# NJU-LHRS/LHRS-Bot

Hardware: AMD Instinct MI355X
Metric: stage-1 pretrain samples/sec (224^2 image + 128-tok caption) (higher is better)
Workload: dtype bf16

## Files before the change

### include/lhrs_hip.h

```cpp
#ifndef LHRS_HIP_H
#define LHRS_HIP_H
#include <stdint.h>
#ifdef __cplusplus
extern "C" {
#endif

typedef uint16_t lhrs_bf16_t;

const char* lhrs_last_error(void);
int lhrs_abi_version(void);
const char* lhrs_target_arch(void);

int lhrs_gemm_bf16_nt(const void* A, int lda, const void* B, int ldb, void* C, int ldc, int M, int N, int K,
                      const void* bias, const void* residual, int ldr, int act, int out_f32, int accumulate,
                      float alpha, void* stream);

int lhrs_gemm_bf16_nt_lora(const void* A, int lda, const void* B, int ldb, const void* A2, int lda2, const void* B2, int ldb2,
                           int K2, void* C, int ldc, int M, int N, int K, const void* bias, const void* residual, int ldr,
                           int out_f32, int accumulate, float alpha, void* stream);
int lhrs_gemm_fp8_nt(const void* A8, long lda, const float* sa, const void* B8, long ldb, const float* sb, void* C, int ldc,
                     int M, int N, int K, const void* residual, int ldr, float alpha, void* stream);
int lhrs_gemm_fp8_nt_lora(const void* A8, long lda, const float* sa, const void* B8, long ldb, const float* sb, const void* A2,
                          int lda2, const void* B2, int ldb2, int K2, void* C, int ldc, int M, int N, int K,
                          const void* residual, int ldr, float alpha, void* stream);
int lhrs_rmsnorm_fwd_q(const void* x, long ldx, const void* w, void* y, long ldy, void* y8, float* y8scale, int rows,
                       int cols, float eps, void* stream);
int lhrs_rmsnorm_bwd_q(const void* dy, const void* x, const void* w, const float* rstd, const void* add, void* dx,
                       void* dx8, float* dx8scale, int rows, int cols, float eps, void* stream);
int lhrs_swiglu_fwd_q(const void* gate_up, void* act, void* act8, float* scale, long rows, int F, void* stream);
int lhrs_swiglu_bwd_q(const void* dact, const void* gate_up, void* dgu, void* dgu8, float* scale, long rows, int F, void* stream);
int lhrs_gemm_skinny_splits(int K, int N);
int lhrs_gemm_bf16_nt_skinny(const void* A, int lda, const void* B, int ldb, void* C, int ldc, int M, int N, int K, float alpha,
                             float* workspace, void* stream);
int lhrs_gemm_splitk_splits(int M, int N, int K);
int lhrs_gemm_tn_splits(int T, int Mo, int No);
int lhrs_gemm_tn_f32(const void* P, long ldp, const void* Q, long ldq, float* C, long ldc, int T, int Mo, int No, float* workspace,
                     void* stream);
int lhrs_gemm_bf16_nt_splitk_f32(const void* A, int lda, const void* B, int ldb, float* C, int ldc, int M, int N, int K,
                                 float* workspace, void* stream);
int lhrs_gemm_swiglu_fusable(int M, int ff, int K_fwd, int K_bwd, int K2);
int lhrs_gemm_swiglu_fwd(const void* X, int ldx, const void* Wgu, int ldw, const void* A2, int lda2, const void* B2, int ldb2,
                         int K2, void* gu, int ld_gu, void* act, int ld_act, int M, int ff, int K, void* stream);
int lhrs_gemm_swiglu_bwd(const void* dY, int ldy, const void* WdT, int ldw, const void* A2, int lda2, const void* B2, int ldb2,
                         int K2, const void* gu, void* dgu, int ld_gu, void* dact_scratch, int M, int ff, int K, void* stream);
int lhrs_gemm_rope_fwd(const void* X, int ldx, const void* W, int ldw, const void* A2, int lda2, const void* B2, int ldb2, int K2,
                       void* C, int ldc, int M, int N, int K, const float* cos_t, const float* sin_t, int pos_mod, int pos0,
                       int rope_cols, int head_dim, void* stream);
int lhrs_dropout_bf16(const void* x, long ldx, void* out, long ldo, long rows, int cols, float p, unsigned seed, void* stream);
int lhrs_gemm_bf16_nt_dropmask(const void* A, int lda, const void* B, int ldb, void* C, int ldc, int M, int N, int K,
                               const void* residual, int ldr, float alpha, float p, unsigned seed, void* stream);
int lhrs_gemm_set_policy(int allow_256);
int lhrs_gemm_set_tail_split(int on);
int lhrs_gemm_set_persistent(int on);

int lhrs_gemm_set_bm144(int mode);
long lhrs_gemm_workspace_bytes(void);
int lhrs_gemm_set_workspace(void* ws, long bytes);
int lhrs_quant_int8_rows(const void* W, long ldw, void* Q, long ldq, float* scale, int N, int K, void* stream);
int lhrs_dequant_int8_rows(const void* Q, long ldq, const float* scale, void* W, long ldw, int N, int K, void* stream);
int lhrs_int8_prepare(const void* X, long ldx, int M, int K, float thr, const void* WQ, long ldwq, const float* wscale, int N, void* XQ,
                      long ldq, float* sx, int* flags, int* idx, int* meta, void* A2, long lda2, void* B2, long ldb2, void* stream);
int lhrs_gemm_int8_nt(const void* A8, long lda, const float* sa, const void* B8, long ldb, const float* sb, const void* A2, int lda2,
                      const void* B2, int ldb2, int K2, const int* k2_dev, void* C, int ldc, int M, int N, int K, const void* residual, int ldr,
                      float alpha, void* stream);
int lhrs_quant4_blocks(const void* W, long n, int fp4, void* packed, float* absmax, void* stream);
int lhrs_dequant4_blocks(const void* packed, const float* absmax, long n, int fp4, void* W, void* stream);
int lhrs_quant8_dynamic(const float* x, long n, const float* code256, void* q, float* absmax2, void* stream);
int lhrs_dequant8_dynamic(const void* q, const float* absmax2, long n, const float* code256, float offset, float* out, void* stream);
int lhrs_gemm_set_small_thresh(int n);
int lhrs_gemm_set_min_tiles(int n);
int lhrs_gemm_profile_enable(int max_samples);
int lhrs_gemm_profile_stride(int n);
int lhrs_gemm_profile_read(double* out5_host);
int lhrs_gemm_profile_read_kinds(double* out30_host);
int lhrs_gemm_set_u4(int on);
int lhrs_gemm_u4_takes(int M, int N, int K, int lda, int ldb, int ldc, int ldr, int has_bias, int act, int out_f32, int accumulate, float alpha);
int lhrs_gemm_u4_nt(const void* A, int lda, const void* B, int ldb, void* C, int ldc, int M, int N, int K, const void* residual, int ldr,
                    void* stream);
int lhrs_gemm_u4_nt_lora(const void* A, int lda, const void* B, int ldb, const void* A2, int lda2, const void* B2, int ldb2, int K2, void* C, int ldc,
                         int M, int N, int K, const void* residual, int ldr, void* stream);
int lhrs_gemm_u4_fused_takes(int kind, int M, int tiles_n, int K, int K2);
int lhrs_gemm_u4_main_rows(int M, int N);
int lhrs_gemm_u4_rope(const void* X, int ldx, const void* W, int ldw, void* C, int ldc, int M, int N, int K, const float* cos_t,
                      const float* sin_t, int pos_mod, int pos0, int rope_cols, void* stream);
int lhrs_gemm_u4_rope_lora(const void* X, int ldx, const void* W, int ldw, const void* A2, int lda2, const void* B2, int ldb2, int K2, void* C, int ldc,
                           int M, int N, int K, const float* cos_t, const float* sin_t, int pos_mod, int pos0, int rope_cols, void* stream);
int lhrs_gemm_u4_swiglu_fwd(const void* X, int ldx, const void* Wgu, int ldw, void* gu, int ld_gu, void* act, int ld_act, int M, int ff, int K,
                            void* stream);
int lhrs_gemm_u4_swiglu_bwd(const void* dY, int ldy, const void* WdT, int ldw, const void* gu, void* dgu, int ld_gu, int M, int ff, int K,
                            void* stream);

int lhrs_tn_skinny_splits(int M, int N);
int lhrs_gemm_tn_skinny(const void* P, long ldp, const void* Q, long ldq, float* C, long ldc, float* partial, int M, int N,
                        int KP, int accumulate, void* stream);
int lhrs_blockdiag_mask(float* g, long ld, int rows, int cols, int r, int w, int active_mask, void* stream);

int lhrs_layernorm_fwd(const void* x, long ldx, const void* gamma, const void* beta, void* y, long ldy, float* mean,
                       float* rstd, int rows, int cols, float eps, void* stream);
int lhrs_layernorm_bwd_nblk(int rows);
int lhrs_layernorm_bwd(const void* dy, long ld_dy, const void* x, long ldx, const void* gamma, const float* mean,
                       const float* rstd, const void* add, void* dx, long ld_dx, float* dgamma, float* dbeta,
                       float* partial, int accumulate, int rows, int cols, void* stream);
int lhrs_rmsnorm_fwd(const void* x, long ldx, const void* w, void* y, long ldy, float* rstd, int rows, int cols,
                     float eps, void* stream);
int lhrs_rmsnorm_bwd(const void* dy, const void* x, const void* w, const float* rstd, const void* add, void* dx,
                     int rows, int cols, float eps, void* stream);

int lhrs_seq_transpose(const void* in, long ld_in, void* out, int cols, int LT, const int* desc, int nseq, int use_kv,
                       void* stream);
int lhrs_attn_fwd(const void* q, long ldq, const void* k, long ldk, const void* v, long ldv, void* o, long ldo, float* lse,
                  const int* desc, int nseq, int H, int D, int max_q, int max_kv, int LTq, int causal, float scale,
                  void* stream);
int lhrs_attn_fwd_kmask(const void* q, long ldq, const void* k, long ldk, const void* v, long ldv, void* o, long ldo,
                        float* lse, const int* desc, int nseq, int H, int D, int max_q, int max_kv, int LTq,
                        int causal, float scale, const unsigned char* key_mask, long ld_mask, void* stream);
int lhrs_attn_delta(const void* o, long ldo, const void* dout, long ld_do, float* delta, const int* desc, int nseq, int H,
                    int D, int max_q, int LTq, void* stream);
int lhrs_attn_bwd(const void* q, long ldq, const void* k, long ldk, const void* v, long ldv, const void* dout,
                  long ld_do, const float* lse, const float* delta, void* dq, long ld_dq, void* dk, long ld_dk, void* dv,
                  long ld_dv, const int* desc, int nseq, int H, int D, int max_q, int max_kv, int LTq, int causal,
                  float scale, void* stream);
int lhrs_attn_bwd_rope(const void* q, long ldq, const void* k, long ldk, const void* v, long ldv, const void* dout,
                       long ld_do, const float* lse, const float* delta, void* dq, long ld_dq, void* dk, long ld_dk, void* dv,
                       long ld_dv, const int* desc, int nseq, int H, int D, int max_q, int max_kv, int LTq, int causal,
                       float scale, const float* cos_t, const float* sin_t, int pos_mod, int pos0, long rows, void* stream);
int lhrs_attn_bwd_o(const void* q, long ldq, const void* k, long ldk, const void* v, long ldv, const void* dout, long ld_do,
                    const void* o, long ldo, const float* lse, float* delta, void* dq, long ld_dq, void* dk, long ld_dk, void* dv,
                    long ld_dv, const int* desc, int nseq, int H, int D, int max_q, int max_kv, int LTq, int causal, float scale,
                    const float* cos_t, const float* sin_t, int pos_mod, int pos0, long rows, void* stream);

int lhrs_patchify(const float* rgb, void* out, int B, int img, int P, int KP, void* stream);
int lhrs_vit_assemble(const void* patch, const void* cls, const void* pos, void* out, int B, int NP, int dim,
                      void* stream);
int lhrs_rope(void* x, long ld, int rows, int nheads, int D, const float* cos_t, const float* sin_t, const int* pos_ids,
              int pos_mod, int pos0, int inverse, void* stream);
int lhrs_swiglu_fwd(const void* gate_up, void* act, long rows, int F, void* stream);
int lhrs_swiglu_bwd(const void* dact, const void* gate_up, void* dgate_up, long rows, int F, void* stream);
int lhrs_map(int op, const void* a, const void* b, void* out, long n, void* stream);
int lhrs_colsum_nsplit(int rows);
int lhrs_colsum(const void* x, long ld, float* out, float* partial, int rows, int cols, int accumulate, void* stream);
int lhrs_cast_f32_to_bf16(const float* in, void* out, long n, void* stream);
int lhrs_cast_bf16_to_f32(const void* in, float* out, long n, void* stream);
int lhrs_transpose(const void* in, long ld_in, void* out, long ld_out, int rows, int cols, int rows_pad, void* stream);
int lhrs_transpose_batched(const long* desc, int n, int total_tiles, void* stream);

int lhrs_pooler_build(const void* query, const void* img, void* t, void* kv, int B, int nq0, int nq1, int nq2, int ni0,
                      int ni1, int ni2, int dim, void* stream);
int lhrs_pooler_query_grad(const void* dt0, const void* dkv, float* dquery, int B, int nq0, int nq1, int nq2, int ni0,
                           int ni1, int ni2, int dim, int accumulate, void* stream);
int lhrs_copy_2d(void* dst, long dst_pitch_bytes, const void* src, long src_pitch_bytes, long width_bytes, long height,
                 void* stream);
int lhrs_debug_poison_lds(unsigned pattern, void* stream);

int lhrs_splice_fwd(const long* ids, const long* labels, const uint8_t* mask, const void* image, const void* embed,
                    void* out_embeds, long* out_labels, uint8_t* out_mask, int* img_pos, int B, int T, int NI, int dim,
                    int S, int vocab, void* stream);
int lhrs_splice_bwd(const void* d_embeds, const int* img_pos, void* d_image, int B, int NI, int dim, int S, void* stream);
int lhrs_splice_map_fwd(const long* ids, const int* src_tok, const int* src_img, const void* image, const void* embed, void* out_embeds, int B,
                        int T, int dim, int S, int vocab, void* stream);
int lhrs_splice_map_bwd(const void* d_embeds, const int* inv, void* d_image, int n_rows, int dim, void* stream);
int lhrs_gather_rows(const void* src, long ld_src, const int* idx, void* dst, long ld_dst, int n, int dim, void* stream);
int lhrs_scatter_rows(const void* src, long ld_src, const int* idx, void* dst, long ld_dst, int n, int dim, void* stream);
int lhrs_argmax_rows(const float* x, long ld, long* out, int n, int V, void* stream);
int lhrs_sample_rows(const float* logits, long ld, long* out, int n, int V,
                     int mode,
                     float temperature, int top_k , float top_p ,
                     float repetition_penalty , unsigned* seen ,
                     unsigned long long seed, const int* step_dev , long step_host,
                     long long* weights_out , void* stream);
int lhrs_cross_entropy(const void* logits, long ld, const int* target, float* row_loss, float* loss_out, void* dlogits,
                       long ld_d, int n, int V, void* stream);

int lhrs_gemv_bf16(const void* W, long ldw, const void* x, long ldx, const void* residual, long ldr, void* y, long ldy, int B,
                   int N, int K, int out_f32, void* stream);
int lhrs_gemv(const void* W, long ldw, const float* wscale, int w_format, const void* x, long ldx, int prologue, const void* norm_w,
              float eps, const void* residual, long ldr, void* y, long ldy, int B, int N, int K, int out_f32, void* stream);
int lhrs_repack_bf16_mfma(const void* W, long ldw, void* out, int N, int K, void* stream);
int lhrs_gemv_set_tuning(int rows_per_wave, int chunks_per_iteration);
int lhrs_quant_fp8_rows(const void* W, long ldw, void* W8, long ld8, float* scale, int N, int K, void* stream);
int lhrs_rope_kv_append(void* qkv, long ld, void* kcache, void* vcache, const float* cos_t, const float* sin_t, const int* pos, int B,
                        int H, int D, int max_ctx, void* stream);
int lhrs_decode_advance(int* state, int* desc, int* pos, int B, int max_ctx, int step_inc, void* stream);
int lhrs_decode_advance_cs(int* state, int* desc, int* pos, const float* cos_t, const float* sin_t, float* cs, int B, int max_ctx,
                           int step_inc, void* stream);
int lhrs_kv_append(const void* qkv, long ld, void* kcache, void* vcache, const int* pos, int B, int d, int max_ctx, void* stream);
int lhrs_decode_emit(const long* next_ids, int* tok32, long* out_ids, int* state, int B, int max_new, void* stream);
int lhrs_graph_begin(void* stream);
int lhrs_graph_end(void* stream, void** exec_out);
int lhrs_graph_launch(void* exec, void* stream);
int lhrs_graph_destroy(void* exec);

int lhrs_sqnorm_nblk(long n);
int lhrs_sqnorm(const float* g, long n, float* partial, float* out, int accumulate, void* stream);
int lhrs_accum_f32(float* y, const float* x, long n, int copy_only, void* stream);
int lhrs_adan_step(float* param, const float* grad, float* exp_avg, float* exp_avg_diff, float* exp_avg_sq,
                   float* pre_grad, void* shadow_bf16, long n, int step, float lr, float beta1, float beta2, float beta3,
                   float eps, float weight_decay, int no_prox, const float* gnorm_sq, float max_norm, float grad_scale,
                   void* stream);
int lhrs_adamw_step(float* param, const float* grad, float* exp_avg, float* exp_avg_sq, void* shadow_bf16, long n,
                    int step, float lr, float beta1, float beta2, float eps, float weight_decay, const float* gnorm_sq,
                    float max_norm, float grad_scale, void* stream);

int lhrs_gemv_fp8_mfma(const void* W8, long ldw, const float* wscale, const void* x8, long ldx, const float* xscale,
                       const void* residual, long ldr, void* y, long ldy, int B, int N, int K, int out_f32, int w_packed, void* stream);
int lhrs_gemv_fp8_mfma_fused(const void* W8, long ldw, const float* wscale, const void* x, long ldx, int prologue, const void* norm_w,
                             float eps, const void* residual, long ldr, void* y, long ldy, int B, int N, int K, int out_f32,
                             int w_packed, void* stream);
int lhrs_repack_fp8_mfma(const void* W8, long ldw, void* out, int N, int K, void* stream);
int lhrs_decode_attn(const void* qkv, long ld, void* kcache, void* vcache, const float* cos_t, const float* sin_t,
                     const int* pos, const unsigned char* key_mask, long ld_mask, void* out, long ldo, int B, int H, int D,
                     int max_ctx, float scale, void* stream);
int lhrs_decode_attn_split(const void* qkv, long ld, void* kcache, void* vcache, const float* cos_t, const float* sin_t,
                           const int* pos, const unsigned char* key_mask, long ld_mask, void* out, long ldo, int B, int H, int D,
                           int max_ctx, float scale, int nsplit, float* part, int* tickets, const float* cs, void* stream);
long lhrs_clip_preprocess_workspace(int H, int W);
int lhrs_clip_preprocess(const unsigned char* img, int H, int W, long row_stride, float* out, void* workspace,
                         long workspace_bytes, void* stream);
long lhrs_image_preprocess_workspace(int H, int W, int short_edge);
int lhrs_image_preprocess(const unsigned char* img, int H, int W, long row_stride, float* out, void* workspace, long workspace_bytes,
                          int short_edge, int crop_round, int rescale_mode, const float* mean, const float* stdv, void* stream);

int lhrs_llama_layer_forward(const void* x, const void* ln1_w, const void* qkv_w, const void* o_w, const void* ln2_w, const void* gu_w,
                             const void* down_w, const float* cos_t, const float* sin_t, const int* desc, int B, int S, int LT, int d,
                             int heads, int ff, float eps, void* h, void* qkv, void* o, float* lse, void* x_mid, void* gu,
                             void* act, void* x_out, void* stream);
int lhrs_vit_layer_forward(void* x, const void* ln1_w, const void* ln1_b, const void* qkv_w, const void* qkv_b, const void* o_w,
                           const void* o_b, const void* ln2_w, const void* ln2_b, const void* fc1_w, const void* fc1_b, const void* fc2_w,
                           const void* fc2_b, const int* desc, int B, int n, int LT, int d, int heads, int ff, void* h, void* qkv, void* o,
                           void* f, void* stream);
int lhrs_llama_layer_backward(const void* dx_out, const void* x_in, const void* x_mid, const void* qkv, const void* o, const float* lse,
                              void* gu, const void* ln1_w, const void* ln2_w, const void* qkv_wT, const void* o_wT, const void* gu_wT,
                              const void* down_wT, const float* cos_t, const float* sin_t, const int* desc, int B, int S, int LT, int d,
                              int heads, int ff, float eps, void* dh, void* d_o, void* dqkv, float* delta, void* dact, void* dx_in,
                              void* stream);

#ifdef __cplusplus
}
#endif
#endif
```

### lhrs_bot_amd/csrc/attention.hip

```cpp
#include "common.h"
#include <type_traits>

namespace {

struct AttnArgs {
  const bf16_t* q; const bf16_t* k; const bf16_t* v; const bf16_t* dout;
  long ldq, ldk, ldv, ldo, ld_do, ld_dq, ld_dk, ld_dv;
  bf16_t* o; bf16_t* dq; bf16_t* dk; bf16_t* dv;
  int LTq;
  float* lse;
  const float* delta;
  const int* desc;
  int H;
  float scale;
  const unsigned char* kmask;
  long ld_kmask;
  const float* rope_cos;
  const float* rope_sin;
  int rope_mod, rope_pos0;
  const bf16_t* o_in;
  long ld_oin;
  float* delta_w;
  int wide;
};
// ... 318 lines not shown
#pragma unroll
    for (int db = 0; db < DB; ++db) store4bf(p + db * 16, dq[db], 1.f);
  }
}

template <int D, bool CAUSAL>
__global__ __launch_bounds__(256) void attn_bwd_dkv_kernel(AttnArgs a) {
  constexpr int KS = D / 32, DB = D / 16;
  __shared__ __attribute__((aligned(16))) char lds_q[64 * D * 2];
  __shared__ __attribute__((aligned(16))) char lds_do[64 * D * 2];
  __shared__ __attribute__((aligned(16))) float lds_lse[64];
  __shared__ __attribute__((aligned(16))) float lds_delta[64];
  const int seq = blockIdx.z, h = blockIdx.y;
  const int* ds = a.desc + seq * 8;
  const int q_off = ds[0], q_len = ds[1], kv_off = ds[2], kv_len = ds[3], kv_rows = ds[4], coff = ds[5];
  const int k0 = blockIdx.x * 64;
  if (k0 >= kv_rows) return;
  const int tid = threadIdx.x, lane = tid & 63, wave = tid >> 6, fr = lane & 15, fg = lane >> 4;
  const int key = k0 + wave * 16 + fr;
  const int key_c = min(key, kv_rows - 1);
  const bf16_t* kp = a.k + (long)(kv_off + key_c) * a.ldk + h * D;
  const bf16_t* vp = a.v + (long)(kv_off + key_c) * a.ldv + h * D;
  bf16x8 kf[KS], vf[KS];
#pragma unroll
  for (int ks = 0; ks < KS; ++ks) {
    kf[ks] = *reinterpret_cast<const bf16x8*>(kp + ks * 32 + fg * 8);
    vf[ks] = *reinterpret_cast<const bf16x8*>(vp + ks * 32 + fg * 8);
  }
  f32x4 dk[DB], dv[DB];
#pragma unroll
  for (int i = 0; i < DB; ++i) { dk[i] = f32x4{0.f, 0.f, 0.f, 0.f}; dv[i] = f32x4{0.f, 0.f, 0.f, 0.f}; }

  const int nq_tiles = (q_len + 63) >> 6;
  int i0 = 0;
  if (CAUSAL) i0 = max(0, (k0 - coff) >> 6);
  const bf16_t* qbase = a.q + (long)q_off * a.ldq + h * D;
  const bf16_t* dobase = a.dout + (long)q_off * a.ld_do + h * D;
  const float* lsebase = a.lse + (long)(seq * a.H + h) * a.LTq;
  const float* deltabase = a.delta + (long)(seq * a.H + h) * a.LTq;
  TrAddr<D> tq, tdo;
  tq.init(lds_q, lane);
  tdo.init(lds_do, lane);
  TileRegs<D> qr, dor;
  float stat_r = 0.f;
  auto prefetch = [&](int i) {
    tile_load<D>(qr, qbase, a.ldq, i * 64, q_len, tid);
    tile_load<D>(dor, dobase, a.ld_do, i * 64, q_len, tid);
    if (tid < 64) stat_r = lsebase[i * 64 + tid];
    else if (tid < 128) stat_r = deltabase[i * 64 + tid - 64];
  };
  if (i0 < nq_tiles) prefetch(i0);

  for (int i = i0; i < nq_tiles; ++i) {
    __syncthreads();
    tile_store<D>(lds_q, qr, tid);
    tile_store<D>(lds_do, dor, tid);
    if (tid < 64) lds_lse[tid] = stat_r;
    else if (tid < 128) lds_delta[tid - 64] = stat_r;
    __syncthreads();
    if (i + 1 < nq_tiles) prefetch(i + 1);
    f32x4 s[4], dp[4];
#pragma unroll
    for (int qb = 0; qb < 4; ++qb) {
      s[qb] = f32x4{0.f, 0.f, 0.f, 0.f};
      dp[qb] = f32x4{0.f, 0.f, 0.f, 0.f};
#pragma unroll
      for (int ks = 0; ks < KS; ++ks) {
        s[qb] = MFMA(frag_rm<D>(lds_q, qb * 16 + fr, ks, fg), kf[ks], s[qb]);
        dp[qb] = MFMA(frag_rm<D>(lds_do, qb * 16 + fr, ks, fg), vf[ks], dp[qb]);
      }
    }
    bf16x4 alo[DB], ahi[DB], blo[DB], bhi[DB];
    tr_issue<D, 0>(tdo, alo, ahi);
#pragma unroll
    for (int qb = 0; qb < 4; ++qb) {
      const f32x4 lq = *reinterpret_cast<const f32x4*>(&lds_lse[qb * 16 + fg * 4]);
      const f32x4 dl = *reinterpret_cast<const f32x4*>(&lds_delta[qb * 16 + fg * 4]);
#pragma unroll
      for (int r = 0; r < 4; ++r) {
        const int q = i * 64 + qb * 16 + fg * 4 + r;
        const bool ok = q < q_len && key < kv_len && (!CAUSAL || key <= q + coff);
        const float p = ok ? __expf(s[qb][r] * a.scale - lq[r]) : 0.f;
        dp[qb][r] = ok ? p * (dp[qb][r] - dl[r]) * a.scale : 0.f;
        s[qb][r] = p;
      }
    }
    const bf16x8 p0 = pack_frag(s[0], s[1]), p1 = pack_frag(s[2], s[3]);
    const bf16x8 d0 = pack_frag(dp[0], dp[1]), d1 = pack_frag(dp[2], dp[3]);
    tr_wait<DB>(alo, ahi);
    tr_issue<D, 0>(tq, blo, bhi);
    __builtin_amdgcn_sched_barrier(0);
#pragma unroll
    for (int db = 0; db < DB; ++db) dv[db] = MFMA(join(alo[db], ahi[db]), p0, dv[db]);
    tr_wait<DB>(blo, bhi);
    tr_issue<D, 1>(tdo, alo, ahi);
    __builtin_amdgcn_sched_barrier(0);
#pragma unroll
    for (int db = 0; db < DB; ++db) dk[db] = MFMA(join(blo[db], bhi[db]), d0, dk[db]);
    tr_wait<DB>(alo, ahi);
    tr_issue<D, 1>(tq, blo, bhi);
    __builtin_amdgcn_sched_barrier(0);
#pragma unroll
    for (int db = 0; db < DB; ++db) dv[db] = MFMA(join(alo[db], ahi[db]), p1, dv[db]);
    tr_wait<DB>(blo, bhi);
#pragma unroll
    for (int db = 0; db < DB; ++db) dk[db] = MFMA(join(blo[db], bhi[db]), d1, dk[db]);
  }
  if (key < kv_rows) {
    bf16_t* pk = a.dk + (long)(kv_off + key) * a.ld_dk + h * D + fg * 4;
    bf16_t* pv = a.dv + (long)(kv_off + key) * a.ld_dv + h * D + fg * 4;
#pragma unroll
    for (int db = 0; db < DB; ++db) { store4bf(pk + db * 16, dk[db], 1.f); store4bf(pv + db * 16, dv[db], 1.f); }
  }
}

template <int D> constexpr int res_rows() { return 163840 / (2 * D * 2); }

template <int D>
__device__ __forceinline__ void res_load(char* lds, const bf16_t* base, long ld, int rows, int len, int lane, int wave) {
  constexpr int CH = D / 8, R = 1024 / (D * 2);
  typedef const __attribute__((address_space(1))) void* gp;
  typedef __attribute__((address_space(3))) void* lp;
  for (int r0 = wave * R; r0 < rows; r0 += 8 * R) {
    const int row = r0 + lane / CH;
    const int c = (lane % CH) ^ swz<D>(row);
    const bf16_t* src = base + (long)min(row, len - 1) * ld + c * 8;
    __builtin_amdgcn_global_load_lds((gp)src, (lp)(lds + r0 * (D * 2)), 16, 0, 0);
  }
}
__device__ __forceinline__ int zigzag_group(int p, int wave, int G, bool descending) {
  const int k = p * 8 + ((p & 1) ? 7 - wave : wave);
  if (k >= G) return -1;
  return descending ? G - 1 - k : k;
}

#ifdef ATTN_DIAG
__device__ unsigned long long* g_attn_dbg = nullptr;
__device__ int g_attn_dbg_sel = 0;
#define DIAG_T(slot) do { if (g_attn_dbg && g_attn_dbg_sel == DIAG_KID && lane == 0) g_attn_dbg[((long)(blockIdx.y * gridDim.x + blockIdx.x) * 8 + wave) * 8 + (slot)] = wall_clock64(); } while (0)
#define DIAG_DECL(id) constexpr int DIAG_KID = id; unsigned long long dg_t = 0, dg_acc[3] = {0, 0, 0}; int dg_units = 0
#define DIAG_MARK() do { asm volatile("s_waitcnt vmcnt(0) lgkmcnt(0)" ::: "memory"); dg_t = wall_clock64(); } while (0)
#define DIAG_ACC(k) do { asm volatile("s_waitcnt vmcnt(0) lgkmcnt(0)" ::: "memory"); const unsigned long long t_ = wall_clock64(); dg_acc[k] += t_ - dg_t; dg_t = t_; } while (0)
#define DIAG_UNITS(n) dg_units += (n)
#define DIAG_FLUSH() do { if (g_attn_dbg && g_attn_dbg_sel == DIAG_KID && lane == 0) { unsigned long long* d_ = g_attn_dbg + ((long)(blockIdx.y * gridDim.x + blockIdx.x) * 8 + wave) * 8; d_[2] = dg_acc[0]; d_[3] = dg_acc[1]; d_[5] = dg_acc[2]; d_[6] = dg_units; } } while (0)
#else
#define DIAG_T(slot) do { } while (0)
#define DIAG_DECL(id)
#define DIAG_MARK() do { } while (0)
#define DIAG_ACC(k) do { } while (0)
#define DIAG_UNITS(n) do { } while (0)
#define DIAG_FLUSH() do { } while (0)
#endif

template <int D, bool CAUSAL>
__global__ __launch_bounds__(512, 2) void attn_fwd_res_kernel(AttnArgs a) {
  constexpr int KS = D / 32, DB = D / 16, TILE = 64 * D * 2;
  __shared__ __attribute__((aligned(16))) char smem[163840];
  char* lds_k = smem;
  char* lds_v = smem + res_rows<D>() * D * 2;
  const int seq = blockIdx.y, h = blockIdx.x;
  const int* ds = a.desc + seq * 8;
  const int q_off = ds[0], q_len = ds[1], kv_off = ds[2], kv_len = ds[3], coff = ds[5];
  const int tid = threadIdx.x, lane = tid & 63, fr = lane & 15, fg = lane >> 4;
  const int wave = __builtin_amdgcn_readfirstlane(tid >> 6);
  DIAG_DECL(0);
  DIAG_T(0);
  int kv_need = kv_len;
  if (CAUSAL) kv_need = max(0, min(kv_len, q_len + coff));
  const int rows = ((kv_need + 63) >> 6) << 6;
  if (rows > 0) {
    res_load<D>(lds_k, a.k + (long)kv_off * a.ldk + h * D, a.ldk, rows, kv_len, lane, wave);
    res_load<D>(lds_v, a.v + (long)kv_off * a.ldv + h * D, a.ldv, rows, kv_len, lane, wave);
  }
  asm volatile("s_waitcnt vmcnt(0)" ::: "memory");
  __syncthreads();
  DIAG_T(1);
  TrAddr<D> tv;
  tv.init(lds_v, lane);
  const float c2 = a.scale * 1.4426950408889634f;
  const int G = (q_len + 15) >> 4;
  for (int p = 0;; ++p) {
    const int g = zigzag_group(p, wave, G, CAUSAL);
    if (g < 0) break;
    DIAG_MARK();
    const int qrow = g * 16 + fr;
    const bf16_t* qp = a.q + (long)(q_off + min(qrow, q_len - 1)) * a.ldq + h * D;
    bf16x8 qf[KS];
#pragma unroll
    for (int ks = 0; ks < KS; ++ks) qf[ks] = *reinterpret_cast<const bf16x8*>(qp + ks * 32 + fg * 8);
    DIAG_ACC(0);
    float m = NEG_INF, l = 0.f;
    f32x4 o[DB];
#pragma unroll
    for (int i = 0; i < DB; ++i) o[i] = f32x4{0.f, 0.f, 0.f, 0.f};
    int kv_end = kv_len;
    if (CAUSAL) kv_end = max(0, min(kv_len, min(g * 16 + 16, q_len) + coff));
    const int ntiles = (kv_end + 63) >> 6;
    for (int j = 0; j < ntiles; ++j) {
      const char* kt = lds_k + j * TILE;
      f32x4 s[4];
#pragma unroll
      for (int nb = 0; nb < 4; ++nb) {
        s[nb] = f32x4{0.f, 0.f, 0.f, 0.f};
#pragma unroll
        for (int ks = 0; ks < KS; ++ks) s[nb] = MFMA(frag_rm<D>(kt, nb * 16 + fr, ks, fg), qf[ks], s[nb]);
      }
      TrAddr<D> tj;
#pragma unroll
      for (int db = 0; db < DB; ++db) tj.base[db] = tv.base[db] + j * TILE;
      bf16x4 v0lo[DB], v0hi[DB], v1lo[DB], v1hi[DB];
      tr_issue<D, 0>(tj, v0lo, v0hi);
      const bool full = (j + 1) * 64 <= kv_len && (!CAUSAL || j * 64 + 63 <= g * 16 + coff);
      if (!full) {
#pragma unroll
        for (int nb = 0; nb < 4; ++nb)
#pragma unroll
          for (int r = 0; r < 4; ++r) {
            const int key = j * 64 + nb * 16 + fg * 4 + r;
            const bool ok = key < kv_len && (!CAUSAL || key <= qrow + coff);
            s[nb][r] = ok ? s[nb][r] : NEG_INF;
          }
      }
      float mx = NEG_INF;
#pragma unroll
      for (int nb = 0; nb < 4; ++nb)
#pragma unroll
        for (int r = 0; r < 4; ++r) mx = fmaxf(mx, s[nb][r]);
      mx = group_max(mx);
      const float m_new = fmaxf(m, mx);
      const float m_use = (m_new == NEG_INF) ? 0.f : m_new;
      const float mc = m_use * c2;
      const float alpha = __builtin_amdgcn_exp2f(m * c2 - mc);
      float rs = 0.f;
#pragma unroll
      for (int nb = 0; nb < 4; ++nb)
#pragma unroll
        for (int r = 0; r < 4; ++r) {
          s[nb][r] = __builtin_amdgcn_exp2f(__builtin_fmaf(s[nb][r], c2, -mc));
          rs += s[nb][r];
        }
      l = l * alpha + rs;
      m = m_new;
#pragma unroll
      for (int i = 0; i < DB; ++i) o[i] *= alpha;
      const bf16x8 p0 = pack_frag(s[0], s[1]), p1 = pack_frag(s[2], s[3]);
      tr_wait<DB>(v0lo, v0hi);
      tr_issue<D, 1>(tj, v1lo, v1hi);
      __builtin_amdgcn_sched_barrier(0);
#pragma unroll
      for (int db = 0; db < DB; ++db) o[db] = MFMA(join(v0lo[db], v0hi[db]), p0, o[db]);
      tr_wait<DB>(v1lo, v1hi);
#pragma unroll
      for (int db = 0; db < DB; ++db) o[db] = MFMA(join(v1lo[db], v1hi[db]), p1, o[db]);
    }
    DIAG_ACC(1);
    DIAG_UNITS(ntiles);
    l = group_sum(l);
    if (qrow < q_len) {
      const float inv = l > 0.f ? 1.f / l : 0.f;
      bf16_t* op = a.o + (long)(q_off + qrow) * a.ldo + h * D;
      if (a.wide) store_row_wide<DB>(op, o, inv, fg);
      else {
#pragma unroll
        for (int db = 0; db < DB; ++db) store4bf(op + fg * 4 + db * 16, o[db], inv);
      }
      if (a.lse && fg == 0) a.lse[(long)(seq * a.H + h) * a.LTq + qrow] = (l > 0.f) ? m * a.scale + __logf(l) : NEG_INF;
    }
    DIAG_ACC(2);
  }
  DIAG_T(4);
  DIAG_FLUSH();
}

template <int D, bool CAUSAL>
__global__ __launch_bounds__(512, 2) void attn_bwd_dq_res_kernel(AttnArgs a) {
  constexpr int KS = D / 32, DB = D / 16, TILE = 64 * D * 2;
  __shared__ __attribute__((aligned(16))) char smem[163840];
  char* lds_k = smem;
  char* lds_v = smem + res_rows<D>() * D * 2;
  const int seq = blockIdx.y, h = blockIdx.x;
  const int* ds = a.desc + seq * 8;
  const int q_off = ds[0], q_len = ds[1], kv_off = ds[2], kv_len = ds[3], coff = ds[5];
  const int tid = threadIdx.x, lane = tid & 63, fr = lane & 15, fg = lane >> 4;
  const int wave = __builtin_amdgcn_readfirstlane(tid >> 6);
  DIAG_DECL(1);
  DIAG_T(0);
  int kv_need = kv_len;
  if (CAUSAL) kv_need = max(0, min(kv_len, q_len + coff));
  const int rows = ((kv_need + 63) >> 6) << 6;
  if (rows > 0) {
    res_load<D>(lds_k, a.k + (long)kv_off * a.ldk + h * D, a.ldk, rows, kv_len, lane, wave);
    res_load<D>(lds_v, a.v + (long)kv_off * a.ldv + h * D, a.ldv, rows, kv_len, lane, wave);
  }
  asm volatile("s_waitcnt vmcnt(0)" ::: "memory");
  __syncthreads();
  DIAG_T(1);
  TrAddr<D> tk;
  tk.init(lds_k, lane);
  const int G = (q_len + 15) >> 4;
  for (int p = 0;; ++p) {
    const int g = zigzag_group(p, wave, G, CAUSAL);
    if (g < 0) break;
    DIAG_MARK();
    const int qrow = g * 16 + fr;
    const int qrow_c = min(qrow, q_len - 1);
    const bf16_t* qp = a.q + (long)(q_off + qrow_c) * a.ldq + h * D;
    const bf16_t* dop = a.dout + (long)(q_off + qrow_c) * a.ld_do + h * D;
    bf16x8 qf[KS], dof[KS];
#pragma unroll
    for (int ks = 0; ks < KS; ++ks) {
      qf[ks] = *reinterpret_cast<const bf16x8*>(qp + ks * 32 + fg * 8);
      dof[ks] = *reinterpret_cast<const bf16x8*>(dop + ks * 32 + fg * 8);
// ... 155 lines not shown
          s[qb] = MFMA(frag_rm<D>(qt, qb * 16 + fr, ks, fg), kf[ks], s[qb]);
          dp[qb] = MFMA(frag_rm<D>(dot, qb * 16 + fr, ks, fg), vf[ks], dp[qb]);
        }
      }
      if (!hf) {
#pragma unroll
        for (int qb = 2; qb < 4; ++qb) {
          s[qb] = f32x4{0.f, 0.f, 0.f, 0.f};
          dp[qb] = f32x4{0.f, 0.f, 0.f, 0.f};
#pragma unroll
          for (int ks = 0; ks < KS; ++ks) {
            s[qb] = MFMA(frag_rm<D>(qt, qb * 16 + fr, ks, fg), kf[ks], s[qb]);
            dp[qb] = MFMA(frag_rm<D>(dot, qb * 16 + fr, ks, fg), vf[ks], dp[qb]);
          }
        }
      }
      TrAddr<D> tqi, tdi;
#pragma unroll
      for (int db = 0; db < DB; ++db) { tqi.base[db] = tq.base[db] + i * TILE; tdi.base[db] = tdo.base[db] + i * TILE; }
      bf16x4 alo[DB], ahi[DB];
      const bool full = (i + 1) * 64 <= q_len && g * 16 + 15 < kv_len && (!CAUSAL || g * 16 + 15 <= i * 64 + coff);
      auto probs = [&](const int qb) {
        const f32x4 lq = *reinterpret_cast<const f32x4*>(lds_lse + i * 64 + qb * 16 + fg * 4);
        const f32x4 dl = *reinterpret_cast<const f32x4*>(lds_delta + i * 64 + qb * 16 + fg * 4);
        if (full) {
#pragma unroll
          for (int r = 0; r < 4; ++r) {
            const float pv = __expf(s[qb][r] * a.scale - lq[r]);
            dp[qb][r] = pv * (dp[qb][r] - dl[r]) * a.scale;
            s[qb][r] = pv;
          }
        } else {
#pragma unroll
          for (int r = 0; r < 4; ++r) {
            const int q = i * 64 + qb * 16 + fg * 4 + r;
            const bool ok = q < q_len && key < kv_len && (!CAUSAL || key <= q + coff);
            const float pv = ok ? __expf(s[qb][r] * a.scale - lq[r]) : 0.f;
            dp[qb][r] = ok ? pv * (dp[qb][r] - dl[r]) * a.scale : 0.f;
            s[qb][r] = pv;
          }
        }
      };
      probs(0); probs(1);
      const bf16x8 p0 = pack_frag(s[0], s[1]), d0 = pack_frag(dp[0], dp[1]);
      tr_issue<D, 0>(tdi, alo, ahi);
      tr_wait<DB>(alo, ahi);
#pragma unroll
      for (int db = 0; db < DB; ++db) dv[db] = MFMA(join(alo[db], ahi[db]), p0, dv[db]);
      __builtin_amdgcn_sched_barrier(0);
      tr_issue<D, 0>(tqi, alo, ahi);
      tr_wait<DB>(alo, ahi);
#pragma unroll
      for (int db = 0; db < DB; ++db) dk[db] = MFMA(join(alo[db], ahi[db]), d0, dk[db]);
      __builtin_amdgcn_sched_barrier(0);
      if (!hf) {
        probs(2); probs(3);
        const bf16x8 p1 = pack_frag(s[2], s[3]), d1 = pack_frag(dp[2], dp[3]);
        tr_issue<D, 1>(tdi, alo, ahi);
        tr_wait<DB>(alo, ahi);
#pragma unroll
        for (int db = 0; db < DB; ++db) dv[db] = MFMA(join(alo[db], ahi[db]), p1, dv[db]);
        __builtin_amdgcn_sched_barrier(0);
        tr_issue<D, 1>(tqi, alo, ahi);
        tr_wait<DB>(alo, ahi);
#pragma unroll
        for (int db = 0; db < DB; ++db) dk[db] = MFMA(join(alo[db], ahi[db]), d1, dk[db]);
        __builtin_amdgcn_sched_barrier(0);
      }
    }
    RopeRow<DB> rr;
    const bool rope = a.rope_cos != nullptr;
    if (rope) rope_row_load<DB>(rr, a, (long)kv_off + key_c, fg);
    DIAG_ACC(1);
    if (key < kv_rows) {
      if (rope) rope_row_apply<DB>(dk, rr);
      bf16_t* pk = a.dk + (long)(kv_off + key) * a.ld_dk + h * D;
      bf16_t* pv = a.dv + (long)(kv_off + key) * a.ld_dv + h * D;
      if (a.wide) { store_row_wide<DB>(pk, dk, 1.f, fg); store_row_wide<DB>(pv, dv, 1.f, fg); }
      else {
#pragma unroll
        for (int db = 0; db < DB; ++db) { store4bf(pk + fg * 4 + db * 16, dk[db], 1.f); store4bf(pv + fg * 4 + db * 16, dv[db], 1.f); }
      }
    }
    DIAG_ACC(2);
  }
  DIAG_T(4);
  DIAG_FLUSH();
}

template <int D>
__global__ void attn_delta_kernel(const bf16_t* __restrict__ o, long ldo, const bf16_t* __restrict__ dout, long ld_do,
                                  float* __restrict__ delta, const int* __restrict__ desc, int H, int LTq) {
  constexpr int TPR = D / 8;
  const int seq = blockIdx.z, h = blockIdx.y;
  const int q_off = desc[seq * 8 + 0], q_len = desc[seq * 8 + 1];
  const int t = blockIdx.x * (256 / TPR) + threadIdx.x / TPR;
  const int c = threadIdx.x % TPR;
  float s = 0.f;
  if (t < q_len) {
    const uint4 a = *reinterpret_cast<const uint4*>(o + (long)(q_off + t) * ldo + h * D + c * 8);
    const uint4 b = *reinterpret_cast<const uint4*>(dout + (long)(q_off + t) * ld_do + h * D + c * 8);
    s = bflo(a.x) * bflo(b.x) + bfhi(a.x) * bfhi(b.x) + bflo(a.y) * bflo(b.y) + bfhi(a.y) * bfhi(b.y) +
        bflo(a.z) * bflo(b.z) + bfhi(a.z) * bfhi(b.z) + bflo(a.w) * bflo(b.w) + bfhi(a.w) * bfhi(b.w);
  }
#pragma unroll
  for (int off = TPR / 2; off > 0; off >>= 1) s += __shfl_xor(s, off, 64);
  if (t < q_len && c == 0) delta[(long)(seq * H + h) * LTq + t] = s;
}

__global__ __launch_bounds__(256) void seq_transpose_kernel(const bf16_t* __restrict__ in, long ld_in, bf16_t* __restrict__ out,
                                                            int cols, int LT, const int* __restrict__ desc, int off_idx,
                                                            int len_idx) {
  __shared__ bf16_t tile[64][66];
  const int seq = blockIdx.z;
  const int off = desc[seq * 8 + off_idx], len = desc[seq * 8 + len_idx];
  const int t0 = blockIdx.x * 64, c0 = blockIdx.y * 64;
  const int tx = threadIdx.x & 63, ty = threadIdx.x >> 6;
  for (int r = ty; r < 64; r += 4) {
    const int t = t0 + r, c = c0 + tx;
    tile[r][tx] = (t < len && c < cols) ? in[(long)(off + t) * ld_in + c] : (bf16_t)0;
  }
  __syncthreads();
  for (int r = ty; r < 64; r += 4) {
    const int c = c0 + r, t = t0 + tx;
    if (c < cols && t < LT) out[((long)seq * cols + c) * LT + t] = tile[tx][r];
  }
}

int check_common(const AttnArgs& a, int D, int nseq, const char* who) {
  LHRS_REQUIRE(D == 64 || D == 128, "%s: head_dim %d unsupported (64 or 128)", who, D);
  LHRS_REQUIRE(nseq > 0 && a.H > 0, "%s: nseq=%d H=%d", who, nseq, a.H);
  LHRS_REQUIRE(a.LTq % 64 == 0, "%s: LTq must be a multiple of 64", who);
  return 0;
}

}

#ifdef ATTN_DIAG
extern "C" int lhrs_attn_set_dbg(void* p, int sel) {
  unsigned long long* v = (unsigned long long*)p;
  if (hipMemcpyToSymbol(HIP_SYMBOL(g_attn_dbg_sel), &sel, sizeof(sel)) != hipSuccess) return -1;
  return hipMemcpyToSymbol(HIP_SYMBOL(g_attn_dbg), &v, sizeof(v)) == hipSuccess ? 0 : -1;
}
#endif
extern "C" int lhrs_seq_transpose(const void* in, long ld_in, void* out, int cols, int LT, const int* desc, int nseq,
                                  int use_kv, void* stream) {
  LHRS_REQUIRE(LT % 64 == 0 && cols > 0 && nseq > 0, "seq_transpose: LT=%d cols=%d nseq=%d", LT, cols, nseq);
  hipLaunchKernelGGL(seq_transpose_kernel, dim3(LT / 64, cdiv(cols, 64), nseq), dim3(256), 0, (hipStream_t)stream,
                     (const bf16_t*)in, ld_in, (bf16_t*)out, cols, LT, desc, use_kv ? 2 : 0, use_kv ? (use_kv == 2 ? 4 : 3) : 1);
  LHRS_CHECK_LAUNCH("seq_transpose");
  return 0;
}

static int attn_fwd_impl(const void* q, long ldq, const void* k, long ldk, const void* v, long ldv, void* o, long ldo,
                         float* lse, const int* desc, int nseq, int H, int D, int max_q, int max_kv, int LTq,
                         int causal, float scale, const unsigned char* key_mask, long ld_mask, void* stream) {
  AttnArgs a; memset(&a, 0, sizeof(a));
  a.kmask = key_mask; a.ld_kmask = ld_mask;
  if (key_mask != nullptr) max_kv = 1 << 30;
  a.q = (const bf16_t*)q; a.ldq = ldq; a.k = (const bf16_t*)k; a.ldk = ldk; a.v = (const bf16_t*)v; a.ldv = ldv;
  a.o = (bf16_t*)o; a.ldo = ldo; a.lse = lse; a.desc = desc; a.H = H; a.LTq = LTq; a.scale = scale;
  a.wide = (ldo % 8 == 0 && (size_t)o % 16 == 0) ? 1 : 0;
  if (check_common(a, D, nseq, "attn_fwd")) return -1;
  const dim3 grid(cdiv(max_q, 64), H, nseq), blk(256);
  hipStream_t s = (hipStream_t)stream;
  if (max_kv > 0 && max_kv <= (D == 128 ? res_rows<128>() : res_rows<64>())) {
    const dim3 rg(H, nseq), rb(512);
    if (D == 128) {
      if (causal) hipLaunchKernelGGL((attn_fwd_res_kernel<128, true>), rg, rb, 0, s, a);
      else hipLaunchKernelGGL((attn_fwd_res_kernel<128, false>), rg, rb, 0, s, a);
    } else {
      if (causal) hipLaunchKernelGGL((attn_fwd_res_kernel<64, true>), rg, rb, 0, s, a);
      else hipLaunchKernelGGL((attn_fwd_res_kernel<64, false>), rg, rb, 0, s, a);
    }
    LHRS_CHECK_LAUNCH("attn_fwd_res");
    return 0;
  }
  if (D == 128) {
    if (causal) hipLaunchKernelGGL((attn_fwd_kernel<128, true>), grid, blk, 0, s, a);
    else hipLaunchKernelGGL((attn_fwd_kernel<128, false>), grid, blk, 0, s, a);
  } else {
    if (causal) hipLaunchKernelGGL((attn_fwd_kernel<64, true>), grid, blk, 0, s, a);
    else hipLaunchKernelGGL((attn_fwd_kernel<64, false>), grid, blk, 0, s, a);
  }
  LHRS_CHECK_LAUNCH("attn_fwd");
  return 0;
}

extern "C" int lhrs_attn_fwd(const void* q, long ldq, const void* k, long ldk, const void* v, long ldv, void* o, long ldo,
                             float* lse, const int* desc, int nseq, int H, int D, int max_q, int max_kv, int LTq,
                             int causal, float scale, void* stream) {
  return attn_fwd_impl(q, ldq, k, ldk, v, ldv, o, ldo, lse, desc, nseq, H, D, max_q, max_kv, LTq, causal, scale, nullptr, 0, stream);
}

extern "C" int lhrs_attn_fwd_kmask(const void* q, long ldq, const void* k, long ldk, const void* v, long ldv, void* o, long ldo,
                                   float* lse, const int* desc, int nseq, int H, int D, int max_q, int max_kv, int LTq,
                                   int causal, float scale, const unsigned char* key_mask, long ld_mask, void* stream) {
  LHRS_REQUIRE(key_mask != nullptr && ld_mask > 0, "attn_fwd_kmask: key_mask=%p ld_mask=%ld", (const void*)key_mask, ld_mask);
  return attn_fwd_impl(q, ldq, k, ldk, v, ldv, o, ldo, lse, desc, nseq, H, D, max_q, max_kv, LTq, causal, scale, key_mask, ld_mask, stream);
}

extern "C" int lhrs_attn_delta(const void* o, long ldo, const void* dout, long ld_do, float* delta, const int* desc,
                               int nseq, int H, int D, int max_q, int LTq, void* stream) {
  LHRS_REQUIRE(D == 64 || D == 128, "attn_delta: head_dim %d", D);
  const int rows_per_blk = 256 / (D / 8);
  const dim3 grid(cdiv(max_q, rows_per_blk), H, nseq);
  if (D == 128)
    hipLaunchKernelGGL((attn_delta_kernel<128>), grid, dim3(256), 0, (hipStream_t)stream, (const bf16_t*)o, ldo,
                       (const bf16_t*)dout, ld_do, delta, desc, H, LTq);
  else
    hipLaunchKernelGGL((attn_delta_kernel<64>), grid, dim3(256), 0, (hipStream_t)stream, (const bf16_t*)o, ldo,
                       (const bf16_t*)dout, ld_do, delta, desc, H, LTq);
  LHRS_CHECK_LAUNCH("attn_delta");
  return 0;
}

extern "C" int lhrs_rope(void* x, long ld, int rows, int nheads, int D, const float* cos_t, const float* sin_t, const int* pos_ids, int pos_mod,
                         int pos0, int inverse, void* stream);

static int attn_bwd_impl(const void* q, long ldq, const void* k, long ldk, const void* v, long ldv,
                         const void* dout, long ld_do, const float* lse, const float* delta, void* dq, long ld_dq,
                         void* dk, long ld_dk, void* dv, long ld_dv, const int* desc, int nseq, int H, int D,
                         int max_q, int max_kv, int LTq, int causal, float scale, const float* rope_cos, const float* rope_sin,
                         int rope_mod, int rope_pos0, long rope_rows, void* stream, const void* o = nullptr, long ldo = 0) {
  AttnArgs a; memset(&a, 0, sizeof(a));
  if (o != nullptr) {
    const int rmax0 = D == 128 ? res_rows<128>() : res_rows<64>();
    if (max_kv <= rmax0) { a.o_in = (const bf16_t*)o; a.ld_oin = ldo; a.delta_w = const_cast<float*>(delta); }
    else if (lhrs_attn_delta(o, ldo, dout, ld_do, const_cast<float*>(delta), desc, nseq, H, D, max_q, LTq, stream)) return -1;
  }
  const bool rope = rope_cos != nullptr;
  const int rmax_ = D == 128 ? res_rows<128>() : res_rows<64>();
  const bool dkv_fits = max_q <= rmax_ && (long)((max_q + 31) / 32 * 32) * D * 2 + 2L * LTq * 4 <= (long)rmax_ * D * 2;
  const bool fuse_rope = rope && max_kv <= rmax_ && dkv_fits;
  if (fuse_rope) { a.rope_cos = rope_cos; a.rope_sin = rope_sin; a.rope_mod = rope_mod; a.rope_pos0 = rope_pos0; }
  a.q = (const bf16_t*)q; a.ldq = ldq; a.k = (const bf16_t*)k; a.ldk = ldk; a.v = (const bf16_t*)v; a.ldv = ldv;
  a.dout = (const bf16_t*)dout; a.ld_do = ld_do; a.lse = (float*)lse; a.delta = delta;
  a.dq = (bf16_t*)dq; a.ld_dq = ld_dq; a.dk = (bf16_t*)dk; a.ld_dk = ld_dk; a.dv = (bf16_t*)dv; a.ld_dv = ld_dv;
  a.desc = desc; a.H = H; a.LTq = LTq; a.scale = scale;
  a.wide = (ld_dq % 8 == 0 && ld_dk % 8 == 0 && ld_dv % 8 == 0 && ((size_t)dq | (size_t)dk | (size_t)dv) % 16 == 0) ? 1 : 0;
  if (check_common(a, D, nseq, "attn_bwd")) return -1;
  hipStream_t s = (hipStream_t)stream;
  const dim3 gq(cdiv(max_q, 64), H, nseq), gk(cdiv(max_kv, 64), H, nseq), blk(256);
  const int rmax = D == 128 ? res_rows<128>() : res_rows<64>();
  const dim3 rg(H, nseq), rb(512);
  bool dq_done = false, dkv_done = false;
  if (max_kv <= rmax) {
    if (D == 128) { if (causal) hipLaunchKernelGGL((attn_bwd_dq_res_kernel<128, true>), rg, rb, 0, s, a); else hipLaunchKernelGGL((attn_bwd_dq_res_kernel<128, false>), rg, rb, 0, s, a); }
    else { if (causal) hipLaunchKernelGGL((attn_bwd_dq_res_kernel<64, true>), rg, rb, 0, s, a); else hipLaunchKernelGGL((attn_bwd_dq_res_kernel<64, false>), rg, rb, 0, s, a); }
    dq_done = true;
  }
  if (dkv_fits) {
    if (D == 128) { if (causal) hipLaunchKernelGGL((attn_bwd_dkv_res_kernel<128, true>), rg, rb, 0, s, a); else hipLaunchKernelGGL((attn_bwd_dkv_res_kernel<128, false>), rg, rb, 0, s, a); }
    else { if (causal) hipLaunchKernelGGL((attn_bwd_dkv_res_kernel<64, true>), rg, rb, 0, s, a); else hipLaunchKernelGGL((attn_bwd_dkv_res_kernel<64, false>), rg, rb, 0, s, a); }
    dkv_done = true;
  }
  if (dq_done && dkv_done) { LHRS_CHECK_LAUNCH("attn_bwd_res"); return 0; }
#define LAUNCH_TILED(KERN, GRID)                                                                 \
  do {                                                                                           \
    if (D == 128) { if (causal) hipLaunchKernelGGL((KERN<128, true>), GRID, blk, 0, s, a); else hipLaunchKernelGGL((KERN<128, false>), GRID, blk, 0, s, a); } \
    else { if (causal) hipLaunchKernelGGL((KERN<64, true>), GRID, blk, 0, s, a); else hipLaunchKernelGGL((KERN<64, false>), GRID, blk, 0, s, a); }          \
  } while (0)
  if (!dq_done) LAUNCH_TILED(attn_bwd_dq_kernel, gq);
  if (!dkv_done) LAUNCH_TILED(attn_bwd_dkv_kernel, gk);
#undef LAUNCH_TILED
  LHRS_CHECK_LAUNCH("attn_bwd");
  if (rope) {
    if (lhrs_rope(dq, ld_dq, (int)rope_rows, H, D, rope_cos, rope_sin, nullptr, rope_mod, rope_pos0, 1, stream)) return -1;
    if (lhrs_rope(dk, ld_dk, (int)rope_rows, H, D, rope_cos, rope_sin, nullptr, rope_mod, rope_pos0, 1, stream)) return -1;
  }
  return 0;
}

extern "C" int lhrs_attn_bwd(const void* q, long ldq, const void* k, long ldk, const void* v, long ldv,
                             const void* dout, long ld_do, const float* lse, const float* delta, void* dq, long ld_dq,
                             void* dk, long ld_dk, void* dv, long ld_dv, const int* desc, int nseq, int H, int D,
                             int max_q, int max_kv, int LTq, int causal, float scale, void* stream) {
  return attn_bwd_impl(q, ldq, k, ldk, v, ldv, dout, ld_do, lse, delta, dq, ld_dq, dk, ld_dk, dv, ld_dv, desc, nseq, H, D, max_q, max_kv, LTq,
                       causal, scale, nullptr, nullptr, 1, 0, 0, stream);
}

extern "C" int lhrs_attn_bwd_rope(const void* q, long ldq, const void* k, long ldk, const void* v, long ldv,
                                  const void* dout, long ld_do, const float* lse, const float* delta, void* dq, long ld_dq,
                                  void* dk, long ld_dk, void* dv, long ld_dv, const int* desc, int nseq, int H, int D,
                                  int max_q, int max_kv, int LTq, int causal, float scale, const float* cos_t, const float* sin_t,
                                  int pos_mod, int pos0, long rows, void* stream) {
  LHRS_REQUIRE(cos_t && sin_t && pos_mod > 0 && rows > 0, "attn_bwd_rope: cos/sin tables, pos_mod=%d, rows=%ld", pos_mod, rows);
  return attn_bwd_impl(q, ldq, k, ldk, v, ldv, dout, ld_do, lse, delta, dq, ld_dq, dk, ld_dk, dv, ld_dv, desc, nseq, H, D, max_q, max_kv, LTq,
                       causal, scale, cos_t, sin_t, pos_mod, pos0, rows, stream);
}

extern "C" int lhrs_attn_bwd_o(const void* q, long ldq, const void* k, long ldk, const void* v, long ldv, const void* dout, long ld_do,
                               const void* o, long ldo, const float* lse, float* delta, void* dq, long ld_dq, void* dk, long ld_dk,
                               void* dv, long ld_dv, const int* desc, int nseq, int H, int D, int max_q, int max_kv, int LTq, int causal,
                               float scale, const float* cos_t, const float* sin_t, int pos_mod, int pos0, long rows, void* stream) {
  LHRS_REQUIRE(o != nullptr && delta != nullptr, "attn_bwd_o: o=%p delta=%p", o, (void*)delta);
  LHRS_REQUIRE(cos_t == nullptr || (sin_t && pos_mod > 0 && rows > 0), "attn_bwd_o: cos/sin tables, pos_mod=%d, rows=%ld", pos_mod, rows);
  return attn_bwd_impl(q, ldq, k, ldk, v, ldv, dout, ld_do, lse, delta, dq, ld_dq, dk, ld_dk, dv, ld_dv, desc, nseq, H, D, max_q, max_kv, LTq,
                       causal, scale, cos_t, sin_t, cos_t ? pos_mod : 1, cos_t ? pos0 : 0, cos_t ? rows : 0, stream, o, ldo);
}
```

### lhrs_bot_amd/csrc/gemm.hip

```cpp
#include "common.h"
#include <array>
#include <map>
#include <type_traits>

namespace {

struct GemmArgs {
  const bf16_t* A;
  const bf16_t* B;
  void* C;
  const bf16_t* bias;
  const bf16_t* res;
  int M, N, K;
  int lda, ldb, ldc, ldr;
  float alpha;
  int act;
  int out_f32;
  int accum;
  int tilesM, tilesN;
  const bf16_t* A2;
  const bf16_t* B2;
  int lda2, ldb2, K2;
  int epi, ff;
  const bf16_t* aux;
// ... 193 lines not shown
  __shared__ __attribute__((aligned(16))) char smem[2 * STAGE];

  const int ntiles = g.tilesM * g.tilesN;
  int t = blockIdx.x;
  if (t >= ntiles) return;
  const int tid = threadIdx.x;
  const int lane = tid & 63;
  const int wave = __builtin_amdgcn_readfirstlane(tid >> 6);

  const bool isA = wave < 8;
  const char* base1 = reinterpret_cast<const char*>(isA ? g.A : g.B);
  const char* base2 = reinterpret_cast<const char*>(isA ? g.A2 : g.B2);
  const long ld1 = isA ? g.lda : g.ldb, ld2 = isA ? g.lda2 : g.ldb2;
  const int rmax = (isA ? g.M : g.N) - 1;
  const int nk1 = g.K / BK;
  const int nk = (g.K + (K2P ? g.K2 : 0)) / BK;
  auto dma_row = [&](int tm_, int tn_, int j) {
    const int row0 = isA ? tm_ * BM : tn_ * BN;
    const int ridx = (wave & 7) * 4 + j;
    int row = min(row0 + ridx * 8 + (lane >> 3), rmax);
    if (EPI == 1 && !isA) {
      const int r = ridx * 8 + (lane >> 3);
      row = ((r >> 5) & 1) * g.ff + tn_ * 128 + (r >> 6) * 32 + (r & 31);
    }
    if (EPI == 3 && !isA && tn_ * BN < g.rope_cols) {
      const int r = ridx * 8 + (lane >> 3);
      row = tn_ * BN + ((r >> 7) << 7) + ((r >> 5) & 1) * 64 + ((r >> 6) & 1) * 32 + (r & 31);
    }
    return row;
  };
  auto dma_rows = [&](int tm_, int tn_, unsigned (&o1)[4]) {
#pragma unroll
    for (int j = 0; j < 4; ++j) {
      const int lchunk = (lane & 7) ^ ((((j & 1) << 2) + (lane >> 4)) & 7);
      o1[j] = (unsigned)(((long)dma_row(tm_, tn_, j) * ld1 + lchunk * 8) * 2);
    }
  };
  const int dst0 = (isA ? 0 : A_BYTES) + (wave & 7) * 4096;
  auto dma_piece = [&](const char* sp, unsigned vo, int buf, int j) {
    const unsigned lds_dst = (unsigned)(size_t)((__attribute__((address_space(3))) char*)smem) + buf * STAGE + dst0 + j * 1024;
    asm volatile("s_mov_b64 s[100:101], %1\n\ts_mov_b32 m0, %2\n\ts_nop 0\n\tglobal_load_lds_dwordx4 %0, s[100:101]" ::"v"(vo), "s"(sp), "s"(lds_dst) : "memory", "m0", "s100", "s101");
  };
  auto issue1 = [&](const unsigned (&o1)[4], int kt, int buf, int j) {
    const int kb_ = __builtin_amdgcn_readfirstlane(kt * (BK * 2));
    dma_piece(base1 + kb_, o1[j], buf, j);
  };
  auto issue2 = [&](int tm_, int tn_, int kt2, int buf, int j) {
    const int kb_ = __builtin_amdgcn_readfirstlane(kt2 * (BK * 2));
    const int lchunk = (lane & 7) ^ ((((j & 1) << 2) + (lane >> 4)) & 7);
    dma_piece(base2 + kb_, (unsigned)(((long)dma_row(tm_, tn_, j) * ld2 + lchunk * 8) * 2), buf, j);
  };

  const int wm = wave >> 2, wn = wave & 3;
  const int sw = ((lane & 15) >> 1) & 7;
  const unsigned lds0 = (unsigned)(size_t)((__attribute__((address_space(3))) char*)smem);
  const unsigned a0 = lds0 + (wm * 64 + (lane & 15)) * 128 + (((lane >> 4)) ^ sw) * 16;
  const unsigned b0 = lds0 + A_BYTES + (wn * 64 + (lane & 15)) * 128 + (((lane >> 4)) ^ sw) * 16;

  const int nkl = nk;
  int tm, tn;
  tile_coords_lin(g, t, ntiles, tm, tn);
  unsigned off1[4];
  dma_rows(tm, tn, off1);
  int pb = 0;
#pragma unroll
  for (int j = 0; j < 4; ++j) issue1(off1, 0, 0, j);
  asm volatile("s_waitcnt vmcnt(0)" ::: "memory");

  bf16x8 A[4], B[4];
#define RDQ(dst, addr, off) asm volatile("ds_read_b128 %0, %1 offset:" #off : "=v"(dst) : "v"(addr))
#define SB __builtin_amdgcn_sched_barrier(0);
#define MF(mi, ni) acc[mi][ni] = __builtin_amdgcn_mfma_f32_16x16x32_bf16(B[ni], A[mi], acc[mi][ni], 0, 0, 0); SB

  for (;;) {
    const int tnext = t + (int)gridDim.x;
    const bool has_next = tnext < ntiles;
    f32x4 acc[4][4];
#pragma unroll
    for (int i = 0; i < 4; ++i)
#pragma unroll
      for (int j = 0; j < 4; ++j) acc[i][j] = f32x4{0.f, 0.f, 0.f, 0.f};

    __builtin_amdgcn_s_barrier();
#pragma unroll
    for (int j = 0; j < 4; ++j) {
      if (!K2P || 1 < nk1) issue1(off1, 1, pb ^ 1, j);
      else issue2(tm, tn, 1 - nk1, pb ^ 1, j);
    }
    {
      const unsigned aa = a0 ^ (unsigned)(pb * STAGE), ba = b0 ^ (unsigned)(pb * STAGE);
      RDQ(A[0], aa, 0); RDQ(A[1], aa, 2048); RDQ(A[2], aa, 4096); RDQ(A[3], aa, 6144);
      RDQ(B[0], ba, 0); RDQ(B[1], ba, 2048); RDQ(B[2], ba, 4096); RDQ(B[3], ba, 6144);
      lds_wait8(A, B);
    }
#define STAGE_S(s_)                                                                                             \
    {                                                                                                           \
      const unsigned so = (((s_) + pb) & 1) * STAGE, sn = so ^ STAGE;                                           \
      { const unsigned aa = a0 ^ (so | 64u), ba = b0 ^ (so | 64u); S_BLOCK0(aa, ba) }                           \
      { const unsigned aa = a0 ^ sn, ba = b0 ^ sn; S_BLOCK1(aa, ba) }                                           \
    }
    const int nA = K2P ? min(nkl - 2, nk1 - 2) : nkl - 2;
#define ISS(j) issue1(off1, s + 2, (s + pb) & 1, j);
    for (int s = 0; s < nA; ++s) STAGE_S(s)
#undef ISS
    if (K2P) {
#define ISS(j) issue2(tm, tn, s + 2 - nk1, (s + pb) & 1, j);
      for (int s = max(nA, 0); s < nkl - 2; ++s) STAGE_S(s)
#undef ISS
    }
    int ntm = 0, ntn = 0;
    if (has_next) {
      tile_coords_lin(g, tnext, ntiles, ntm, ntn);
      dma_rows(ntm, ntn, off1);
    }
#define ISS(j) if (has_next) issue1(off1, 0, (nkl + pb) & 1, j);
    STAGE_S(nkl - 2)
#undef ISS
#undef STAGE_S
    {
      const unsigned so = ((nkl - 1 + pb) & 1) * STAGE;
      { const unsigned aa = a0 ^ (so | 64u), ba = b0 ^ (so | 64u); S_BLOCK0(aa, ba) }
      S_BLOCK1_FINAL(0, 0)
    }

    int le = lane;
    asm volatile("" : "+v"(le));
    const int fr = le & 15, fg = le >> 4;
    if (g.out_f32) {
#pragma unroll
      for (int mi = 0; mi < 4; ++mi) {
        const int m = tm * BM + wm * 64 + mi * 16 + fr;
        if (m >= g.M) continue;
#pragma unroll
        for (int ni = 0; ni < 4; ++ni) {
          const int n = tn * BN + wn * 64 + ni * 16 + fg * 4;
          if (n >= g.N) continue;
          store4<ACT>(g, m, n, acc[mi][ni]);
        }
      }
    } else {
      __builtin_amdgcn_s_barrier();
      char* reg = smem + ((nkl - 1 + pb) & 1) * STAGE + wave * 4096;
      const bool rope_tile = EPI == 3 && tn * BN < g.rope_cols;
      const int rsub = le >> 3, c = le & 7;
      const int n = EPI == 1   ? (c < 4 ? 0 : g.ff) + tn * 128 + wn * 32 + (c & 3) * 8
                    : rope_tile ? tn * BN + (wn >> 1) * 128 + (c < 4 ? 0 : 64) + (wn & 1) * 32 + (c & 3) * 8
                                : tn * BN + wn * 64 + c * 8;
      constexpr bool SWB = EPI == 2;
      const int nlim = SWB ? g.ff : g.N;
      const bool col_ok = n < nlim;
#pragma unroll
      for (int ps = 0; ps < 2; ++ps) {
        uint4 pre_a[4], pre_b[4];
        if (SWB || (EPI == 0 && g.res)) {
#pragma unroll
          for (int i = 0; i < 4; ++i) {
            const int m = tm * BM + wm * 64 + ps * 32 + i * 8 + rsub;
            pre_a[i] = make_uint4(0, 0, 0, 0); pre_b[i] = make_uint4(0, 0, 0, 0);
            if (m < g.M && col_ok) {
              if (SWB) {
                pre_a[i] = *reinterpret_cast<const uint4*>(g.aux + (long)m * g.ld_aux + n);
                pre_b[i] = *reinterpret_cast<const uint4*>(g.aux + (long)m * g.ld_aux + g.ff + n);
              } else {
                pre_a[i] = *reinterpret_cast<const uint4*>(g.res + (long)m * g.ldr + n);
              }
            }
          }
        }
#pragma unroll
        for (int h = 0; h < 2; ++h) {
          const int mi = ps * 2 + h;
          const int row = h * 16 + fr;
          if (rope_tile) {
            const int pos = (tm * BM + wm * 64 + mi * 16 + fr) % g.rope_mod + g.rope_pos0;
#pragma unroll
            for (int ni = 0; ni < 2; ++ni) {
              const float4 c4 = *reinterpret_cast<const float4*>(g.rope_cos + (long)pos * 64 + (wn & 1) * 32 + ni * 16 + fg * 4);
              const float4 s4 = *reinterpret_cast<const float4*>(g.rope_sin + (long)pos * 64 + (wn & 1) * 32 + ni * 16 + fg * 4);
              const float cv[4] = {c4.x, c4.y, c4.z, c4.w}, sv[4] = {s4.x, s4.y, s4.z, s4.w};
              float o1[4], o2[4];
#pragma unroll
              for (int i = 0; i < 4; ++i)
                rope_pair(bf2f(f2bf(acc[mi][ni][i] * g.alpha)), bf2f(f2bf(acc[mi][ni + 2][i] * g.alpha)), cv[i], sv[i], o1[i], o2[i]);
              const int u = ni * 4 + fg;
              *reinterpret_cast<uint2*>(reg + row * 128 + ((u ^ ((row & 7) << 1)) << 3)) = make_uint2(pack2bf(o1[0], o1[1]), pack2bf(o1[2], o1[3]));
              *reinterpret_cast<uint2*>(reg + row * 128 + (((8 + u) ^ ((row & 7) << 1)) << 3)) = make_uint2(pack2bf(o2[0], o2[1]), pack2bf(o2[2], o2[3]));
            }
          } else {
#pragma unroll
            for (int ni = 0; ni < 4; ++ni) {
              float v[4];
              uint2 bb = make_uint2(0, 0);
              if (EPI == 0 && g.bias) bb = *reinterpret_cast<const uint2*>(g.bias + min(tn * BN + wn * 64 + ni * 16 + fg * 4, g.N - 4));
              const float bias_v[4] = {bflo(bb.x), bfhi(bb.x), bflo(bb.y), bfhi(bb.y)};
#pragma unroll
              for (int i = 0; i < 4; ++i) {
                v[i] = acc[mi][ni][i] * g.alpha;
                if (EPI == 0 && g.drop_thresh) {
                  const long e = (long)(tm * BM + wm * 64 + mi * 16 + fr) * g.N + tn * BN + wn * 64 + ni * 16 + fg * 4 + i;
                  v[i] = drop_keep(g.drop_seed, e, g.drop_thresh) ? v[i] * g.drop_scale : 0.f;
                }
                v[i] += bias_v[i];
                if (ACT) v[i] = apply_act(v[i], ACT);
              }
              const int u = ni * 4 + fg;
              *reinterpret_cast<uint2*>(reg + row * 128 + ((u ^ ((row & 7) << 1)) << 3)) = make_uint2(pack2bf(v[0], v[1]), pack2bf(v[2], v[3]));
            }
          }
        }
        asm volatile("s_waitcnt vmcnt(0) lgkmcnt(0)" ::: "memory");
#pragma unroll
        for (int i = 0; i < 4; ++i) {
          const int r32 = i * 8 + rsub;
          const int m = tm * BM + wm * 64 + ps * 32 + r32;
          uint4 val = *reinterpret_cast<const uint4*>(reg + r32 * 128 + ((c ^ (r32 & 7)) << 4));
          if (SWB && m < g.M && col_ok) {
            const uint4 gq = pre_a[i], uq = pre_b[i];
            float d[8], gg[8], uu[8], dg[8], du[8];
            unpack8(val, d); unpack8(gq, gg); unpack8(uq, uu);
#pragma unroll
            for (int e = 0; e < 8; ++e) {
              const float sg = sigmoid_f(gg[e]);
              du[e] = d[e] * gg[e] * sg;
              dg[e] = d[e] * uu[e] * sg * (1.f + gg[e] * (1.f - sg));
            }
            bf16_t* out = reinterpret_cast<bf16_t*>(g.C) + (long)m * g.ldc + n;
            *reinterpret_cast<uint4*>(out) = pack8(dg);
            *reinterpret_cast<uint4*>(out + g.ff) = pack8(du);
          }
          if (SWB) continue;
          if (m < g.M && col_ok) {
            if (EPI == 0 && g.res) {
              const uint4 r = pre_a[i];
              val.x = pack2bf(bflo(val.x) + bflo(r.x), bfhi(val.x) + bfhi(r.x));
              val.y = pack2bf(bflo(val.y) + bflo(r.y), bfhi(val.y) + bfhi(r.y));
              val.z = pack2bf(bflo(val.z) + bflo(r.z), bfhi(val.z) + bfhi(r.z));
              val.w = pack2bf(bflo(val.w) + bflo(r.w), bfhi(val.w) + bfhi(r.w));
            }
            *reinterpret_cast<uint4*>(reinterpret_cast<bf16_t*>(g.C) + (long)m * g.ldc + n) = val;
          }
        }
      }
      if (EPI == 1) {
#pragma unroll
        for (int mi = 0; mi < 4; ++mi) {
          const int row = mi * 16 + fr;
#pragma unroll
          for (int ni = 0; ni < 2; ++ni) {
            float v[4];
#pragma unroll
            for (int i = 0; i < 4; ++i) {
              const float gv = bf2f(f2bf(acc[mi][ni][i] * g.alpha)), uv = bf2f(f2bf(acc[mi][ni + 2][i] * g.alpha));
              v[i] = silu(gv) * uv;
            }
            const int u = ni * 4 + fg;
            *reinterpret_cast<uint2*>(reg + row * 64 + ((u ^ ((row & 3) << 1)) << 3)) = make_uint2(pack2bf(v[0], v[1]), pack2bf(v[2], v[3]));
          }
        }
        asm volatile("s_waitcnt lgkmcnt(0)" ::: "memory");
        const int rsub4 = le >> 2, c4 = le & 3;
        const int n2 = tn * 128 + wn * 32 + c4 * 8;
#pragma unroll
        for (int i = 0; i < 4; ++i) {
          const int row = i * 16 + rsub4;
          const int m = tm * BM + wm * 64 + row;
          const uint4 val = *reinterpret_cast<const uint4*>(reg + row * 64 + ((c4 ^ (row & 3)) << 4));
          if (m < g.M) *reinterpret_cast<uint4*>(g.aux_out + (long)m * g.ld_aux + n2) = val;
        }
      }
    }
    if (!has_next) break;
    if (g.out_f32) asm volatile("s_waitcnt vmcnt(0)" ::: "memory");
    t = tnext; tm = ntm; tn = ntn;
    pb = (pb + nkl) & 1;
  }
#undef MF
#undef SB
#undef RDQ
}



#include "gemm_144s_kernel.inc"

typedef __attribute__((ext_vector_type(8))) int i32x8;

template <bool I8>
__global__ __launch_bounds__(512, 2) void gemm_fp8_256_kernel(GemmArgs g) {
  constexpr int BM = 256, BN = 256, BKB = 128;
  constexpr int A_BYTES = BM * BKB, STAGE = A_BYTES + BN * BKB;
  __shared__ __attribute__((aligned(16))) char smem[2 * STAGE];

  int tm, tn;
  tile_coords(g, tm, tn);
  const int tid = threadIdx.x;
  const int lane = tid & 63;
  const int wave = __builtin_amdgcn_readfirstlane(tid >> 6);

  const bool isA = wave < 4;
  const char* base1 = reinterpret_cast<const char*>(isA ? g.A : g.B);
  const long ld1 = isA ? g.lda : g.ldb;
  const int row0 = isA ? tm * BM : tn * BN, rmax = (isA ? g.M : g.N) - 1;
  const char* base2 = reinterpret_cast<const char*>(isA ? g.A2 : g.B2);
  const long ld2 = (isA ? g.lda2 : g.ldb2) * 2L;
  const int nk1 = g.K / BKB;
  const int K2 = g.K2 + (g.k2_dev ? __builtin_amdgcn_readfirstlane(g.k2_dev[0]) : 0);
  unsigned off1[8], off2[8];
#pragma unroll
  for (int j = 0; j < 8; ++j) {
    const int ridx = (wave & 3) * 8 + j;
    const int lchunk = (lane & 7) ^ ((((j & 1) << 2) + (lane >> 4)) & 7);
    const int row = min(row0 + ridx * 8 + (lane >> 3), rmax);
    off1[j] = (unsigned)((long)row * ld1 + lchunk * 16);
    off2[j] = K2 > 0 ? (unsigned)((long)row * ld2 + lchunk * 16) : 0u;
  }
  const int dst0 = (isA ? 0 : A_BYTES) + (wave & 3) * 8192;
  const int nk_all = nk1 + K2 / 64;
  auto issue1 = [&](int kt, int j) {
    if (kt >= nk_all) return;
    const char* p = kt < nk1 ? base1 + (long)kt * BKB + off1[j] : base2 + (long)(kt - nk1) * BKB + off2[j];
    __builtin_amdgcn_global_load_lds((gptr_t)p, (lptr_t)(smem + (kt & 1) * STAGE + dst0 + j * 1024), 16, 0, 0);
  };

  const int wm = wave >> 2, wn = wave & 3;
  const int fr = lane & 31, fh = lane >> 5;
  const int sw = (fr >> 1) & 7;
  const unsigned lds0 = (unsigned)(size_t)((__attribute__((address_space(3))) char*)smem);
  const unsigned a_base = lds0 + (wm * 128 + fr) * 128;
  const unsigned b_base = lds0 + A_BYTES + (wn * 64 + fr) * 128;
  unsigned kofs[2][2];
#pragma unroll
  for (int ks = 0; ks < 2; ++ks)
#pragma unroll
    for (int hh = 0; hh < 2; ++hh) kofs[ks][hh] = ((ks * 4 + fh * 2 + hh) ^ sw) * 16;

  f32x16 acc[4][2];
#pragma unroll
  for (int i = 0; i < 4; ++i)
#pragma unroll
    for (int j = 0; j < 2; ++j)
#pragma unroll
      for (int r = 0; r < 16; ++r) acc[i][j][r] = 0.f;

  i32x8 a0[4], b0[2], a1[4], b1[2];
  typedef const __attribute__((address_space(3))) i32x4* lds4_t;
#define RD8(dst, addr0, addr1, off)                                                                                  \
  do {                                                                                                               \
    const i32x4 lo_ = *reinterpret_cast<lds4_t>((size_t)((addr0) + (off)));                                          \
    const i32x4 hi_ = *reinterpret_cast<lds4_t>((size_t)((addr1) + (off)));                                          \
    dst = i32x8{lo_[0], lo_[1], lo_[2], lo_[3], hi_[0], hi_[1], hi_[2], hi_[3]};                                     \
  } while (0)
  typedef __attribute__((ext_vector_type(16))) int i32x16_t;
#define MF8(A_, B_, mi, ni)                                                                                          \
  if constexpr (I8) {                                                                                                \
    i32x16_t c_ = __builtin_bit_cast(i32x16_t, acc[mi][ni]);                                                         \
    c_ = __builtin_amdgcn_mfma_i32_32x32x32_i8(__builtin_shufflevector(B_[ni], B_[ni], 0, 1, 2, 3),                  \
                                               __builtin_shufflevector(A_[mi], A_[mi], 0, 1, 2, 3), c_, 0, 0, 0);   \
    c_ = __builtin_amdgcn_mfma_i32_32x32x32_i8(__builtin_shufflevector(B_[ni], B_[ni], 4, 5, 6, 7),                  \
                                               __builtin_shufflevector(A_[mi], A_[mi], 4, 5, 6, 7), c_, 0, 0, 0);   \
    acc[mi][ni] = __builtin_bit_cast(f32x16, c_);                                                                    \
  } else {                                                                                                           \
    acc[mi][ni] = __builtin_amdgcn_mfma_scale_f32_32x32x64_f8f6f4(B_[ni], A_[mi], acc[mi][ni], 0, 0, 0, 0x7F7F7F7F, 0, 0x7F7F7F7F); \
  }                                                                                                                  \
  __builtin_amdgcn_sched_barrier(0);
#define SB8 __builtin_amdgcn_sched_barrier(0);
#define BLOCK8(Ac, Bc, An, Bn, aa0, aa1, ba0, ba1, RD, kd, d0, NDMA)                                       \
  MF8(Ac, Bc, 0, 0) if (RD) RD8(Bn[0], ba0, ba1, 0);     if (NDMA > 0) issue1(kd, d0);     SB8             \
  MF8(Ac, Bc, 0, 1) if (RD) RD8(Bn[1], ba0, ba1, 4096);  if (NDMA > 1) issue1(kd, d0 + 1); SB8             \
  MF8(Ac, Bc, 1, 0) if (RD) RD8(An[0], aa0, aa1, 0);     if (NDMA > 2) issue1(kd, d0 + 2); SB8             \
  MF8(Ac, Bc, 1, 1) if (RD) RD8(An[1], aa0, aa1, 4096);  if (NDMA > 3) issue1(kd, d0 + 3); SB8             \
  MF8(Ac, Bc, 2, 0) if (RD) RD8(An[2], aa0, aa1, 8192);  if (NDMA > 4) issue1(kd, d0 + 4); SB8             \
  MF8(Ac, Bc, 2, 1) if (RD) RD8(An[3], aa0, aa1, 12288); if (NDMA > 5) issue1(kd, d0 + 5); SB8             \
  MF8(Ac, Bc, 3, 0)                                      if (NDMA > 6) issue1(kd, d0 + 6); SB8             \
  MF8(Ac, Bc, 3, 1)                                      if (NDMA > 7) issue1(kd, d0 + 7); SB8

  const int nk = nk1;
#pragma unroll
  for (int j = 0; j < 8; ++j) issue1(0, j);
  asm volatile("s_waitcnt vmcnt(0)" ::: "memory");
  __builtin_amdgcn_s_barrier();
#pragma unroll
  for (int j = 0; j < 8; ++j) issue1(1, j);
  {
    const unsigned aa0 = a_base + kofs[0][0], aa1 = a_base + kofs[0][1], ba0 = b_base + kofs[0][0], ba1 = b_base + kofs[0][1];
    RD8(b0[0], ba0, ba1, 0); RD8(b0[1], ba0, ba1, 4096);
    RD8(a0[0], aa0, aa1, 0); RD8(a0[1], aa0, aa1, 4096); RD8(a0[2], aa0, aa1, 8192); RD8(a0[3], aa0, aa1, 12288);
  }
  {
    const unsigned aa0 = a_base + kofs[1][0], aa1 = a_base + kofs[1][1], ba0 = b_base + kofs[1][0], ba1 = b_base + kofs[1][1];
    BLOCK8(a0, b0, a1, b1, aa0, aa1, ba0, ba1, true, 0, 0, 0)
  }
  auto stage = [&](int kt) {
// ... 517 lines not shown
      const dim3 grid16 = grid_256s((long)g.tilesM * g.tilesN);
      switch (act) {
        case 0: LAUNCH_256(0, 0, grid16, s, g); break;
        case 1: LAUNCH_256(1, 0, grid16, s, g); break;
        case 2: LAUNCH_256(2, 0, grid16, s, g); break;
        default: LAUNCH_256(3, 0, grid16, s, g); break;
      }
    }
  } else if (big) LAUNCH_TILE(4, 4);
  else if (t64x128 >= g_gemm_small_thresh) LAUNCH_TILE(2, 4);
  else LAUNCH_TILE(2, 2);
#undef LAUNCH_TILE
  if (slot >= 0) (void)hipEventRecord(g_prof.ev[2 * slot + 1], s);
  LHRS_CHECK_LAUNCH("gemm_bf16_nt");
  return 0;
}


extern "C" int lhrs_swiglu_fwd(const void* gate_up, void* act, long rows, int F, void* stream);
extern "C" int lhrs_swiglu_bwd(const void* dact, const void* gate_up, void* dgate_up, long rows, int F, void* stream);
extern "C" int lhrs_rope(void* x, long ld, int rows, int nheads, int D, const float* cos_t, const float* sin_t, const int* pos_ids, int pos_mod,
                         int pos0, int inverse, void* stream);

static bool swiglu_fusable(long tiles, int ff, int K, int K2, int lda, int ldb) {
  return g_gemm_allow_256 == 2 && ff % 256 == 0 && K % 64 == 0 && K2 % 64 == 0 && K + K2 >= 128 && tiles >= g_gemm_min256 &&
         lda % 8 == 0 && ldb % 8 == 0;
}
extern "C" int lhrs_gemm_swiglu_fusable(int M, int ff, int K_fwd, int K_bwd, int K2) {
  const long tf = (long)cdiv(M, 256) * (ff / 128), tb = (long)cdiv(M, 256) * cdiv(ff, 256);
  return swiglu_fusable(tf, ff, K_fwd, K2, 8, 8) && swiglu_fusable(tb, ff, K_bwd, K2, 8, 8);
}

static int prof_count(int M, int N, int K, int kind, hipStream_t s) {
  if (!g_prof.on) return -1;
  g_prof.launches_all++; g_prof.total_flops_all += 2.0 * M * N * K;
  if (g_prof.used >= g_prof.cap || !g_prof.take(kind)) return -1;
  const int slot = g_prof.used++;
  g_prof.flops[slot] = 2.0 * M * N * K; g_prof.kind[slot] = kind;
  (void)hipEventRecord(g_prof.ev[2 * slot], s);
  return slot;
}
static void prof_end(int slot, hipStream_t s) {
  if (slot >= 0) (void)hipEventRecord(g_prof.ev[2 * slot + 1], s);
}
static void prof_undo(int slot, int kind, double flops) {
  if (!g_prof.on) return;
  g_prof.launches_all--; g_prof.total_flops_all -= flops;
  if (slot >= 0) g_prof.used--;
  if (slot >= 0 || g_prof.used < g_prof.cap) g_prof.seen[kind]--;
}

extern "C" int lhrs_gemm_swiglu_fwd(const void* X, int ldx, const void* Wgu, int ldw, const void* A2, int lda2, const void* B2, int ldb2,
                                    int K2, void* gu, int ld_gu, void* act, int ld_act, int M, int ff, int K, void* stream) {
  LHRS_REQUIRE(M > 0 && ff > 0 && K > 0 && ff % 8 == 0 && ld_gu >= 2 * ff && ld_act >= ff && ld_gu % 8 == 0 && ld_act % 8 == 0,
               "gemm_swiglu_fwd: M=%d ff=%d K=%d ld_gu=%d ld_act=%d", M, ff, K, ld_gu, ld_act);
  if (ff % 128 == 0 && lhrs_gemm_u4_fused_takes(1, M, ff / 128, K, K2))
    U4_FUSED_TRY(7, 2 * ff, lhrs_gemm_u4_swiglu_fwd(X, ldx, Wgu, ldw, gu, ld_gu, act, ld_act, M, ff, K, stream))
  if (!swiglu_fusable((long)cdiv(M, 256) * (ff / 128), ff, K, K2, ldx, ldw)) {
    if (gemm_launch(X, ldx, Wgu, ldw, gu, ld_gu, M, 2 * ff, K, nullptr, nullptr, 0, 0, 0, 0, 1.f, A2, lda2, B2, ldb2, K2, stream)) return -1;
    LHRS_REQUIRE(ld_gu == 2 * ff && ld_act == ff, "gemm_swiglu_fwd: the unfused fallback needs dense gu / act");
    return lhrs_swiglu_fwd(gu, act, M, ff, stream);
  }
  const bool bm144 = pick_144(M, ff / 128, K, K2, false);
  if (!bm144 && t_split_ok && g_gemm_tail_split && ld_gu == 2 * ff && ld_act == ff) {
    const int tm = cdiv(M, 256), tn = ff / 128;
    const long T = (long)tm * tn, rounds = (T + 255) / 256, full = T / 256;
    const int tm_main = (int)(full * 256 / tn);
    if (full >= 1 && T % 256 != 0 && tm_main >= 1 && tm_main < tm) {
      const long t_main = (long)tm_main * tn, t_tail = T - t_main;
      if ((double)((t_main + 255) / 256) + 2.5 * (double)t_tail / 256.0 + 0.05 < (double)rounds) {
        const int M_main = tm_main * 256, M_tail = M - M_main;
        t_split_ok = false;
        int rc = lhrs_gemm_swiglu_fwd(X, ldx, Wgu, ldw, A2, lda2, B2, ldb2, K2, gu, ld_gu, act, ld_act, M_main, ff, K, stream);
        t_split_ok = true;
        if (rc) return rc;
        bf16_t* gu_t = (bf16_t*)gu + (long)M_main * ld_gu;
        if (gemm_launch((const bf16_t*)X + (long)M_main * ldx, ldx, Wgu, ldw, gu_t, ld_gu, M_tail, 2 * ff, K, nullptr, nullptr, 0, 0, 0, 0, 1.f,
                        A2 ? (const bf16_t*)A2 + (long)M_main * lda2 : nullptr, lda2, B2, ldb2, K2, stream))
          return -1;
        return lhrs_swiglu_fwd(gu_t, (bf16_t*)act + (long)M_main * ld_act, M_tail, ff, stream);
      }
    }
  }
  GemmArgs g; memset(&g, 0, sizeof(g));
  g.A = (const bf16_t*)X; g.B = (const bf16_t*)Wgu; g.C = gu; g.M = M; g.N = 2 * ff; g.K = K; g.lda = ldx; g.ldb = ldw; g.ldc = ld_gu;
  g.alpha = 1.f; g.A2 = (const bf16_t*)A2; g.B2 = (const bf16_t*)B2; g.lda2 = lda2; g.ldb2 = ldb2; g.K2 = K2;
  g.epi = 1; g.ff = ff; g.aux_out = (bf16_t*)act; g.ld_aux = ld_act;
  g.tilesM = cdiv(M, bm144 ? 144 : 256); g.tilesN = ff / 128;
  hipStream_t s = (hipStream_t)stream;
  const int pslot = prof_count(M, 2 * ff, K + K2, 1, s);
  if (bm144) LAUNCH_144(0, 1, grid_256s((long)g.tilesM * g.tilesN), s, g);
  else LAUNCH_256(0, 1, grid_256s((long)g.tilesM * g.tilesN), s, g);
  prof_end(pslot, s);
  LHRS_CHECK_LAUNCH("gemm_swiglu_fwd");
  return 0;
}

extern "C" int lhrs_gemm_rope_fwd(const void* X, int ldx, const void* W, int ldw, const void* A2, int lda2, const void* B2, int ldb2, int K2,
                                  void* C, int ldc, int M, int N, int K, const float* cos_t, const float* sin_t, int pos_mod, int pos0,
                                  int rope_cols, int head_dim, void* stream) {
  LHRS_REQUIRE(M > 0 && N > 0 && K > 0 && head_dim % 16 == 0 && rope_cols >= 0 && rope_cols <= N && rope_cols % head_dim == 0 && pos_mod > 0 &&
                   cos_t && sin_t && ldc % 8 == 0,
               "gemm_rope_fwd: M=%d N=%d K=%d rope_cols=%d head_dim=%d pos_mod=%d", M, N, K, rope_cols, head_dim, pos_mod);
  const long tiles = (long)cdiv(M, 256) * cdiv(N, 256);
  const bool fused = g_gemm_allow_256 == 2 && head_dim == 128 && rope_cols % 256 == 0 && N % 8 == 0 && K % 64 == 0 &&
                     K2 % 64 == 0 && K + K2 >= 128 && tiles >= g_gemm_min256 && ldx % 8 == 0 && ldw % 8 == 0;
  if (!fused) {
    if (gemm_launch(X, ldx, W, ldw, C, ldc, M, N, K, nullptr, nullptr, 0, 0, 0, 0, 1.f, A2, lda2, B2, ldb2, K2, stream)) return -1;
    if (rope_cols == 0) return 0;
    return lhrs_rope(C, ldc, M, rope_cols / head_dim, head_dim, cos_t, sin_t, nullptr, pos_mod, pos0, 0, stream);
  }
  if (head_dim == 128 && rope_cols % 256 == 0 && lhrs_gemm_u4_fused_takes(0, M, cdiv(N, 256), K, K2))
    U4_FUSED_TRY(9, N, K2 > 0 ? lhrs_gemm_u4_rope_lora(X, ldx, W, ldw, A2, lda2, B2, ldb2, K2, C, ldc, M, N, K, cos_t, sin_t, pos_mod, pos0, rope_cols, stream)
                              : lhrs_gemm_u4_rope(X, ldx, W, ldw, C, ldc, M, N, K, cos_t, sin_t, pos_mod, pos0, rope_cols, stream))
  GemmArgs g; memset(&g, 0, sizeof(g));
  g.A = (const bf16_t*)X; g.B = (const bf16_t*)W; g.C = C; g.M = M; g.N = N; g.K = K; g.lda = ldx; g.ldb = ldw; g.ldc = ldc;
  g.alpha = 1.f; g.A2 = (const bf16_t*)A2; g.B2 = (const bf16_t*)B2; g.lda2 = lda2; g.ldb2 = ldb2; g.K2 = K2;
  g.epi = 3; g.rope_cos = cos_t; g.rope_sin = sin_t; g.rope_mod = pos_mod; g.rope_pos0 = pos0; g.rope_cols = rope_cols;
  const bool bm144 = pick_144(M, cdiv(N, 256), K, K2, false);
  g.tilesM = cdiv(M, bm144 ? 144 : 256); g.tilesN = cdiv(N, 256);
  const int pslot = prof_count(M, N, K + K2, 3, (hipStream_t)stream);
  if (bm144) LAUNCH_144(0, 3, grid_256s((long)g.tilesM * g.tilesN), (hipStream_t)stream, g);
  else LAUNCH_256(0, 3, grid_256s((long)g.tilesM * g.tilesN), (hipStream_t)stream, g);
  prof_end(pslot, (hipStream_t)stream);
  LHRS_CHECK_LAUNCH("gemm_rope_fwd");
  return 0;
}

extern "C" int lhrs_gemm_swiglu_bwd(const void* dY, int ldy, const void* WdT, int ldw, const void* A2, int lda2, const void* B2, int ldb2,
                                    int K2, const void* gu, void* dgu, int ld_gu, void* dact_scratch, int M, int ff, int K, void* stream) {
  LHRS_REQUIRE(M > 0 && ff > 0 && K > 0 && ff % 8 == 0 && ld_gu >= 2 * ff && ld_gu % 8 == 0, "gemm_swiglu_bwd: M=%d ff=%d K=%d ld_gu=%d", M, ff, K, ld_gu);
  if (lhrs_gemm_u4_fused_takes(2, M, cdiv(ff, 256), K, K2))
    U4_FUSED_TRY(8, ff, lhrs_gemm_u4_swiglu_bwd(dY, ldy, WdT, ldw, gu, dgu, ld_gu, M, ff, K, stream))
  if (!swiglu_fusable((long)cdiv(M, 256) * cdiv(ff, 256), ff, K, K2, ldy, ldw)) {
    LHRS_REQUIRE(dact_scratch != nullptr && ld_gu == 2 * ff, "gemm_swiglu_bwd: the unfused fallback needs a [M, ff] scratch and dense gu");
    if (gemm_launch(dY, ldy, WdT, ldw, dact_scratch, ff, M, ff, K, nullptr, nullptr, 0, 0, 0, 0, 1.f, A2, lda2, B2, ldb2, K2, stream)) return -1;
    return lhrs_swiglu_bwd(dact_scratch, gu, dgu, M, ff, stream);
  }
  GemmArgs g; memset(&g, 0, sizeof(g));
  g.A = (const bf16_t*)dY; g.B = (const bf16_t*)WdT; g.C = dgu; g.M = M; g.N = ff; g.K = K; g.lda = ldy; g.ldb = ldw; g.ldc = ld_gu;
  g.alpha = 1.f; g.A2 = (const bf16_t*)A2; g.B2 = (const bf16_t*)B2; g.lda2 = lda2; g.ldb2 = ldb2; g.K2 = K2;
  g.epi = 2; g.ff = ff; g.aux = (const bf16_t*)gu; g.ld_aux = ld_gu;
  const bool bm144 = pick_144(M, cdiv(ff, 256), K, K2, false);
  g.tilesM = cdiv(M, bm144 ? 144 : 256); g.tilesN = cdiv(ff, 256);
  hipStream_t s = (hipStream_t)stream;
  const int pslot = prof_count(M, ff, K + K2, 2, s);
  if (bm144) LAUNCH_144(0, 2, grid_256s((long)g.tilesM * g.tilesN), s, g);
  else LAUNCH_256(0, 2, grid_256s((long)g.tilesM * g.tilesN), s, g);
  prof_end(pslot, s);
  LHRS_CHECK_LAUNCH("gemm_swiglu_bwd");
  return 0;
}

template <int WM_FR, int WN_FR>
__global__ __launch_bounds__(256) void gemm_fp8_small_kernel(GemmArgs g) {
  constexpr int BM = WM_FR * 32, BN = WN_FR * 32, ROWB = 128;
  constexpr int A_BYTES = BM * ROWB, B_BYTES = BN * ROWB, STAGE = A_BYTES + B_BYTES;
  __shared__ __attribute__((aligned(16))) char smem[2 * STAGE];
  int tm, tn;
  tile_coords(g, tm, tn);
  const int tid = threadIdx.x;
  const int lane = tid & 63;
  const int wave = __builtin_amdgcn_readfirstlane(tid >> 6);
  constexpr int A_INSTR = BM / 32, B_INSTR = BN / 32;
  const int lrow = lane >> 3;
  const int lchunk = (lane & 7) ^ lrow;
  const char *a_src[A_INSTR], *b_src[B_INSTR], *a2_src[A_INSTR], *b2_src[B_INSTR];
#pragma unroll
  for (int i = 0; i < A_INSTR; ++i) {
    const int row = min(tm * BM + (wave * A_INSTR + i) * 8 + lrow, g.M - 1);
    a_src[i] = reinterpret_cast<const char*>(g.A) + (long)row * g.lda + lchunk * 16;
    a2_src[i] = reinterpret_cast<const char*>(g.A2) + ((long)row * g.lda2 + lchunk * 8) * 2;
  }
#pragma unroll
  for (int i = 0; i < B_INSTR; ++i) {
    const int row = min(tn * BN + (wave * B_INSTR + i) * 8 + lrow, g.N - 1);
    b_src[i] = reinterpret_cast<const char*>(g.B) + (long)row * g.ldb + lchunk * 16;
    b2_src[i] = reinterpret_cast<const char*>(g.B2) + ((long)row * g.ldb2 + lchunk * 8) * 2;
  }
  const int nk1 = g.K / 128, nk = nk1 + g.K2 / 64;
  auto issue = [&](int kt) {
    char* sa = smem + (kt & 1) * STAGE;
    char* sb = sa + A_BYTES;
    const bool e4 = kt < nk1;
    const long ko = (long)(e4 ? kt : kt - nk1) * ROWB;
#pragma unroll
    for (int i = 0; i < A_INSTR; ++i)
      __builtin_amdgcn_global_load_lds((gptr_t)((e4 ? a_src[i] : a2_src[i]) + ko), (lptr_t)(sa + (wave * A_INSTR + i) * 1024), 16, 0, 0);
#pragma unroll
    for (int i = 0; i < B_INSTR; ++i)
      __builtin_amdgcn_global_load_lds((gptr_t)((e4 ? b_src[i] : b2_src[i]) + ko), (lptr_t)(sb + (wave * B_INSTR + i) * 1024), 16, 0, 0);
  };
  const int wm = wave >> 1, wn = wave & 1;
  const int fr = lane & 15, fg = lane >> 4;
  const int a_row0 = wm * (WM_FR * 16) + fr, b_row0 = wn * (WN_FR * 16) + fr;
  f32x4 acc[WM_FR][WN_FR];
#pragma unroll
  for (int i = 0; i < WM_FR; ++i)
#pragma unroll
    for (int j = 0; j < WN_FR; ++j) acc[i][j] = f32x4{0.f, 0.f, 0.f, 0.f};
  issue(0);
  for (int kt = 0; kt < nk; ++kt) {
    asm volatile("s_waitcnt vmcnt(0)" ::: "memory");
    __syncthreads();
    if (kt + 1 < nk) issue(kt + 1);
    const char* sa = smem + (kt & 1) * STAGE;
    const char* sb = sa + A_BYTES;
    if (kt < nk1) {
      const int c0 = ((2 * fg) ^ (fr & 7)) * 16, c1 = ((2 * fg + 1) ^ (fr & 7)) * 16;
      i32x8 af[WM_FR], bfr[WN_FR];
#pragma unroll
      for (int mi = 0; mi < WM_FR; ++mi) {
        const i32x4 lo = *reinterpret_cast<const i32x4*>(sa + (a_row0 + mi * 16) * ROWB + c0), hi = *reinterpret_cast<const i32x4*>(sa + (a_row0 + mi * 16) * ROWB + c1);
        af[mi] = i32x8{lo[0], lo[1], lo[2], lo[3], hi[0], hi[1], hi[2], hi[3]};
      }
#pragma unroll
      for (int ni = 0; ni < WN_FR; ++ni) {
        const i32x4 lo = *reinterpret_cast<const i32x4*>(sb + (b_row0 + ni * 16) * ROWB + c0), hi = *reinterpret_cast<const i32x4*>(sb + (b_row0 + ni * 16) * ROWB + c1);
        bfr[ni] = i32x8{lo[0], lo[1], lo[2], lo[3], hi[0], hi[1], hi[2], hi[3]};
      }
#pragma unroll
      for (int mi = 0; mi < WM_FR; ++mi)
#pragma unroll
        for (int ni = 0; ni < WN_FR; ++ni)
          acc[mi][ni] = __builtin_amdgcn_mfma_scale_f32_16x16x128_f8f6f4(bfr[ni], af[mi], acc[mi][ni], 0, 0, 0, 0x7F7F7F7F, 0, 0x7F7F7F7F);
      if (kt + 1 == nk1 && g.K2 > 0) {
#pragma unroll
        for (int mi = 0; mi < WM_FR; ++mi) {
          const float sam = g.sa[min(tm * BM + wm * (WM_FR * 16) + mi * 16 + fr, g.M - 1)];
#pragma unroll
          for (int ni = 0; ni < WN_FR; ++ni) {
            const float4 s4 = *reinterpret_cast<const float4*>(g.sb + min(tn * BN + wn * (WN_FR * 16) + ni * 16 + fg * 4, g.N - 4));
            acc[mi][ni][0] *= sam * s4.x; acc[mi][ni][1] *= sam * s4.y; acc[mi][ni][2] *= sam * s4.z; acc[mi][ni][3] *= sam * s4.w;
          }
        }
      }
    } else {
#pragma unroll
      for (int kk = 0; kk < 2; ++kk) {
        const int ko = ((kk * 4 + fg) ^ (fr & 7)) * 16;
        bf16x8 af[WM_FR], bfr[WN_FR];
#pragma unroll
        for (int mi = 0; mi < WM_FR; ++mi) af[mi] = *reinterpret_cast<const bf16x8*>(sa + (a_row0 + mi * 16) * ROWB + ko);
#pragma unroll
        for (int ni = 0; ni < WN_FR; ++ni) bfr[ni] = *reinterpret_cast<const bf16x8*>(sb + (b_row0 + ni * 16) * ROWB + ko);
#pragma unroll
        for (int mi = 0; mi < WM_FR; ++mi)
#pragma unroll
          for (int ni = 0; ni < WN_FR; ++ni) acc[mi][ni] = __builtin_amdgcn_mfma_f32_16x16x32_bf16(bfr[ni], af[mi], acc[mi][ni], 0, 0, 0);
      }
    }
  }
  const bool scaled = g.K2 > 0;
#pragma unroll
  for (int mi = 0; mi < WM_FR; ++mi) {
    const int m = tm * BM + wm * (WM_FR * 16) + mi * 16 + fr;
    if (m >= g.M) continue;
    const float sam = (scaled ? 1.f : g.sa[m]) * g.alpha;
#pragma unroll
    for (int ni = 0; ni < WN_FR; ++ni) {
      const int n = tn * BN + wn * (WN_FR * 16) + ni * 16 + fg * 4;
      if (n >= g.N) continue;
      float4 s4 = scaled ? make_float4(1.f, 1.f, 1.f, 1.f) : *reinterpret_cast<const float4*>(g.sb + n);
      uint2 o = make_uint2(pack2bf(acc[mi][ni][0] * sam * s4.x, acc[mi][ni][1] * sam * s4.y), pack2bf(acc[mi][ni][2] * sam * s4.z, acc[mi][ni][3] * sam * s4.w));
      if (g.res) {
        const uint2 r = *reinterpret_cast<const uint2*>(g.res + (long)m * g.ldr + n);
        o.x = pack2bf(bflo(o.x) + bflo(r.x), bfhi(o.x) + bfhi(r.x));
        o.y = pack2bf(bflo(o.y) + bflo(r.y), bfhi(o.y) + bfhi(r.y));
      }
      *reinterpret_cast<uint2*>(reinterpret_cast<bf16_t*>(g.C) + (long)m * g.ldc + n) = o;
    }
  }
}

static int gemm_fp8_launch(const void* A8, long lda, const float* sa, const void* B8, long ldb, const float* sb, const void* A2, int lda2,
                           const void* B2, int ldb2, int K2, void* C, int ldc, int M, int N, int K, const void* residual, int ldr,
                           float alpha, void* stream, bool i8 = false, const int* k2_dev = nullptr) {
  LHRS_REQUIRE(M > 0 && N > 0 && K >= 256 && K % 128 == 0, "gemm_fp8: M=%d N=%d K=%d (K %% 128 == 0, K >= 256)", M, N, K);
  LHRS_REQUIRE(lda % 16 == 0 && ldb % 16 == 0 && lda >= K && ldb >= K && sa && sb, "gemm_fp8: lda=%ld ldb=%ld", lda, ldb);
  LHRS_REQUIRE(N % 8 == 0 && ldc % 8 == 0 && ldc >= N && (residual == nullptr || ldr % 8 == 0), "gemm_fp8: N=%d ldc=%d ldr=%d", N, ldc, ldr);
  LHRS_REQUIRE((K2 == 0 && !k2_dev) || (A2 && B2 && K2 % 64 == 0 && lda2 % 8 == 0 && ldb2 % 8 == 0 && lda2 >= K2 && ldb2 >= K2),
               "gemm_fp8: bad bf16 pair (K2=%d lda2=%d ldb2=%d)", K2, lda2, ldb2);
  if (!i8 && t_split_ok && g_gemm_tail_split) {
    const int tm = cdiv(M, 256), tn = cdiv(N, 256);
    const long T = (long)tm * tn, rounds = (T + 255) / 256, full = T / 256;
    const int tm_main = (int)(full * 256 / tn);
    if (full >= 1 && T % 256 != 0 && tm_main >= 1 && tm_main < tm) {
      const long t_main = (long)tm_main * tn, t_tail = T - t_main;
      if ((double)((t_main + 255) / 256) + 2.5 * (double)t_tail / 256.0 + 0.05 < (double)rounds) {
        const int M_main = tm_main * 256;
        t_split_ok = false;
        int rc = gemm_fp8_launch(A8, lda, sa, B8, ldb, sb, A2, lda2, B2, ldb2, K2, C, ldc, M_main, N, K, residual, ldr, alpha, stream);
        t_split_ok = true;
        if (rc) return rc;
        GemmArgs h; memset(&h, 0, sizeof(h));
        h.A = (const bf16_t*)((const char*)A8 + (long)M_main * lda); h.B = (const bf16_t*)B8; h.C = (bf16_t*)C + (long)M_main * ldc;
        h.res = residual ? (const bf16_t*)residual + (long)M_main * ldr : nullptr;
        h.M = M - M_main; h.N = N; h.K = K; h.lda = (int)lda; h.ldb = (int)ldb; h.ldc = ldc; h.ldr = ldr; h.alpha = alpha; h.sa = sa + M_main; h.sb = sb;
        h.A2 = A2 ? (const bf16_t*)A2 + (long)M_main * lda2 : nullptr; h.B2 = (const bf16_t*)B2; h.lda2 = lda2; h.ldb2 = ldb2; h.K2 = K2;
        h.tilesM = cdiv(h.M, 64); h.tilesN = cdiv(N, 128);
        if (g_prof.on) { g_prof.launches_all++; g_prof.total_flops_all += 2.0 * h.M * N * (K + K2); }
        hipLaunchKernelGGL((gemm_fp8_small_kernel<2, 4>), dim3(h.tilesM * h.tilesN), dim3(256), 0, (hipStream_t)stream, h);
        LHRS_CHECK_LAUNCH("gemm_fp8_nt (tail rows)");
        return 0;
      }
    }
// ... 96 lines not shown
```

### lhrs_bot_amd/csrc/gemm_144s_kernel.inc

```
template <int ACT, int EPI>
__global__ __launch_bounds__(768, 1) void gemm_nt_144s_kernel(GemmArgs g) {
  constexpr int FM = 3, NW = 12;
  constexpr int BM = 144, BN = 256, BK = 64;
  constexpr int A_BYTES = BM * BK * 2, STAGE = A_BYTES + BN * BK * 2, NBUF = 3;
  constexpr int NPA = BM / 8, NP = NPA + BN / 8;
  __shared__ __attribute__((aligned(16))) char smem[NBUF * STAGE];

  const int ntiles = g.tilesM * g.tilesN;
  int t = blockIdx.x;
  if (t >= ntiles) return;
  const int tid = threadIdx.x;
  const int lane = tid & 63;
  const int wave = __builtin_amdgcn_readfirstlane(tid >> 6);
  const int nk = g.K / BK;

  const int grp = wave >= 6 ? 1 : 0, w6 = wave - 6 * grp;
  const bool has9 = w6 + 48 < NP;
  auto dma_rows = [&](int tm_, int tn_, unsigned (&o1)[9]) {
#pragma unroll
    for (int j = 0; j < 9; ++j) {
      const int q = w6 + 6 * j;
      const bool pa = q < NPA;
      const int rb = pa ? q : q - NPA;
      const int r = rb * 8 + (lane >> 3);
// ... 7 lines not shown
      }
      const int lchunk = (lane & 7) ^ ((((rb & 1) << 2) + (lane >> 4)) & 7);
      o1[j] = (unsigned)(((long)row * (pa ? g.lda : g.ldb) + lchunk * 8) * 2);
    }
  };
  const char* const baseA = reinterpret_cast<const char*>(g.A);
  const char* const baseB = reinterpret_cast<const char*>(g.B);
  auto issue = [&](const unsigned (&o1)[9], int kt, int buf, int j) {
    const int kb_ = __builtin_amdgcn_readfirstlane(kt * (BK * 2));
    const int q = w6 + 6 * j;
    const char* sp = (q < NPA ? baseA : baseB) + kb_;
    const unsigned lds_dst = (unsigned)(size_t)((__attribute__((address_space(3))) char*)smem) + buf * STAGE + q * 1024;
    asm volatile("s_mov_b64 s[100:101], %1\n\ts_mov_b32 m0, %2\n\ts_nop 0\n\tglobal_load_lds_dwordx4 %0, s[100:101]" ::"v"(o1[j]), "s"(sp), "s"(lds_dst) : "memory", "m0", "s100", "s101");
  };
  auto issue_stage = [&](const unsigned (&o1)[9], int kt, int buf) {
#pragma unroll
    for (int j = 0; j < 8; ++j) issue(o1, kt, buf, j);
    if (has9) issue(o1, kt, buf, 8);
  };

  const int wm = wave >> 2, wn = wave & 3;
  const int sw = ((lane & 15) >> 1) & 7;
  const unsigned lds0 = (unsigned)(size_t)((__attribute__((address_space(3))) char*)smem);
  const unsigned a0 = lds0 + (wm * (FM * 16) + (lane & 15)) * 128 + (((lane >> 4)) ^ sw) * 16;
  const unsigned b0 = lds0 + A_BYTES + (wn * 64 + (lane & 15)) * 128 + (((lane >> 4)) ^ sw) * 16;

  int tm, tn;
  tile_coords_lin(g, t, ntiles, tm, tn);
  unsigned off1[9];
  dma_rows(tm, tn, off1);
  int cb = 0;
  int par = 0;
  issue_stage(off1, grp, grp);
  asm volatile("s_waitcnt vmcnt(0)" ::: "memory");

  bf16x8 A0[3], A1[3], B0[4], B1[4];
#define RDQ(dst, addr, off) asm volatile("ds_read_b128 %0, %1 offset:" #off : "=v"(dst) : "v"(addr)); SB
#define SB __builtin_amdgcn_sched_barrier(0);
#define MFS(S_, mi, ni) acc[mi][ni] = __builtin_amdgcn_mfma_f32_16x16x32_bf16(B##S_[ni], A##S_[mi], acc[mi][ni], 0, 0, 0); SB
#define T_BLOCK0(aa, ba)                                                                          \
  asm volatile("s_waitcnt lgkmcnt(5)" : "+v"(A0[0]), "+v"(B0[0])); SB                              \
  MFS(0, 0, 0) RDQ(A1[0], aa, 0)                                                                  \
  asm volatile("s_waitcnt lgkmcnt(5)" : "+v"(A0[1])); SB                                           \
  MFS(0, 1, 0) RDQ(B1[0], ba, 0)                                                                  \
  asm volatile("s_waitcnt lgkmcnt(5)" : "+v"(A0[2])); SB                                           \
  MFS(0, 2, 0) RDQ(A1[1], aa, 2048)                                                               \
  asm volatile("s_waitcnt lgkmcnt(5)" : "+v"(B0[1])); SB                                           \
  MFS(0, 0, 1) RDQ(A1[2], aa, 4096)                                                               \
  MFS(0, 1, 1) MFS(0, 2, 1)                                                                       \
  asm volatile("s_waitcnt lgkmcnt(5)" : "+v"(B0[2])); SB                                           \
  MFS(0, 0, 2) RDQ(B1[1], ba, 2048)                                                               \
  MFS(0, 1, 2) MFS(0, 2, 2)                                                                       \
  asm volatile("s_waitcnt lgkmcnt(5)" : "+v"(B0[3])); SB                                           \
  MFS(0, 0, 3) RDQ(B1[2], ba, 4096)                                                               \
  MFS(0, 1, 3) RDQ(B1[3], ba, 6144)                                                               \
  MFS(0, 2, 3)
#define T_BLOCK1(aa, ba)                                                                          \
  asm volatile("s_waitcnt lgkmcnt(0)" : "+v"(A1[0]), "+v"(A1[1]), "+v"(A1[2]), "+v"(B1[0]), "+v"(B1[1]), "+v"(B1[2]), "+v"(B1[3])); \
  if (issuer) asm volatile("s_waitcnt vmcnt(0)" ::: "memory");                                     \
  __builtin_amdgcn_s_barrier(); SB                                                                \
  MFS(1, 0, 0) { ISS(0) } SB                                                                      \
  MFS(1, 1, 0) { ISS(1) } SB                                                                      \
  MFS(1, 2, 0) { ISS(2) } SB                                                                      \
  MFS(1, 0, 1) { ISS(3) } SB                                                                      \
  MFS(1, 1, 1) { ISS(4) } SB                                                                      \
  MFS(1, 2, 1) { ISS(5) } SB RDQ(A0[0], aa, 0)                                                    \
  MFS(1, 0, 2) { ISS(6) } SB RDQ(B0[0], ba, 0)                                                    \
  MFS(1, 1, 2) { ISS(7) } SB RDQ(A0[1], aa, 2048)                                                 \
  MFS(1, 2, 2) { ISS(8) } SB RDQ(A0[2], aa, 4096)                                                 \
  MFS(1, 0, 3) RDQ(B0[1], ba, 2048)                                                               \
  MFS(1, 1, 3) RDQ(B0[2], ba, 4096)                                                               \
  MFS(1, 2, 3) RDQ(B0[3], ba, 6144)
#define T_BLOCK1_FINAL                                                                            \
  asm volatile("s_waitcnt lgkmcnt(0)" : "+v"(A1[0]), "+v"(A1[1]), "+v"(A1[2]), "+v"(B1[0]), "+v"(B1[1]), "+v"(B1[2]), "+v"(B1[3])); SB \
  MFS(1, 0, 0) MFS(1, 1, 0) MFS(1, 2, 0) MFS(1, 0, 1) MFS(1, 1, 1) MFS(1, 2, 1)                    \
  MFS(1, 0, 2) MFS(1, 1, 2) MFS(1, 2, 2) MFS(1, 0, 3) MFS(1, 1, 3) MFS(1, 2, 3)

  for (;;) {
    const int tnext = t + (int)gridDim.x;
    const bool has_next = tnext < ntiles;
    f32x4 acc[3][4];
#pragma unroll
    for (int i = 0; i < 3; ++i)
#pragma unroll
      for (int j = 0; j < 4; ++j) acc[i][j] = f32x4{0.f, 0.f, 0.f, 0.f};

    __builtin_amdgcn_s_barrier();
    int b0i = cb, b1i = cb == 2 ? 0 : cb + 1, b2i = b1i == 2 ? 0 : b1i + 1;
    if (grp == par) issue_stage(off1, 2, b2i);
    {
      const unsigned aa = a0 + (unsigned)(b0i * STAGE), ba = b0 + (unsigned)(b0i * STAGE);
      RDQ(A0[0], aa, 0) RDQ(B0[0], ba, 0) RDQ(A0[1], aa, 2048) RDQ(A0[2], aa, 4096) RDQ(B0[1], ba, 2048) RDQ(B0[2], ba, 4096) RDQ(B0[3], ba, 6144)
    }
#define STAGE_T                                                                                                 \
    {                                                                                                           \
      const unsigned so = (unsigned)(b0i * STAGE), sn = (unsigned)(b1i * STAGE);                                \
      { const unsigned aa = (a0 + so) ^ 64u, ba = (b0 + so) ^ 64u; T_BLOCK0(aa, ba) }                           \
      { const unsigned aa = a0 + sn, ba = b0 + sn; const bool issuer = grp != par; T_BLOCK1(aa, ba) }          \
      const int t_ = b0i; b0i = b1i; b1i = b2i; b2i = t_; par ^= 1;                                             \
    }
#define ISS(j) if (issuer && ((j) < 8 || has9)) issue(off1, s + 3, b0i, j);
    for (int s = 0; s < nk - 3; ++s) STAGE_T
#undef ISS
    int ntm = 0, ntn = 0;
    if (has_next) {
      tile_coords_lin(g, tnext, ntiles, ntm, ntn);
      dma_rows(ntm, ntn, off1);
    }
#define ISS(j) if (issuer && has_next && ((j) < 8 || has9)) issue(off1, 0, b0i, j);
    STAGE_T
#undef ISS
#define ISS(j) if (issuer && has_next && ((j) < 8 || has9)) issue(off1, 1, b0i, j);
    STAGE_T
#undef ISS
#undef STAGE_T
    const int last_buf = b0i;
    {
      const unsigned so = (unsigned)(b0i * STAGE);
      { const unsigned aa = (a0 + so) ^ 64u, ba = (b0 + so) ^ 64u; T_BLOCK0(aa, ba) }
      T_BLOCK1_FINAL
      par ^= 1;
    }

    int le = lane;
    asm volatile("" : "+v"(le));
    const int fr = le & 15, fg = le >> 4;
    if (g.out_f32) {
#pragma unroll
      for (int mi = 0; mi < FM; ++mi) {
        const int m = tm * BM + wm * (FM * 16) + mi * 16 + fr;
        if (m >= g.M) continue;
#pragma unroll
        for (int ni = 0; ni < 4; ++ni) {
          const int n = tn * BN + wn * 64 + ni * 16 + fg * 4;
          if (n >= g.N) continue;
          store4<ACT>(g, m, n, acc[mi][ni]);
        }
      }
    } else {
      __builtin_amdgcn_s_barrier();
      char* reg = smem + last_buf * STAGE + wave * 4096;
      const bool rope_tile = EPI == 3 && tn * BN < g.rope_cols;
      const int rsub = le >> 3, c = le & 7;
      const int n = EPI == 1   ? (c < 4 ? 0 : g.ff) + tn * 128 + wn * 32 + (c & 3) * 8
                    : rope_tile ? tn * BN + (wn >> 1) * 128 + (c < 4 ? 0 : 64) + (wn & 1) * 32 + (c & 3) * 8
                                : tn * BN + wn * 64 + c * 8;
      const int nlim = EPI == 2 ? g.ff : g.N;
      const bool col_ok = n < nlim;
      const int mrow0 = tm * BM + wm * (FM * 16);
#pragma unroll
      for (int ps = 0; ps < 2; ++ps) {
        constexpr int NH[2] = {2, 1};
        uint4 pre_a[4], pre_b[4];
        if (EPI == 2 || (EPI == 0 && g.res)) {
#pragma unroll
          for (int i = 0; i < 2 * NH[ps]; ++i) {
            const int m = mrow0 + ps * 32 + i * 8 + rsub;
            pre_a[i] = make_uint4(0, 0, 0, 0); pre_b[i] = make_uint4(0, 0, 0, 0);
            if (m < g.M && col_ok) {
              if (EPI == 2) {
                pre_a[i] = *reinterpret_cast<const uint4*>(g.aux + (long)m * g.ld_aux + n);
                pre_b[i] = *reinterpret_cast<const uint4*>(g.aux + (long)m * g.ld_aux + g.ff + n);
              } else {
                pre_a[i] = *reinterpret_cast<const uint4*>(g.res + (long)m * g.ldr + n);
              }
            }
          }
        }
#pragma unroll
        for (int h = 0; h < NH[ps]; ++h) {
          const int mi = ps * 2 + h;
          const int row = h * 16 + fr;
          if (rope_tile) {
            const int pos = (mrow0 + mi * 16 + fr) % g.rope_mod + g.rope_pos0;
#pragma unroll
            for (int ni = 0; ni < 2; ++ni) {
              const float4 c4 = *reinterpret_cast<const float4*>(g.rope_cos + (long)pos * 64 + (wn & 1) * 32 + ni * 16 + fg * 4);
              const float4 s4 = *reinterpret_cast<const float4*>(g.rope_sin + (long)pos * 64 + (wn & 1) * 32 + ni * 16 + fg * 4);
              const float cv[4] = {c4.x, c4.y, c4.z, c4.w}, sv[4] = {s4.x, s4.y, s4.z, s4.w};
              float o1[4], o2[4];
#pragma unroll
              for (int i = 0; i < 4; ++i)
                rope_pair(bf2f(f2bf(acc[mi][ni][i] * g.alpha)), bf2f(f2bf(acc[mi][ni + 2][i] * g.alpha)), cv[i], sv[i], o1[i], o2[i]);
              const int u = ni * 4 + fg;
              *reinterpret_cast<uint2*>(reg + row * 128 + ((u ^ ((row & 7) << 1)) << 3)) = make_uint2(pack2bf(o1[0], o1[1]), pack2bf(o1[2], o1[3]));
              *reinterpret_cast<uint2*>(reg + row * 128 + (((8 + u) ^ ((row & 7) << 1)) << 3)) = make_uint2(pack2bf(o2[0], o2[1]), pack2bf(o2[2], o2[3]));
            }
          } else {
#pragma unroll
            for (int ni = 0; ni < 4; ++ni) {
              float v[4];
              uint2 bb = make_uint2(0, 0);
              if (EPI == 0 && g.bias) bb = *reinterpret_cast<const uint2*>(g.bias + min(tn * BN + wn * 64 + ni * 16 + fg * 4, g.N - 4));
              const float bias_v[4] = {bflo(bb.x), bfhi(bb.x), bflo(bb.y), bfhi(bb.y)};
#pragma unroll
              for (int i = 0; i < 4; ++i) {
                v[i] = acc[mi][ni][i] * g.alpha;
                v[i] += bias_v[i];
                if (ACT) v[i] = apply_act(v[i], ACT);
              }
              const int u = ni * 4 + fg;
              *reinterpret_cast<uint2*>(reg + row * 128 + ((u ^ ((row & 7) << 1)) << 3)) = make_uint2(pack2bf(v[0], v[1]), pack2bf(v[2], v[3]));
            }
          }
        }
        asm volatile("s_waitcnt vmcnt(0) lgkmcnt(0)" ::: "memory");
#pragma unroll
        for (int i = 0; i < 2 * NH[ps]; ++i) {
          const int r32 = i * 8 + rsub;
          const int m = mrow0 + ps * 32 + r32;
          uint4 val = *reinterpret_cast<const uint4*>(reg + r32 * 128 + ((c ^ (r32 & 7)) << 4));
          if (m < g.M && col_ok) {
            if (EPI == 2) {
              const uint4 gq = pre_a[i], uq = pre_b[i];
              float d[8], gg[8], uu[8], dg[8], du[8];
              unpack8(val, d); unpack8(gq, gg); unpack8(uq, uu);
#pragma unroll
              for (int e = 0; e < 8; ++e) {
                const float sg = sigmoid_f(gg[e]);
                du[e] = d[e] * gg[e] * sg;
                dg[e] = d[e] * uu[e] * sg * (1.f + gg[e] * (1.f - sg));
              }
              bf16_t* out = reinterpret_cast<bf16_t*>(g.C) + (long)m * g.ldc + n;
              *reinterpret_cast<uint4*>(out) = pack8(dg);
              *reinterpret_cast<uint4*>(out + g.ff) = pack8(du);
              continue;
            }
            if (EPI == 0 && g.res) {
              const uint4 r = pre_a[i];
              val.x = pack2bf(bflo(val.x) + bflo(r.x), bfhi(val.x) + bfhi(r.x));
              val.y = pack2bf(bflo(val.y) + bflo(r.y), bfhi(val.y) + bfhi(r.y));
              val.z = pack2bf(bflo(val.z) + bflo(r.z), bfhi(val.z) + bfhi(r.z));
              val.w = pack2bf(bflo(val.w) + bflo(r.w), bfhi(val.w) + bfhi(r.w));
            }
            *reinterpret_cast<uint4*>(reinterpret_cast<bf16_t*>(g.C) + (long)m * g.ldc + n) = val;
          }
        }
      }
      if (EPI == 1) {
#pragma unroll
        for (int mi = 0; mi < FM; ++mi) {
          const int row = mi * 16 + fr;
#pragma unroll
          for (int ni = 0; ni < 2; ++ni) {
            float v[4];
#pragma unroll
            for (int i = 0; i < 4; ++i) {
              const float gv = bf2f(f2bf(acc[mi][ni][i] * g.alpha)), uv = bf2f(f2bf(acc[mi][ni + 2][i] * g.alpha));
              v[i] = silu(gv) * uv;
            }
            const int u = ni * 4 + fg;
            *reinterpret_cast<uint2*>(reg + row * 64 + ((u ^ ((row & 3) << 1)) << 3)) = make_uint2(pack2bf(v[0], v[1]), pack2bf(v[2], v[3]));
          }
        }
        asm volatile("s_waitcnt lgkmcnt(0)" ::: "memory");
        const int rsub4 = le >> 2, c4 = le & 3;
        const int n2 = tn * 128 + wn * 32 + c4 * 8;
#pragma unroll
        for (int i = 0; i < FM; ++i) {
          const int row = i * 16 + rsub4;
          const int m = mrow0 + row;
          const uint4 val = *reinterpret_cast<const uint4*>(reg + row * 64 + ((c4 ^ (row & 3)) << 4));
          if (m < g.M) *reinterpret_cast<uint4*>(g.aux_out + (long)m * g.ld_aux + n2) = val;
        }
      }
    }
    if (!has_next) break;
    if (g.out_f32) asm volatile("s_waitcnt vmcnt(0)" ::: "memory");
    t = tnext; tm = ntm; tn = ntn;
    cb = b1i;
  }
#undef T_BLOCK0
#undef T_BLOCK1
#undef T_BLOCK1_FINAL
#undef MFS
#undef SB
#undef RDQ
}
```

### lhrs_bot_amd/csrc/gemm_tn.hip

```cpp
#include "common.h"

namespace {

typedef const __attribute__((address_space(1))) void* gptr_t;
typedef __attribute__((address_space(3))) void* lptr_t;

constexpr int TK = 64;
constexpr int TILE_B = TK * 128 * 2;

__device__ __forceinline__ int swz128(int row) { return ((row & 7) << 1) | ((row >> 3) & 1); }

struct TrAddr4 {
  unsigned base[4];
  __device__ __forceinline__ void init(unsigned tile, int lane, int blk0) {
    const int L = lane & 15, g = lane >> 4;
    const int r0 = 4 * g + (L >> 2);
#pragma unroll
    for (int i = 0; i < 4; ++i) base[i] = tile + r0 * 256 + (((2 * (blk0 + i) + ((L & 3) >> 1)) ^ swz128(r0)) << 4) + (L & 1) * 8;
  }
};
#define TN_TR(dst, addr, off) asm volatile("ds_read_b64_tr_b16 %0, %1 offset:%2" : "=v"(dst) : "v"(addr), "i"(off))

__device__ __forceinline__ bf16x8 join4(const bf16x4& lo, const bf16x4& hi) { return bf16x8{lo[0], lo[1], lo[2], lo[3], hi[0], hi[1], hi[2], hi[3]}; }

struct TnArgs {
  const bf16_t* P;
  const bf16_t* Q;
  float* C;
  long ldp, ldq, ldc;
  int T, Mo, No, stages_per_split;
};

__device__ __forceinline__ void dma_stage(char* lds, const bf16_t* base, long ld, int t0, int col0, int wave, int lane) {
#pragma unroll
  for (int j = 0; j < 4; ++j) {
    const int r0 = wave * 16 + j * 4;
    const int row = r0 + (lane >> 4);
    const int c = (lane & 15) ^ swz128(row);
    __builtin_amdgcn_global_load_lds((gptr_t)(base + (long)(t0 + row) * ld + col0 + c * 8), (lptr_t)(lds + r0 * 256), 16, 0, 0);
  }
}
__device__ __forceinline__ void reg_stage(char* lds, const bf16_t* base, long ld, int t0, int T, int col0, int tid) {
#pragma unroll
  for (int i = 0; i < 4; ++i) {
    const int idx = tid + i * 256;
    const int row = idx >> 4, c = idx & 15;
    uint4 v = make_uint4(0, 0, 0, 0);
    if (t0 + row < T) v = *reinterpret_cast<const uint4*>(base + (long)(t0 + row) * ld + col0 + c * 8);
    *reinterpret_cast<uint4*>(lds + row * 256 + ((c ^ swz128(row)) << 4)) = v;
  }
}

__global__ __launch_bounds__(256, 2) void gemm_tn_f32_kernel(TnArgs a) {
  __shared__ __attribute__((aligned(16))) char smem[2 * 2 * TILE_B];
  const int tid = threadIdx.x, lane = tid & 63;
  const int wave = __builtin_amdgcn_readfirstlane(tid >> 6);
  const int tiles_n = a.No / 128;
  const int tm = blockIdx.x / tiles_n, tn = blockIdx.x % tiles_n;
  const int wo = wave >> 1, wi = wave & 1;
  const int total_stages = (a.T + TK - 1) / TK;
  const int s0 = blockIdx.y * a.stages_per_split, s1 = min(s0 + a.stages_per_split, total_stages);
  const unsigned lds0 = (unsigned)(size_t)((__attribute__((address_space(3))) char*)smem);

  f32x4 acc[4][4];
#pragma unroll
  for (int i = 0; i < 4; ++i)
#pragma unroll
    for (int j = 0; j < 4; ++j) acc[i][j] = f32x4{0.f, 0.f, 0.f, 0.f};

  auto load = [&](int s, int buf) {
    char* p = smem + buf * 2 * TILE_B;
    const int t0 = s * TK;
    if (t0 + TK <= a.T) {
      dma_stage(p, a.P, a.ldp, t0, tm * 128, wave, lane);
      dma_stage(p + TILE_B, a.Q, a.ldq, t0, tn * 128, wave, lane);
    } else {
      reg_stage(p, a.P, a.ldp, t0, a.T, tm * 128, tid);
      reg_stage(p + TILE_B, a.Q, a.ldq, t0, a.T, tn * 128, tid);
    }
  };
  if (s0 < s1) load(s0, 0);
  for (int s = s0; s < s1; ++s) {
    const int buf = (s - s0) & 1;
    asm volatile("s_waitcnt vmcnt(0) lgkmcnt(0)" ::: "memory");
    __syncthreads();
    if (s + 1 < s1) load(s + 1, buf ^ 1);
    TrAddr4 tp, tq;
    tp.init(lds0 + buf * 2 * TILE_B, lane, wo * 4);
    tq.init(lds0 + buf * 2 * TILE_B + TILE_B, lane, wi * 4);
#pragma unroll
    for (int ks = 0; ks < 2; ++ks) {
      bf16x4 plo[4], phi[4], qlo[4], qhi[4];
#pragma unroll
      for (int i = 0; i < 4; ++i) {
        if (ks == 0) { TN_TR(plo[i], tp.base[i], 0); TN_TR(phi[i], tp.base[i], 16 * 256); TN_TR(qlo[i], tq.base[i], 0); TN_TR(qhi[i], tq.base[i], 16 * 256); }
        else { TN_TR(plo[i], tp.base[i], 32 * 256); TN_TR(phi[i], tp.base[i], 48 * 256); TN_TR(qlo[i], tq.base[i], 32 * 256); TN_TR(qhi[i], tq.base[i], 48 * 256); }
      }
      asm volatile("s_waitcnt lgkmcnt(0)"
                   : "+v"(plo[0]), "+v"(plo[1]), "+v"(plo[2]), "+v"(plo[3]), "+v"(phi[0]), "+v"(phi[1]), "+v"(phi[2]), "+v"(phi[3]),
                     "+v"(qlo[0]), "+v"(qlo[1]), "+v"(qlo[2]), "+v"(qlo[3]), "+v"(qhi[0]), "+v"(qhi[1]), "+v"(qhi[2]), "+v"(qhi[3]));
      __builtin_amdgcn_sched_barrier(0);
#pragma unroll
      for (int ob = 0; ob < 4; ++ob)
#pragma unroll
        for (int ib = 0; ib < 4; ++ib)
          acc[ob][ib] = __builtin_amdgcn_mfma_f32_16x16x32_bf16(join4(qlo[ib], qhi[ib]), join4(plo[ob], phi[ob]), acc[ob][ib], 0, 0, 0);
    }
  }
  const int L = lane & 15, g = lane >> 4;
  float* c = a.C + (long)blockIdx.y * a.Mo * a.No * (gridDim.y > 1 ? 1 : 0);
  const long ldc = gridDim.y > 1 ? a.No : a.ldc;
#pragma unroll
  for (int ob = 0; ob < 4; ++ob) {
    const int orow = tm * 128 + wo * 64 + ob * 16 + L;
#pragma unroll
    for (int ib = 0; ib < 4; ++ib) {
      const int icol = tn * 128 + wi * 64 + ib * 16 + g * 4;
      *reinterpret_cast<float4*>(c + (long)orow * ldc + icol) = make_float4(acc[ob][ib][0], acc[ob][ib][1], acc[ob][ib][2], acc[ob][ib][3]);
    }
  }
}

__global__ void tn_slab_reduce_kernel(const float* __restrict__ part, float* __restrict__ C, long ldc, int Mo, int No, int splits) {
  const long total = (long)Mo * (No / 4);
  for (long i = blockIdx.x * (long)blockDim.x + threadIdx.x; i < total; i += (long)gridDim.x * blockDim.x) {
    const long m = i / (No / 4);
    const int n = (int)(i % (No / 4)) * 4;
    float4 s = make_float4(0.f, 0.f, 0.f, 0.f);
    for (int k = 0; k < splits; ++k) {
      const float4 v = *reinterpret_cast<const float4*>(part + ((long)k * Mo + m) * No + n);
      s.x += v.x; s.y += v.y; s.z += v.z; s.w += v.w;
    }
    *reinterpret_cast<float4*>(C + m * ldc + n) = s;
  }
}

}

extern "C" int lhrs_gemm_tn_splits(int T, int Mo, int No) {
  const long tiles = (long)(Mo / 128) * (No / 128);
  if (tiles < 1 || T < 1) return 1;
  const int stages = (T + TK - 1) / TK;
  long s = (512 + tiles - 1) / tiles;
  if (s > stages / 8) s = stages / 8;
  if (s > 32) s = 32;
  return s < 1 ? 1 : (int)s;
}

extern "C" int lhrs_gemm_tn_f32(const void* P, long ldp, const void* Q, long ldq, float* C, long ldc, int T, int Mo, int No,
                                float* workspace, void* stream) {
  LHRS_REQUIRE(T > 0 && Mo > 0 && No > 0 && Mo % 128 == 0 && No % 128 == 0, "gemm_tn_f32: T=%d Mo=%d No=%d (Mo, No multiples of 128)", T, Mo, No);
  LHRS_REQUIRE(ldp % 8 == 0 && ldq % 8 == 0 && ldp >= Mo && ldq >= No && ldc % 4 == 0 && ldc >= No, "gemm_tn_f32: ldp=%ld ldq=%ld ldc=%ld", ldp, ldq, ldc);
  LHRS_REQUIRE((((size_t)P | (size_t)Q) & 15) == 0 && ((size_t)C & 15) == 0, "gemm_tn_f32: operands must be 16-byte aligned");
  const int splits = lhrs_gemm_tn_splits(T, Mo, No);
  LHRS_REQUIRE(splits == 1 || workspace != nullptr, "gemm_tn_f32: %d token splits need a workspace of splits * Mo * No floats", splits);
  const int stages = (T + TK - 1) / TK;
  TnArgs a;
  a.P = (const bf16_t*)P; a.Q = (const bf16_t*)Q; a.ldp = ldp; a.ldq = ldq; a.T = T; a.Mo = Mo; a.No = No;
  a.stages_per_split = (stages + splits - 1) / splits;
  const int used = (stages + a.stages_per_split - 1) / a.stages_per_split;
  a.C = used > 1 ? workspace : C; a.ldc = ldc;
  hipStream_t s = (hipStream_t)stream;
  hipLaunchKernelGGL(gemm_tn_f32_kernel, dim3((Mo / 128) * (No / 128), used), dim3(256), 0, s, a);
  LHRS_CHECK_LAUNCH("gemm_tn_f32");
  if (used > 1) {
    const long work = (long)Mo * (No / 4);
    int rg = (int)((work + 255) / 256); if (rg > 8192) rg = 8192;
    hipLaunchKernelGGL(tn_slab_reduce_kernel, dim3(rg), dim3(256), 0, s, workspace, C, ldc, Mo, No, used);
    LHRS_CHECK_LAUNCH("gemm_tn_f32 reduce");
  }
  return 0;
}
```

### lhrs_bot_amd/kernels.py

```python
from __future__ import annotations

import ctypes
import os
from typing import Optional

import torch

from . import _lib

ACT_NONE, ACT_QUICK_GELU, ACT_GELU, ACT_SILU = 0, 1, 2, 3
MAP_GELU, MAP_GELU_BWD, MAP_ADD, MAP_QUICK_GELU = 0, 1, 2, 3


def _L():
    return _lib.load()


def _stream() -> int:
    return torch.cuda.current_stream().cuda_stream


def _p(t: Optional[torch.Tensor]) -> Optional[int]:
    return None if t is None else t.data_ptr()


def _req(t: torch.Tensor, dtype, name: str):
    if t.dtype != dtype or not t.is_cuda:
        raise TypeError(f"{name}: expected cuda {dtype}, got {t.device} {t.dtype}")


_GEMM_WS = {}


def ensure_gemm_workspace(device) -> None:
    dev = torch.device(device)
    if dev.type != "cuda" or os.environ.get("LHRS_GEMM_WORKSPACE", "1") == "0":
        return
    idx = dev.index if dev.index is not None else torch.cuda.current_device()
    if idx in _GEMM_WS:
        return
    with torch.cuda.device(idx):
        n = int(_L().lhrs_gemm_workspace_bytes())
        ws = torch.empty(n, device=f"cuda:{idx}", dtype=torch.uint8)
        torch.cuda.synchronize()
        _lib.check(_L().lhrs_gemm_set_workspace(ws.data_ptr(), n), "gemm_set_workspace")
    _GEMM_WS[idx] = ws


def gemm_set_u4(on: bool) -> None:
    _L().lhrs_gemm_set_u4(int(bool(on)))


def gemm_u4_takes(M, N, K, lda=None, ldb=None, ldc=None, ldr=0, has_bias=False, act=0, out_f32=False, accumulate=False, alpha=1.0) -> bool:
    return bool(_L().lhrs_gemm_u4_takes(int(M), int(N), int(K), int(K if lda is None else lda), int(K if ldb is None else ldb), int(N if ldc is None else ldc),
                                        int(ldr), int(has_bias), int(act), int(out_f32), int(accumulate), float(alpha)))


GEMM_KIND_NAMES = ("gemm_nt_256s_kernel plain", "gemm_nt_256s_kernel SwiGLU-fwd", "gemm_nt_256s_kernel SwiGLU-bwd", "gemm_nt_256s_kernel RoPE", "gemm_nt_144s_kernel plain",
                   "gemm_u4_kernel<0, true> plain + residual", "gemm_u4_kernel<0, false> plain", "gemm_u4_kernel<1, false> SwiGLU-fwd", "gemm_u4_kernel<2, false> SwiGLU-bwd",
                   "gemm_u4_kernel<3, false> RoPE")


class gemm_kernel_census:

    def __enter__(self):
        _lib.check(_L().lhrs_gemm_profile_stride(1), "gemm_profile_stride")
        _lib.check(_L().lhrs_gemm_profile_enable(20000), "gemm_profile_enable")
        self.counts, self.launches = {}, 0
        return self

    def __exit__(self, *exc):
        kinds = (ctypes.c_double * 30)()
        totals = (ctypes.c_double * 5)()
        torch.cuda.synchronize()
        _lib.check(_L().lhrs_gemm_profile_read_kinds(ctypes.addressof(kinds)), "gemm_profile_read_kinds")
        _lib.check(_L().lhrs_gemm_profile_read(ctypes.addressof(totals)), "gemm_profile_read")
        _L().lhrs_gemm_profile_enable(0)
        self.counts = {GEMM_KIND_NAMES[k]: int(kinds[3 * k]) for k in range(10) if kinds[3 * k] > 0}
        self.launches = int(totals[3])
        return False


def gemm_u4_nt(a, b, out, residual=None, a2=None, b2=None) -> bool:
    ldr = residual.stride(0) if residual is not None else 0
    if a2 is not None:
        st = _L().lhrs_gemm_u4_nt_lora(a.data_ptr(), a.stride(0), b.data_ptr(), b.stride(0), a2.data_ptr(), a2.stride(0), b2.data_ptr(), b2.stride(0),
                                       a2.shape[1], out.data_ptr(), out.stride(0), a.shape[0], b.shape[0], a.shape[1], _p(residual), ldr, _stream())
    else:
        st = _L().lhrs_gemm_u4_nt(a.data_ptr(), a.stride(0), b.data_ptr(), b.stride(0), out.data_ptr(), out.stride(0), a.shape[0], b.shape[0], a.shape[1],
                                  _p(residual), ldr, _stream())
    if st < 0:
        _lib.check(st, "gemm_u4_nt")
    return st == 0


def gemm_nt(a: torch.Tensor, b: torch.Tensor, out: Optional[torch.Tensor] = None, *, bias=None, residual=None,
            act: int = ACT_NONE, out_f32: bool = False, accumulate: bool = False, alpha: float = 1.0,
            M: Optional[int] = None, N: Optional[int] = None, K: Optional[int] = None) -> torch.Tensor:
    _req(a, torch.bfloat16, "a"); _req(b, torch.bfloat16, "b")
    assert a.dim() == 2 and b.dim() == 2 and a.stride(1) == 1 and b.stride(1) == 1
    M = a.shape[0] if M is None else M
    N = b.shape[0] if N is None else N
    K = a.shape[1] if K is None else K
    if out is None:
        out = torch.empty((M, N), device=a.device, dtype=torch.float32 if out_f32 else torch.bfloat16)
    assert out.stride(1) == 1 and out.dtype == (torch.float32 if out_f32 else torch.bfloat16)
    ldr = residual.stride(0) if residual is not None else 0
    st = _L().lhrs_gemm_bf16_nt(a.data_ptr(), a.stride(0), b.data_ptr(), b.stride(0), out.data_ptr(), out.stride(0), M, N, K,
                                _p(bias), _p(residual), ldr, act, int(out_f32), int(accumulate), float(alpha), _stream())
    _lib.check(st, "gemm_bf16_nt")
    return out


def gemm_nt_lora(a, b, a2, b2, out=None, *, bias=None, residual=None, out_f32=False, accumulate=False, alpha=1.0):
    M, K = a.shape
    N, K2 = b.shape[0], a2.shape[1]
    if out is None:
        out = torch.empty((M, N), device=a.device, dtype=torch.float32 if out_f32 else torch.bfloat16)
    ldr = residual.stride(0) if residual is not None else 0
    st = _L().lhrs_gemm_bf16_nt_lora(a.data_ptr(), a.stride(0), b.data_ptr(), b.stride(0), a2.data_ptr(), a2.stride(0), b2.data_ptr(),
                                     b2.stride(0), K2, out.data_ptr(), out.stride(0), M, N, K, _p(bias), _p(residual), ldr,
                                     int(out_f32), int(accumulate), float(alpha), _stream())
    _lib.check(st, "gemm_bf16_nt_lora")
    return out


def gemm_swiglu_fwd(x, w_gu, ff, a2=None, b2=None):
    M, K = x.shape
    assert w_gu.shape[0] == 2 * ff
    gu = torch.empty((M, 2 * ff), device=x.device, dtype=torch.bfloat16)
    act = torch.empty((M, ff), device=x.device, dtype=torch.bfloat16)
    K2 = a2.shape[1] if a2 is not None else 0
    st = _L().lhrs_gemm_swiglu_fwd(x.data_ptr(), x.stride(0), w_gu.data_ptr(), w_gu.stride(0), _p(a2), a2.stride(0) if K2 else 0, _p(b2),
                                   b2.stride(0) if K2 else 0, K2, gu.data_ptr(), gu.stride(0), act.data_ptr(), act.stride(0), M, ff, K,
                                   _stream())
    _lib.check(st, "gemm_swiglu_fwd")
    return gu, act


def gemm_rope_fwd(x, w, cos_t, sin_t, *, pos_mod, pos0=0, rope_cols, head_dim, a2=None, b2=None, out=None):
    M, K = x.shape
    N = w.shape[0]
    out = torch.empty((M, N), device=x.device, dtype=torch.bfloat16) if out is None else out
    K2 = a2.shape[1] if a2 is not None else 0
    st = _L().lhrs_gemm_rope_fwd(x.data_ptr(), x.stride(0), w.data_ptr(), w.stride(0), _p(a2), a2.stride(0) if K2 else 0, _p(b2),
                                 b2.stride(0) if K2 else 0, K2, out.data_ptr(), out.stride(0), M, N, K, cos_t.data_ptr(), sin_t.data_ptr(),
                                 int(pos_mod), int(pos0), int(rope_cols), int(head_dim), _stream())
    _lib.check(st, "gemm_rope_fwd")
    return out


def gemm_swiglu_bwd(dy, w_down_t, gu, ff, a2=None, b2=None, out=None):
    M, K = dy.shape
    assert w_down_t.shape[0] == ff and gu.shape == (M, 2 * ff)
    dgu = gu if out is None else out
    K2 = a2.shape[1] if a2 is not None else 0
    L = _L()
    scratch = None
    if not L.lhrs_gemm_swiglu_fusable(M, ff, K, K, K2):
        scratch = torch.empty((M, ff), device=dy.device, dtype=torch.bfloat16)
    st = L.lhrs_gemm_swiglu_bwd(dy.data_ptr(), dy.stride(0), w_down_t.data_ptr(), w_down_t.stride(0), _p(a2), a2.stride(0) if K2 else 0,
                                _p(b2), b2.stride(0) if K2 else 0, K2, gu.data_ptr(), dgu.data_ptr(), gu.stride(0), _p(scratch), M, ff, K,
                                _stream())
    _lib.check(st, "gemm_swiglu_bwd")
    return dgu


def gemm_fp8_nt(a8, sa, b8, sb, out=None, *, residual=None, alpha=1.0, a2=None, b2=None):
    M, K = a8.shape
    N = b8.shape[0]
    assert a8.dtype == torch.uint8 and b8.dtype == torch.uint8 and sa.dtype == torch.float32 and sb.dtype == torch.float32
    if out is None:
        out = torch.empty((M, N), device=a8.device, dtype=torch.bfloat16)
    ldr = residual.stride(0) if residual is not None else 0
    if a2 is None:
        st = _L().lhrs_gemm_fp8_nt(a8.data_ptr(), a8.stride(0), sa.data_ptr(), b8.data_ptr(), b8.stride(0), sb.data_ptr(), out.data_ptr(),
                                   out.stride(0), M, N, K, _p(residual), ldr, float(alpha), _stream())
    else:
        st = _L().lhrs_gemm_fp8_nt_lora(a8.data_ptr(), a8.stride(0), sa.data_ptr(), b8.data_ptr(), b8.stride(0), sb.data_ptr(), a2.data_ptr(),
                                        a2.stride(0), b2.data_ptr(), b2.stride(0), a2.shape[1], out.data_ptr(), out.stride(0), M, N, K,
                                        _p(residual), ldr, float(alpha), _stream())
    _lib.check(st, "gemm_fp8_nt")
    return out


def gemm_nt_skinny(a, b, alpha=1.0):
    M, K = a.shape
    N = b.shape[0]
    if N > 256 or N % 64 or M < 1024 or K < 1024:
        return gemm_nt(a, b, alpha=alpha)
    out = torch.empty((M, N), device=a.device, dtype=torch.bfloat16)
    ws = torch.empty(_L().lhrs_gemm_skinny_splits(K, N) * M * N, device=a.device, dtype=torch.float32)
    st = _L().lhrs_gemm_bf16_nt_skinny(a.data_ptr(), a.stride(0), b.data_ptr(), b.stride(0), out.data_ptr(), out.stride(0), M, N, K,
                                       float(alpha), ws.data_ptr(), _stream())
    _lib.check(st, "gemm_bf16_nt_skinny")
    return out


def gemm_nt_splitk_f32(a, b, out):
    M, K = a.shape
    N = b.shape[0]
    L = _L()
    splits = L.lhrs_gemm_splitk_splits(M, N, K)
    ws = torch.empty(splits * M * N, device=a.device, dtype=torch.float32) if splits > 1 else None
    st = L.lhrs_gemm_bf16_nt_splitk_f32(a.data_ptr(), a.stride(0), b.data_ptr(), b.stride(0), out.data_ptr(), out.stride(0), M, N, K,
                                        _p(ws), _stream())
    _lib.check(st, "gemm_bf16_nt_splitk_f32")
    return out


def gemm_tn_f32(p, q, out):
    T, Mo = p.shape
    No = q.shape[1]
    L = _L()
    splits = L.lhrs_gemm_tn_splits(T, Mo, No)
    ws = torch.empty(splits * Mo * No, device=p.device, dtype=torch.float32) if splits > 1 else None
    st = L.lhrs_gemm_tn_f32(p.data_ptr(), p.stride(0), q.data_ptr(), q.stride(0), out.data_ptr(), out.stride(0), T, Mo, No, _p(ws), _stream())
    _lib.check(st, "gemm_tn_f32")
    return out


class BatchedTranspose:

    def __init__(self, pairs):
        rows, tiles = [], 0
        for src, dst in pairs:
            r, c = src.shape
            assert dst.shape == (c, r) and src.stride(1) == 1 and dst.stride(1) == 1
            rows.append([src.data_ptr(), dst.data_ptr(), src.stride(0), dst.stride(0), r, c, tiles])
            tiles += ((r + 63) // 64) * ((c + 63) // 64)
        self.keep = pairs
        self.n, self.tiles = len(rows), tiles
        self.desc = torch.tensor(rows, dtype=torch.int64).to(pairs[0][0].device)

    def run(self):
        _lib.check(_L().lhrs_transpose_batched(self.desc.data_ptr(), self.n, self.tiles, _stream()), "transpose_batched")


def dropout(x, p, seed, out=None):
    rows, cols = x.shape
    out = torch.empty((rows, cols), device=x.device, dtype=torch.bfloat16) if out is None else out
    _lib.check(_L().lhrs_dropout_bf16(x.data_ptr(), x.stride(0), out.data_ptr(), out.stride(0), rows, cols, float(p), int(seed) & 0xFFFFFFFF,
                                      _stream()), "dropout")
    return out


def gemm_nt_dropmask(a, b, p, seed, residual=None, alpha=1.0):
    M, K = a.shape
    N = b.shape[0]
    out = torch.empty((M, N), device=a.device, dtype=torch.bfloat16)
    st = _L().lhrs_gemm_bf16_nt_dropmask(a.data_ptr(), a.stride(0), b.data_ptr(), b.stride(0), out.data_ptr(), out.stride(0), M, N, K,
                                         _p(residual), residual.stride(0) if residual is not None else 0, float(alpha), float(p),
                                         int(seed) & 0xFFFFFFFF, _stream())
    _lib.check(st, "gemm_bf16_nt_dropmask")
    return out


def gemm_tn_skinny(p, q, out, accumulate=False):
    M, KP = p.shape
    N = q.shape[1]
    ns = _L().lhrs_tn_skinny_splits(M, N)
    part = torch.empty(ns * KP * N, device=p.device, dtype=torch.float32)
    st = _L().lhrs_gemm_tn_skinny(p.data_ptr(), p.stride(0), q.data_ptr(), q.stride(0), out.data_ptr(), out.stride(0), part.data_ptr(),
                                  M, N, KP, int(accumulate), _stream())
    _lib.check(st, "gemm_tn_skinny")
    return out


def blockdiag_mask(g, r, w, active_mask):
    rows, cols = g.shape
    _lib.check(_L().lhrs_blockdiag_mask(g.data_ptr(), g.stride(0), rows, cols, r, w, active_mask, _stream()), "blockdiag_mask")
    return g


def layernorm_fwd(x, gamma, beta, eps=1e-5, save_stats=False, out=None):
    rows, cols = x.shape
    y = torch.empty_like(x) if out is None else out
    mean = rstd = None
    if save_stats:
        mean = torch.empty(rows, device=x.device, dtype=torch.float32)
        rstd = torch.empty(rows, device=x.device, dtype=torch.float32)
    st = _L().lhrs_layernorm_fwd(x.data_ptr(), x.stride(0), gamma.data_ptr(), beta.data_ptr(), y.data_ptr(), y.stride(0),
                                 _p(mean), _p(rstd), rows, cols, eps, _stream())
    _lib.check(st, "layernorm_fwd")
    return (y, mean, rstd) if save_stats else y


def layernorm_bwd(dy, x, gamma, mean, rstd, dgamma=None, dbeta=None, accumulate=False, need_dx=True, add=None, out=None):
    rows, cols = x.shape
    dx = (torch.empty_like(x) if out is None else out) if need_dx else None
    assert add is None or dx is None or add.stride(0) == dx.stride(0), "layernorm_bwd: add is read with dx's row stride"
    part = None
    if dgamma is not None:
        nblk = _L().lhrs_layernorm_bwd_nblk(rows)
        part = torch.empty(nblk * 2 * cols, device=x.device, dtype=torch.float32)
    st = _L().lhrs_layernorm_bwd(dy.data_ptr(), dy.stride(0), x.data_ptr(), x.stride(0), gamma.data_ptr(), mean.data_ptr(),
                                 rstd.data_ptr(), _p(add), _p(dx), dx.stride(0) if dx is not None else 0, _p(dgamma), _p(dbeta),
                                 _p(part), int(accumulate), rows, cols, _stream())
    _lib.check(st, "layernorm_bwd")
    return dx


def rmsnorm_fwd(x, w, eps=1e-5, save_rstd=False, out=None):
    rows, cols = x.shape
    y = torch.empty_like(x) if out is None else out
    rstd = torch.empty(rows, device=x.device, dtype=torch.float32) if save_rstd else None
    st = _L().lhrs_rmsnorm_fwd(x.data_ptr(), x.stride(0), w.data_ptr(), y.data_ptr(), y.stride(0), _p(rstd), rows, cols, eps,
                               _stream())
    _lib.check(st, "rmsnorm_fwd")
    return (y, rstd) if save_rstd else y


def rmsnorm_bwd(dy, x, w, rstd=None, add=None, eps=1e-5, out=None):
    rows, cols = x.shape
    assert dy.is_contiguous() and x.is_contiguous()
    dx = torch.empty_like(x) if out is None else out
    assert dx.is_contiguous() and (add is None or add.is_contiguous()), "rmsnorm_bwd: add and out are read / written with row stride cols"
    st = _L().lhrs_rmsnorm_bwd(dy.data_ptr(), x.data_ptr(), w.data_ptr(), _p(rstd), _p(add), dx.data_ptr(), rows, cols, eps,
                               _stream())
    _lib.check(st, "rmsnorm_bwd")
    return dx


def rmsnorm_fwd_q(x, w, eps=1e-5, want_bf16=True, out=None, q_out=None):
    rows, cols = x.shape
    y = (torch.empty_like(x) if out is None else out) if want_bf16 else None
    y8, sc = q_out if q_out is not None else (torch.empty((rows, cols), device=x.device, dtype=torch.uint8),
                                              torch.empty(rows, device=x.device, dtype=torch.float32))
    st = _L().lhrs_rmsnorm_fwd_q(x.data_ptr(), x.stride(0), w.data_ptr(), _p(y), y.stride(0) if y is not None else 0, y8.data_ptr(),
                                 sc.data_ptr(), rows, cols, eps, _stream())
    _lib.check(st, "rmsnorm_fwd_q")
    return y, (y8, sc)


def rmsnorm_bwd_q(dy, x, w, rstd=None, add=None, eps=1e-5, out=None):
    rows, cols = x.shape
    assert dy.is_contiguous() and x.is_contiguous()
    dx = torch.empty_like(x) if out is None else out
    assert dx.is_contiguous() and (add is None or add.is_contiguous()), "rmsnorm_bwd_q: add and out are read / written with row stride cols"
    d8 = torch.empty((rows, cols), device=x.device, dtype=torch.uint8)
    sc = torch.empty(rows, device=x.device, dtype=torch.float32)
    st = _L().lhrs_rmsnorm_bwd_q(dy.data_ptr(), x.data_ptr(), w.data_ptr(), _p(rstd), _p(add), dx.data_ptr(), d8.data_ptr(), sc.data_ptr(),
                                 rows, cols, eps, _stream())
    _lib.check(st, "rmsnorm_bwd_q")
    return dx, (d8, sc)


def h2d(t: torch.Tensor, device) -> torch.Tensor:
    if t.is_cuda:
        return t
    return t.pin_memory().to(device, non_blocking=True)


def make_desc(entries, device) -> torch.Tensor:
    rows = []
    for e in entries:
        e = list(e)
        if len(e) == 4:
            e.append(e[3])
        if len(e) == 5:
            e.append(0)
        rows.append(e + [0, 0])
    return h2d(torch.tensor(rows, dtype=torch.int32), device)


def pad64(n: int) -> int:
    return (n + 63) // 64 * 64


def seq_transpose(x, cols, LT, desc, nseq, which: str):
    out = torch.empty((nseq, cols, LT), device=x.device, dtype=torch.bfloat16)
# ... 637 lines not shown
```

### lhrs_bot_amd/pooler.py

```python
from __future__ import annotations

from typing import Dict, List, Tuple

import torch

from . import kernels as hk

STAGE_NUM = (64, 48, 32)
SPLIT_PART = (256, 256, 256)


import os as _os

def _dw_tn_enabled() -> bool:
    return _os.environ.get("LHRS_DW_TRANSPOSED", "0") != "1"


class AttnPooler:
    def __init__(self, num_query=144, num_layers=6, num_attention_heads=16, encoder_hidden_size=1024, hidden_size=1024,
                 output_size=4096, device="cuda", **_unused):
        assert encoder_hidden_size == hidden_size, "in_proj is None in every shipped config (common_arch.py:112-115)"
        assert num_query == sum(STAGE_NUM)
        self.device = torch.device(device)
        hk.ensure_gemm_workspace(self.device)
        self.nq, self.nl, self.heads, self.d, self.out_dim = num_query, num_layers, num_attention_heads, hidden_size, output_size
        d, od = hidden_size, output_size
        spec: List[Tuple[str, Tuple[int, ...]]] = [("query", (num_query, d))]
        for l in range(num_layers):
            b = f"layers.{l}."
            spec += [(b + "ln_1.weight", (d,)), (b + "ln_1.bias", (d,)), (b + "ln_1_kv.weight", (d,)), (b + "ln_1_kv.bias", (d,)),
                     (b + "attn.in_proj_weight", (3 * d, d)), (b + "attn.in_proj_bias", (3 * d,)),
                     (b + "attn.out_proj.weight", (d, d)), (b + "attn.out_proj.bias", (d,)),
                     (b + "ln_2.weight", (d,)), (b + "ln_2.bias", (d,)),
                     (b + "mlp.c_fc.weight", (4 * d, d)), (b + "mlp.c_fc.bias", (4 * d,)),
                     (b + "mlp.c_proj.weight", (d, 4 * d)), (b + "mlp.c_proj.bias", (d,))]
        spec += [("out_proj.weight", (od, d)), ("out_proj.bias", (od,))]
        self.spec = spec
        self.offsets: Dict[str, Tuple[int, Tuple[int, ...]]] = {}
        off = 0
        for name, shape in spec:
            n = 1
            for s in shape:
                n *= s
            self.offsets[name] = (off, shape)
            off += (n + 63) // 64 * 64
        self.numel = off
        self.master = torch.zeros(off, device=self.device, dtype=torch.float32)
        self.shadow = torch.zeros(off, device=self.device, dtype=torch.bfloat16)
        self.grad = torch.zeros(off, device=self.device, dtype=torch.float32)
        self.w = {n: self._view(self.shadow, n) for n, _ in spec}
        self.g = {n: self._view(self.grad, n) for n, _ in spec}
        self.wT: Dict[str, torch.Tensor] = {}
        self.requires_grad = True
        self.initialised = False
        self._desc_cache: Dict[int, torch.Tensor] = {}
        self._ctx = None

    def _view(self, flat, name):
        off, shape = self.offsets[name]
        n = 1
        for s in shape:
            n *= s
        return flat[off: off + n].view(*shape)

    def named_parameters(self):
        return [(n, self._view(self.master, n)) for n, _ in self.spec]

    def num_parameters(self) -> int:
        return sum(self._view(self.master, n).numel() for n, _ in self.spec)

    def load_state_dict(self, sd: Dict[str, torch.Tensor], strict: bool = True):
        missing = [n for n, _ in self.spec if n not in sd]
        if strict and missing:
            raise KeyError(f"missing pooler keys: {missing[:4]}...")
        for n, _ in self.spec:
            if n in sd:
                self._view(self.master, n).copy_(sd[n].reshape(self.offsets[n][1]).to(self.device, torch.float32))
        self.sync_shadow()
        return missing

    def load_params(self, p: Dict) -> None:
        sd = {"query": p["query"], "out_proj.weight": p["out_proj_w"], "out_proj.bias": p["out_proj_b"]}
        m = {"ln1_w": "ln_1.weight", "ln1_b": "ln_1.bias", "ln1kv_w": "ln_1_kv.weight", "ln1kv_b": "ln_1_kv.bias",
             "in_w": "attn.in_proj_weight", "in_b": "attn.in_proj_bias", "out_w": "attn.out_proj.weight",
             "out_b": "attn.out_proj.bias", "ln2_w": "ln_2.weight", "ln2_b": "ln_2.bias", "fc_w": "mlp.c_fc.weight",
             "fc_b": "mlp.c_fc.bias", "proj_w": "mlp.c_proj.weight", "proj_b": "mlp.c_proj.bias"}
        for l, L in enumerate(p["layers"]):
            for k, v in L.items():
                sd[f"layers.{l}.{m[k]}"] = v
        self.load_state_dict(sd)

    def state_dict(self) -> Dict[str, torch.Tensor]:
        sd = {n: self._view(self.master, n).detach().cpu().clone() for n, _ in self.spec}
        sd["query"] = sd["query"][None]
        return sd

    def init_random(self, seed: int = 0) -> None:
        g = torch.Generator(device=self.device).manual_seed(seed)
        for n, shape in self.spec:
            v = self._view(self.master, n)
            if n == "query":
                v.copy_(torch.randn(shape, device=self.device, generator=g).clamp_(-2, 2) * 0.02)
            elif n.endswith("weight") and len(shape) == 1:
                v.fill_(1.0)
            elif n.endswith("bias"):
                v.zero_()
            else:
                bound = (6.0 / (shape[0] + shape[1])) ** 0.5 if "in_proj" in n else (1.0 / shape[1]) ** 0.5
                v.copy_((torch.rand(shape, device=self.device, generator=g) * 2 - 1) * bound)
        self.sync_shadow()
        self.initialised = True

    def sync_shadow(self) -> None:
        self.initialised = True
        hk.cast_f32_to_bf16(self.master, self.shadow)
        self.refresh_transposed()

    def refresh_transposed(self) -> None:
        if getattr(self, "_bt", None) is not None:
            self._bt.run()
            return
        d = self.d
        pairs = []
        for l in range(self.nl):
            b = f"layers.{l}."
            W = self.w[b + "attn.in_proj_weight"]
            for key, src in ((b + "q", W[:d]), (b + "kv", W[d:])):
                self.wT[key] = hk.transpose(src, out=self.wT.get(key))
                pairs.append((src, self.wT[key]))
            for key in ("attn.out_proj.weight", "mlp.c_fc.weight", "mlp.c_proj.weight"):
                self.wT[b + key] = hk.transpose(self.w[b + key], out=self.wT.get(b + key))
                pairs.append((self.w[b + key], self.wT[b + key]))
        self.wT["out_proj.weight"] = hk.transpose(self.w["out_proj.weight"], out=self.wT.get("out_proj.weight"))
        pairs.append((self.w["out_proj.weight"], self.wT["out_proj.weight"]))
        self._bt = hk.BatchedTranspose(pairs)

    def _desc(self, B: int) -> torch.Tensor:
        if B not in self._desc_cache:
            NQ, KV = self.nq, self.nq + sum(SPLIT_PART)
            ent = []
            for b in range(B):
                qo, ko = 0, 0
                for nq, ni in zip(STAGE_NUM, SPLIT_PART):
                    ent.append((b * NQ + qo, nq, b * KV + ko, nq + ni))
                    qo += nq
                    ko += nq + ni
            self._desc_cache[B] = hk.make_desc(ent, self.device)
        return self._desc_cache[B]

    def forward(self, image_embs: torch.Tensor, save_ctx: bool = True) -> torch.Tensor:
        B, d, H = image_embs.shape[0], self.d, self.heads
        w = self.w
        desc, nseq = self._desc(B), 3 * B
        LTq, LTkv = hk.pad64(max(STAGE_NUM)), hk.pad64(max(q + i for q, i in zip(STAGE_NUM, SPLIT_PART)))
        t, kv = hk.pooler_build(w["query"], image_embs.contiguous(), B, STAGE_NUM, SPLIT_PART)
        M = t.shape[0]
        scale = (d // H) ** -0.5
        layers = []
        for l in range(self.nl):
            b = f"layers.{l}."
            Win, bin_ = w[b + "attn.in_proj_weight"], w[b + "attn.in_proj_bias"]
            kvn, kv_mean, kv_rstd = hk.layernorm_fwd(kv, w[b + "ln_1_kv.weight"], w[b + "ln_1_kv.bias"], save_stats=True)
            tn, t_mean, t_rstd = hk.layernorm_fwd(t, w[b + "ln_1.weight"], w[b + "ln_1.bias"], save_stats=True)
            q = hk.gemm_nt(tn, Win[:d], bias=bin_[:d])
            kvp = hk.gemm_nt(kvn, Win[d:], bias=bin_[d:])
            o = torch.empty((M, d), device=self.device, dtype=torch.bfloat16)
            lse = torch.empty((nseq, H, LTq), device=self.device, dtype=torch.float32)
            hk.attn_fwd(q, kvp[:, :d], kvp[:, d:], o, lse, desc, nseq, H, d // H, max(STAGE_NUM), LTkv, LTq, False, scale)
            t1 = hk.gemm_nt(o, w[b + "attn.out_proj.weight"], bias=w[b + "attn.out_proj.bias"], residual=t)
            t1n, t1_mean, t1_rstd = hk.layernorm_fwd(t1, w[b + "ln_2.weight"], w[b + "ln_2.bias"], save_stats=True)
            hpre = hk.gemm_nt(t1n, w[b + "mlp.c_fc.weight"], bias=w[b + "mlp.c_fc.bias"])
            hact = hk.map_(hk.MAP_GELU, hpre)
            t2 = hk.gemm_nt(hact, w[b + "mlp.c_proj.weight"], bias=w[b + "mlp.c_proj.bias"], residual=t1)
            if save_ctx:
                layers.append(dict(t=t, tn=tn, t_stats=(t_mean, t_rstd), kvn=kvn, kv_stats=(kv_mean, kv_rstd), q=q, kvp=kvp, o=o,
                                   lse=lse, t1=t1, t1n=t1n, t1_stats=(t1_mean, t1_rstd), hpre=hpre, hact=hact))
            t = t2
        out = hk.gemm_nt(t, w["out_proj.weight"], bias=w["out_proj.bias"])
        if save_ctx:
            self._ctx = dict(B=B, kv=kv, layers=layers, t_final=t, desc=desc, LTq=LTq, LTkv=LTkv)
        return out.view(B, self.nq, self.out_dim)

    __call__ = forward

    def _dw(self, name: str, dy: torch.Tensor, x: torch.Tensor, rows=None) -> None:
        g = self.g[name] if rows is None else self.g[name][rows[0]: rows[1]]
        tn_ok = (g.shape[0] % 128 == 0 and g.shape[1] % 128 == 0 and dy.stride(1) == 1 and x.stride(1) == 1 and dy.stride(0) % 8 == 0 and
                 x.stride(0) % 8 == 0 and dy.data_ptr() % 16 == 0 and x.data_ptr() % 16 == 0 and g.data_ptr() % 16 == 0 and g.stride(1) == 1)
        if _dw_tn_enabled() and tn_ok:
            hk.gemm_tn_f32(dy, x, g)
            return
        Mp = hk.pad64(dy.shape[0])
        dyT = hk.transpose(dy, rows_pad=Mp)
        xT = hk.transpose(x, rows_pad=Mp)
        hk.gemm_nt_splitk_f32(dyT, xT, g)

    def backward(self, d_out: torch.Tensor, on_ready=None) -> None:
        c = self._ctx
        assert c is not None, "forward(save_ctx=True) must precede backward"
        B, d, H, g, w, wT = c["B"], self.d, self.heads, self.g, self.w, self.wT
        nseq, desc, LTq, LTkv = 3 * B, c["desc"], c["LTq"], c["LTkv"]
        scale = (d // H) ** -0.5
        d_out = d_out.reshape(B * self.nq, self.out_dim)
        hk.colsum(d_out, g["out_proj.bias"])
        self._dw("out_proj.weight", d_out, c["t_final"])
        dt = hk.gemm_nt(d_out, wT["out_proj.weight"])
        if on_ready:
            on_ready("out_proj")
        dkv_total = None
        for l in reversed(range(self.nl)):
            b = f"layers.{l}."
            s = c["layers"][l]
            hk.colsum(dt, g[b + "mlp.c_proj.bias"])
            self._dw(b + "mlp.c_proj.weight", dt, s["hact"])
            dh = hk.gemm_nt(dt, wT[b + "mlp.c_proj.weight"])
            dh = hk.map_(hk.MAP_GELU_BWD, dh, s["hpre"], out=dh)
            hk.colsum(dh, g[b + "mlp.c_fc.bias"])
            self._dw(b + "mlp.c_fc.weight", dh, s["t1n"])
            dt1n = hk.gemm_nt(dh, wT[b + "mlp.c_fc.weight"])
            dt1 = hk.layernorm_bwd(dt1n, s["t1"], w[b + "ln_2.weight"], *s["t1_stats"], g[b + "ln_2.weight"], g[b + "ln_2.bias"], add=dt)
            hk.colsum(dt1, g[b + "attn.out_proj.bias"])
            self._dw(b + "attn.out_proj.weight", dt1, s["o"])
            do = hk.gemm_nt(dt1, wT[b + "attn.out_proj.weight"])
            delta = torch.empty((nseq, H, LTq), device=self.device, dtype=torch.float32)
            hk.attn_delta(s["o"], do, delta, desc, nseq, H, d // H, max(STAGE_NUM), LTq)
            kvp = s["kvp"]
            dq = torch.empty_like(s["q"])
            dkvp = torch.empty_like(kvp)
            hk.attn_bwd(s["q"], kvp[:, :d], kvp[:, d:], do, s["lse"], delta, dq, dkvp[:, :d], dkvp[:, d:], desc, nseq, H, d // H,
                        max(STAGE_NUM), LTkv, LTq, False, scale)
            gb = g[b + "attn.in_proj_bias"]
            hk.colsum(dq, gb[:d])
            hk.colsum(dkvp, gb[d:])
            self._dw(b + "attn.in_proj_weight", dq, s["tn"], rows=(0, d))
            self._dw(b + "attn.in_proj_weight", dkvp, s["kvn"], rows=(d, 3 * d))
            dtn = hk.gemm_nt(dq, wT[b + "q"])
            dt = hk.layernorm_bwd(dtn, s["t"], w[b + "ln_1.weight"], *s["t_stats"], g[b + "ln_1.weight"], g[b + "ln_1.bias"], add=dt1)
            dkvn = hk.gemm_nt(dkvp, wT[b + "kv"])
            dkv_total = hk.layernorm_bwd(dkvn, c["kv"], w[b + "ln_1_kv.weight"], *s["kv_stats"], g[b + "ln_1_kv.weight"],
                                         g[b + "ln_1_kv.bias"], add=dkv_total)
            if on_ready:
                on_ready(str(l))
        hk.pooler_query_grad(dt, dkv_total, g["query"], B, STAGE_NUM, SPLIT_PART)
        if on_ready:
            on_ready("query")
        self._ctx = None
```

Measured before the change: 168.9.

## Fuse GELU into pooler MLP GEMMs, bias grads into TN dW, add half-LDS attention

```diff
diff --git a/include/lhrs_hip.h b/include/lhrs_hip.h
--- a/include/lhrs_hip.h
+++ b/include/lhrs_hip.h
@@ -36,8 +36,15 @@
 int lhrs_gemm_tn_splits(int T, int Mo, int No);
 int lhrs_gemm_tn_f32(const void* P, long ldp, const void* Q, long ldq, float* C, long ldc, int T, int Mo, int No, float* workspace,
                      void* stream);
+int lhrs_gemm_tn_f32_bias(const void* P, long ldp, const void* Q, long ldq, float* C, long ldc, float* bias_grad, int T, int Mo, int No,
+                          float* workspace, void* stream);
 int lhrs_gemm_bf16_nt_splitk_f32(const void* A, int lda, const void* B, int ldb, float* C, int ldc, int M, int N, int K,
                                  float* workspace, void* stream);
+int lhrs_gemm_gelu_fusable(int M, int N, int K);
+int lhrs_gemm_gelu_fwd(const void* X, int ldx, const void* W, int ldw, const void* bias, void* pre, int ld_pre, void* act, int ld_act, int M,
+                       int N, int K, void* stream);
+int lhrs_gemm_gelu_bwd(const void* dY, int ldy, const void* Wt, int ldw, const void* pre, int ld_pre, void* dpre, int ld_dpre, int M, int N,
+                       int K, void* stream);
 int lhrs_gemm_swiglu_fusable(int M, int ff, int K_fwd, int K_bwd, int K2);
 int lhrs_gemm_swiglu_fwd(const void* X, int ldx, const void* Wgu, int ldw, const void* A2, int lda2, const void* B2, int ldb2,
                          int K2, void* gu, int ld_gu, void* act, int ld_act, int M, int ff, int K, void* stream);
@@ -111,6 +118,8 @@
 int lhrs_attn_fwd(const void* q, long ldq, const void* k, long ldk, const void* v, long ldv, void* o, long ldo, float* lse,
                   const int* desc, int nseq, int H, int D, int max_q, int max_kv, int LTq, int causal, float scale,
                   void* stream);
+int lhrs_attn_fwd_kind(int D, int max_kv);
+int lhrs_attn_set_shared_cu(int on);
 int lhrs_attn_fwd_kmask(const void* q, long ldq, const void* k, long ldk, const void* v, long ldv, void* o, long ldo,
                         float* lse, const int* desc, int nseq, int H, int D, int max_q, int max_kv, int LTq,
                         int causal, float scale, const unsigned char* key_mask, long ld_mask, void* stream);
diff --git a/lhrs_bot_amd/csrc/attention.hip b/lhrs_bot_amd/csrc/attention.hip
--- a/lhrs_bot_amd/csrc/attention.hip
+++ b/lhrs_bot_amd/csrc/attention.hip
@@ -494,12 +494,12 @@
 #define DIAG_FLUSH() do { } while (0)
 #endif
 
-template <int D, bool CAUSAL>
-__global__ __launch_bounds__(512, 2) void attn_fwd_res_kernel(AttnArgs a) {
+template <int D, bool CAUSAL, int LDSB = 163840>
+__global__ __launch_bounds__(512, LDSB == 163840 ? 2 : 4) void attn_fwd_res_kernel(AttnArgs a) {
   constexpr int KS = D / 32, DB = D / 16, TILE = 64 * D * 2;
-  __shared__ __attribute__((aligned(16))) char smem[163840];
+  __shared__ __attribute__((aligned(16))) char smem[LDSB];
   char* lds_k = smem;
-  char* lds_v = smem + res_rows<D>() * D * 2;
+  char* lds_v = smem + LDSB / 2;
   const int seq = blockIdx.y, h = blockIdx.x;
   const int* ds = a.desc + seq * 8;
   const int q_off = ds[0], q_len = ds[1], kv_off = ds[2], kv_len = ds[3], coff = ds[5];
@@ -961,6 +961,14 @@
   return 0;
 }
 
+static int g_attn_shared_cu = 1;
+extern "C" int lhrs_attn_set_shared_cu(int on) { g_attn_shared_cu = on ? 1 : 0; return 0; }
+extern "C" int lhrs_attn_fwd_kind(int D, int max_kv) {
+  if (max_kv <= 0 || max_kv > (D == 128 ? res_rows<128>() : res_rows<64>())) return 0;
+  const long image = (long)((max_kv + 63) / 64 * 64) * D * 2 * 2;
+  return (D == 64 && image <= 81920 && g_attn_shared_cu) ? 2 : 1;
+}
+
 static int attn_fwd_impl(const void* q, long ldq, const void* k, long ldk, const void* v, long ldv, void* o, long ldo,
                          float* lse, const int* desc, int nseq, int H, int D, int max_q, int max_kv, int LTq,
                          int causal, float scale, const unsigned char* key_mask, long ld_mask, void* stream) {
@@ -973,9 +981,12 @@
   if (check_common(a, D, nseq, "attn_fwd")) return -1;
   const dim3 grid(cdiv(max_q, 64), H, nseq), blk(256);
   hipStream_t s = (hipStream_t)stream;
-  if (max_kv > 0 && max_kv <= (D == 128 ? res_rows<128>() : res_rows<64>())) {
+  if (const int kind = lhrs_attn_fwd_kind(D, max_kv)) {
     const dim3 rg(H, nseq), rb(512);
-    if (D == 128) {
+    if (kind == 2) {
+      if (causal) hipLaunchKernelGGL((attn_fwd_res_kernel<64, true, 81920>), rg, rb, 0, s, a);
+      else hipLaunchKernelGGL((attn_fwd_res_kernel<64, false, 81920>), rg, rb, 0, s, a);
+    } else if (D == 128) {
       if (causal) hipLaunchKernelGGL((attn_fwd_res_kernel<128, true>), rg, rb, 0, s, a);
       else hipLaunchKernelGGL((attn_fwd_res_kernel<128, false>), rg, rb, 0, s, a);
     } else {
diff --git a/lhrs_bot_amd/csrc/gemm.hip b/lhrs_bot_amd/csrc/gemm.hip
--- a/lhrs_bot_amd/csrc/gemm.hip
+++ b/lhrs_bot_amd/csrc/gemm.hip
@@ -369,7 +369,7 @@
 #pragma unroll
       for (int ps = 0; ps < 2; ++ps) {
         uint4 pre_a[4], pre_b[4];
-        if (SWB || (EPI == 0 && g.res)) {
+        if (SWB || EPI == 5 || (EPI == 0 && g.res)) {
 #pragma unroll
           for (int i = 0; i < 4; ++i) {
             const int m = tm * BM + wm * 64 + ps * 32 + i * 8 + rsub;
@@ -378,6 +378,8 @@
               if (SWB) {
                 pre_a[i] = *reinterpret_cast<const uint4*>(g.aux + (long)m * g.ld_aux + n);
                 pre_b[i] = *reinterpret_cast<const uint4*>(g.aux + (long)m * g.ld_aux + g.ff + n);
+              } else if (EPI == 5) {
+                pre_a[i] = *reinterpret_cast<const uint4*>(g.aux + (long)m * g.ld_aux + n);
               } else {
                 pre_a[i] = *reinterpret_cast<const uint4*>(g.res + (long)m * g.ldr + n);
               }
@@ -408,7 +410,7 @@
             for (int ni = 0; ni < 4; ++ni) {
               float v[4];
               uint2 bb = make_uint2(0, 0);
-              if (EPI == 0 && g.bias) bb = *reinterpret_cast<const uint2*>(g.bias + min(tn * BN + wn * 64 + ni * 16 + fg * 4, g.N - 4));
+              if ((EPI == 0 || EPI == 4) && g.bias) bb = *reinterpret_cast<const uint2*>(g.bias + min(tn * BN + wn * 64 + ni * 16 + fg * 4, g.N - 4));
               const float bias_v[4] = {bflo(bb.x), bfhi(bb.x), bflo(bb.y), bfhi(bb.y)};
 #pragma unroll
               for (int i = 0; i < 4; ++i) {
@@ -454,7 +456,21 @@
               val.z = pack2bf(bflo(val.z) + bflo(r.z), bfhi(val.z) + bfhi(r.z));
               val.w = pack2bf(bflo(val.w) + bflo(r.w), bfhi(val.w) + bfhi(r.w));
             }
+            if (EPI == 5) {
+              float d[8], hp[8];
+              unpack8(val, d); unpack8(pre_a[i], hp);
+#pragma unroll
+              for (int e = 0; e < 8; ++e) d[e] = d[e] * gelu_erf_grad(hp[e]);
+              val = pack8(d);
+            }
             *reinterpret_cast<uint4*>(reinterpret_cast<bf16_t*>(g.C) + (long)m * g.ldc + n) = val;
+            if (EPI == 4) {
+              float x[8];
+              unpack8(val, x);
+#pragma unroll
+              for (int e = 0; e < 8; ++e) x[e] = gelu_erf(x[e]);
+              *reinterpret_cast<uint4*>(g.aux_out + (long)m * g.ld_aux + n) = pack8(x);
+            }
           }
         }
       }
@@ -1278,6 +1294,71 @@
   return 0;
 }
 
+extern "C" int lhrs_map(int op, const void* a, const void* b, void* out, long n, void* stream);
+static bool gelu_fusable(int M, int N, int K, int lda, int ldb, int ldc, int ld2) {
+  return g_gemm_allow_256 == 2 && (long)cdiv(M, 256) * cdiv(N, 256) >= g_gemm_min256 && K % 64 == 0 && K >= 128 && N % 8 == 0 && lda % 8 == 0 &&
+         ldb % 8 == 0 && ldc % 8 == 0 && ld2 % 8 == 0;
+}
+extern "C" int lhrs_gemm_gelu_fusable(int M, int N, int K) { return gelu_fusable(M, N, K, 8, 8, 8, 8) ? 1 : 0; }
+
+static int gemm_gelu(int epi, const void* A, int lda, const void* B, int ldb, const void* bias, void* C, int ldc, void* second, int ld2, int M, int N,
+                     int K, void* stream, const char* who) {
+  LHRS_REQUIRE(M > 0 && N > 0 && K > 0 && C != nullptr && second != nullptr && ldc >= N && ld2 >= N && lda >= K && ldb >= K,
+               "%s: M=%d N=%d K=%d lda=%d ldb=%d ldc=%d ld2=%d", who, M, N, K, lda, ldb, ldc, ld2);
+  LHRS_REQUIRE((((size_t)A | (size_t)B | (size_t)C | (size_t)second) & 15) == 0 && ((size_t)bias & 7) == 0, "%s: operands must be 16-byte aligned", who);
+  hipStream_t s = (hipStream_t)stream;
+  const bool fwd = epi == 4;
+  const bool u4 = lhrs_gemm_u4_takes(M, N, K, lda, ldb, ldc, 0, bias != nullptr, 0, 0, 0, 1.f) != 0;
+  if (u4 || !gelu_fusable(M, N, K, lda, ldb, ldc, ld2)) {
+    LHRS_REQUIRE(ldc == N && ld2 == N, "%s: the unfused fallback needs dense rows (ldc=%d ld2=%d N=%d)", who, ldc, ld2, N);
+    if (lhrs_gemm_bf16_nt(A, lda, B, ldb, C, ldc, M, N, K, bias, nullptr, 0, 0, 0, 0, 1.f, stream)) return -1;
+    return fwd ? lhrs_map(0, C, nullptr, second, (long)M * N, stream) : lhrs_map(1, C, second, C, (long)M * N, stream);
+  }
+  const bool bm144 = pick_144(M, cdiv(N, 256), K, 0, false);
+  if (!bm144 && t_split_ok && g_gemm_tail_split && ldc == N && ld2 == N) {
+    const int tm = cdiv(M, 256), tn = cdiv(N, 256);
+    const long T = (long)tm * tn, full = T / 256;
+    const int tm_main = (int)(full * 256 / tn);
+    if (full >= 1 && T % 256 != 0 && tm_main >= 1 && tm_main < tm) {
+      const long t_main = (long)tm_main * tn, t_tail = T - t_main;
+      if ((double)((t_main + 255) / 256) + 2.5 * (double)t_tail / 256.0 + 0.05 < rounds_256(T)) {
+        const int M_main = tm_main * 256, M_tail = M - M_main;
+        t_split_ok = false;
+        int rc = gemm_gelu(epi, A, lda, B, ldb, bias, C, ldc, second, ld2, M_main, N, K, stream, who);
+        bf16_t* c_t = (bf16_t*)C + (long)M_main * ldc;
+        bf16_t* s_t = (bf16_t*)second + (long)M_main * ld2;
+        if (!rc) rc = gemm_launch((const bf16_t*)A + (long)M_main * lda, lda, B, ldb, c_t, ldc, M_tail, N, K, bias, nullptr, 0, 0, 0, 0, 1.f, nullptr, 0, nullptr, 0, 0, stream);
+        t_split_ok = true;
+        if (rc) return rc;
+        return fwd ? lhrs_map(0, c_t, nullptr, s_t, (long)M_tail * N, stream) : lhrs_map(1, c_t, s_t, c_t, (long)M_tail * N, stream);
+      }
+    }
+  }
+  GemmArgs g; memset(&g, 0, sizeof(g));
+  g.A = (const bf16_t*)A; g.B = (const bf16_t*)B; g.C = C; g.M = M; g.N = N; g.K = K; g.lda = lda; g.ldb = ldb; g.ldc = ldc;
+  g.alpha = 1.f; g.drop_scale = 1.f; g.epi = epi; g.ld_aux = ld2;
+  if (fwd) { g.bias = (const bf16_t*)bias; g.aux_out = (bf16_t*)second; }
+  else g.aux = (const bf16_t*)second;
+  g.tilesM = cdiv(M, bm144 ? 144 : 256); g.tilesN = cdiv(N, 256);
+  if (g_prof.on) { g_prof.launches_all++; g_prof.total_flops_all += 2.0 * M * N * K; }
+  const dim3 grid = grid_256s((long)g.tilesM * g.tilesN);
+  if (fwd) { if (bm144) LAUNCH_144(0, 4, grid, s, g); else LAUNCH_256(0, 4, grid, s, g); }
+  else { if (bm144) LAUNCH_144(0, 5, grid, s, g); else LAUNCH_256(0, 5, grid, s, g); }
+  LHRS_CHECK_LAUNCH(who);
+  return 0;
+}
+
+extern "C" int lhrs_gemm_gelu_fwd(const void* X, int ldx, const void* W, int ldw, const void* bias, void* pre, int ld_pre, void* act, int ld_act,
+                                  int M, int N, int K, void* stream) {
+  return gemm_gelu(4, X, ldx, W, ldw, bias, pre, ld_pre, act, ld_act, M, N, K, stream, "gemm_gelu_fwd");
+}
+
+extern "C" int lhrs_gemm_gelu_bwd(const void* dY, int ldy, const void* Wt, int ldw, const void* pre, int ld_pre, void* dpre, int ld_dpre, int M, int N,
+                                  int K, void* stream) {
+  LHRS_REQUIRE(pre != dpre, "gemm_gelu_bwd: dpre must not alias pre");
+  return gemm_gelu(5, dY, ldy, Wt, ldw, nullptr, dpre, ld_dpre, const_cast<void*>(pre), ld_pre, M, N, K, stream, "gemm_gelu_bwd");
+}
+
 template <int WM_FR, int WN_FR>
 __global__ __launch_bounds__(256) void gemm_fp8_small_kernel(GemmArgs g) {
   constexpr int BM = WM_FR * 32, BN = WN_FR * 32, ROWB = 128;
diff --git a/lhrs_bot_amd/csrc/gemm_144s_kernel.inc b/lhrs_bot_amd/csrc/gemm_144s_kernel.inc
--- a/lhrs_bot_amd/csrc/gemm_144s_kernel.inc
+++ b/lhrs_bot_amd/csrc/gemm_144s_kernel.inc
@@ -183,7 +183,7 @@
       for (int ps = 0; ps < 2; ++ps) {
         constexpr int NH[2] = {2, 1};
         uint4 pre_a[4], pre_b[4];
-        if (EPI == 2 || (EPI == 0 && g.res)) {
+        if (EPI == 2 || EPI == 5 || (EPI == 0 && g.res)) {
 #pragma unroll
           for (int i = 0; i < 2 * NH[ps]; ++i) {
             const int m = mrow0 + ps * 32 + i * 8 + rsub;
@@ -192,6 +192,8 @@
               if (EPI == 2) {
                 pre_a[i] = *reinterpret_cast<const uint4*>(g.aux + (long)m * g.ld_aux + n);
                 pre_b[i] = *reinterpret_cast<const uint4*>(g.aux + (long)m * g.ld_aux + g.ff + n);
+              } else if (EPI == 5) {
+                pre_a[i] = *reinterpret_cast<const uint4*>(g.aux + (long)m * g.ld_aux + n);
               } else {
                 pre_a[i] = *reinterpret_cast<const uint4*>(g.res + (long)m * g.ldr + n);
               }
@@ -222,7 +224,7 @@
             for (int ni = 0; ni < 4; ++ni) {
               float v[4];
               uint2 bb = make_uint2(0, 0);
-              if (EPI == 0 && g.bias) bb = *reinterpret_cast<const uint2*>(g.bias + min(tn * BN + wn * 64 + ni * 16 + fg * 4, g.N - 4));
+              if ((EPI == 0 || EPI == 4) && g.bias) bb = *reinterpret_cast<const uint2*>(g.bias + min(tn * BN + wn * 64 + ni * 16 + fg * 4, g.N - 4));
               const float bias_v[4] = {bflo(bb.x), bfhi(bb.x), bflo(bb.y), bfhi(bb.y)};
 #pragma unroll
               for (int i = 0; i < 4; ++i) {
@@ -264,7 +266,21 @@
               val.z = pack2bf(bflo(val.z) + bflo(r.z), bfhi(val.z) + bfhi(r.z));
               val.w = pack2bf(bflo(val.w) + bflo(r.w), bfhi(val.w) + bfhi(r.w));
             }
+            if (EPI == 5) {
+              float d[8], hp[8];
+              unpack8(val, d); unpack8(pre_a[i], hp);
+#pragma unroll
+              for (int e = 0; e < 8; ++e) d[e] = d[e] * gelu_erf_grad(hp[e]);
+              val = pack8(d);
+            }
             *reinterpret_cast<uint4*>(reinterpret_cast<bf16_t*>(g.C) + (long)m * g.ldc + n) = val;
+            if (EPI == 4) {
+              float x[8];
+              unpack8(val, x);
+#pragma unroll
+              for (int e = 0; e < 8; ++e) x[e] = gelu_erf(x[e]);
+              *reinterpret_cast<uint4*>(g.aux_out + (long)m * g.ld_aux + n) = pack8(x);
+            }
           }
         }
       }
diff --git a/lhrs_bot_amd/csrc/gemm_tn.hip b/lhrs_bot_amd/csrc/gemm_tn.hip
--- a/lhrs_bot_amd/csrc/gemm_tn.hip
+++ b/lhrs_bot_amd/csrc/gemm_tn.hip
@@ -29,6 +29,7 @@
   float* C;
   long ldp, ldq, ldc;
   int T, Mo, No, stages_per_split;
+  float* bias;
 };
 
 __device__ __forceinline__ void dma_stage(char* lds, const bf16_t* base, long ld, int t0, int col0, int wave, int lane) {
@@ -51,6 +52,7 @@
   }
 }
 
+template <bool BIAS>
 __global__ __launch_bounds__(256, 2) void gemm_tn_f32_kernel(TnArgs a) {
   __shared__ __attribute__((aligned(16))) char smem[2 * 2 * TILE_B];
   const int tid = threadIdx.x, lane = tid & 63;
@@ -68,6 +70,9 @@
 #pragma unroll
     for (int j = 0; j < 4; ++j) acc[i][j] = f32x4{0.f, 0.f, 0.f, 0.f};
 
+  const bool do_bias = BIAS && tn == 0;
+  float bsum[8] = {0.f, 0.f, 0.f, 0.f, 0.f, 0.f, 0.f, 0.f};
+
   auto load = [&](int s, int buf) {
     char* p = smem + buf * 2 * TILE_B;
     const int t0 = s * TK;
@@ -88,6 +93,18 @@
     TrAddr4 tp, tq;
     tp.init(lds0 + buf * 2 * TILE_B, lane, wo * 4);
     tq.init(lds0 + buf * 2 * TILE_B + TILE_B, lane, wi * 4);
+    if (do_bias) {
+      const char* img = smem + buf * 2 * TILE_B;
+      const int c = tid & 15;
+#pragma unroll
+      for (int i = 0; i < 4; ++i) {
+        const int row = (tid >> 4) * 4 + i;
+        float v[8];
+        unpack8(*reinterpret_cast<const uint4*>(img + row * 256 + ((c ^ swz128(row)) << 4)), v);
+#pragma unroll
+        for (int e = 0; e < 8; ++e) bsum[e] += v[e];
+      }
+    }
 #pragma unroll
     for (int ks = 0; ks < 2; ++ks) {
       bf16x4 plo[4], phi[4], qlo[4], qhi[4];
@@ -119,9 +136,23 @@
       *reinterpret_cast<float4*>(c + (long)orow * ldc + icol) = make_float4(acc[ob][ib][0], acc[ob][ib][1], acc[ob][ib][2], acc[ob][ib][3]);
     }
   }
-}
-
-__global__ void tn_slab_reduce_kernel(const float* __restrict__ part, float* __restrict__ C, long ldc, int Mo, int No, int splits) {
+  if (do_bias) {
+    __syncthreads();
+    float* red = reinterpret_cast<float*>(smem);
+#pragma unroll
+    for (int e = 0; e < 8; ++e) red[(tid >> 4) * 128 + (tid & 15) * 8 + e] = bsum[e];
+    __syncthreads();
+    if (tid < 128) {
+      float s = 0.f;
+#pragma unroll
+      for (int r = 0; r < 16; ++r) s += red[r * 128 + tid];
+      a.bias[(long)blockIdx.y * a.Mo * (gridDim.y > 1 ? 1 : 0) + tm * 128 + tid] = s;
+    }
+  }
+}
+
+__global__ void tn_slab_reduce_kernel(const float* __restrict__ part, float* __restrict__ C, long ldc, int Mo, int No, int splits,
+                                      const float* __restrict__ bpart, float* __restrict__ bias) {
   const long total = (long)Mo * (No / 4);
   for (long i = blockIdx.x * (long)blockDim.x + threadIdx.x; i < total; i += (long)gridDim.x * blockDim.x) {
     const long m = i / (No / 4);
@@ -133,6 +164,12 @@
     }
     *reinterpret_cast<float4*>(C + m * ldc + n) = s;
   }
+  if (bias != nullptr)
+    for (long i = blockIdx.x * (long)blockDim.x + threadIdx.x; i < Mo; i += (long)gridDim.x * blockDim.x) {
+      float s = 0.f;
+      for (int k = 0; k < splits; ++k) s += bpart[(long)k * Mo + i];
+      bias[i] = s;
+    }
 }
 
 }
@@ -147,27 +184,42 @@
   return s < 1 ? 1 : (int)s;
 }
 
-extern "C" int lhrs_gemm_tn_f32(const void* P, long ldp, const void* Q, long ldq, float* C, long ldc, int T, int Mo, int No,
-                                float* workspace, void* stream) {
-  LHRS_REQUIRE(T > 0 && Mo > 0 && No > 0 && Mo % 128 == 0 && No % 128 == 0, "gemm_tn_f32: T=%d Mo=%d No=%d (Mo, No multiples of 128)", T, Mo, No);
-  LHRS_REQUIRE(ldp % 8 == 0 && ldq % 8 == 0 && ldp >= Mo && ldq >= No && ldc % 4 == 0 && ldc >= No, "gemm_tn_f32: ldp=%ld ldq=%ld ldc=%ld", ldp, ldq, ldc);
-  LHRS_REQUIRE((((size_t)P | (size_t)Q) & 15) == 0 && ((size_t)C & 15) == 0, "gemm_tn_f32: operands must be 16-byte aligned");
+static int gemm_tn_launch(const void* P, long ldp, const void* Q, long ldq, float* C, long ldc, float* bias_grad, int T, int Mo, int No,
+                          float* workspace, void* stream, const char* who) {
+  LHRS_REQUIRE(T > 0 && Mo > 0 && No > 0 && Mo % 128 == 0 && No % 128 == 0, "%s: T=%d Mo=%d No=%d (Mo, No multiples of 128)", who, T, Mo, No);
+  LHRS_REQUIRE(ldp % 8 == 0 && ldq % 8 == 0 && ldp >= Mo && ldq >= No && ldc % 4 == 0 && ldc >= No, "%s: ldp=%ld ldq=%ld ldc=%ld", who, ldp, ldq, ldc);
+  LHRS_REQUIRE((((size_t)P | (size_t)Q) & 15) == 0 && ((size_t)C & 15) == 0, "%s: operands must be 16-byte aligned", who);
   const int splits = lhrs_gemm_tn_splits(T, Mo, No);
-  LHRS_REQUIRE(splits == 1 || workspace != nullptr, "gemm_tn_f32: %d token splits need a workspace of splits * Mo * No floats", splits);
+  LHRS_REQUIRE(splits == 1 || workspace != nullptr, "%s: %d token splits need a workspace of splits * (Mo * No%s) floats", who, splits, bias_grad ? " + Mo" : "");
   const int stages = (T + TK - 1) / TK;
   TnArgs a;
   a.P = (const bf16_t*)P; a.Q = (const bf16_t*)Q; a.ldp = ldp; a.ldq = ldq; a.T = T; a.Mo = Mo; a.No = No;
   a.stages_per_split = (stages + splits - 1) / splits;
   const int used = (stages + a.stages_per_split - 1) / a.stages_per_split;
   a.C = used > 1 ? workspace : C; a.ldc = ldc;
+  float* bpart = bias_grad && used > 1 ? workspace + (long)splits * Mo * No : nullptr;
+  a.bias = used > 1 ? bpart : bias_grad;
   hipStream_t s = (hipStream_t)stream;
-  hipLaunchKernelGGL(gemm_tn_f32_kernel, dim3((Mo / 128) * (No / 128), used), dim3(256), 0, s, a);
-  LHRS_CHECK_LAUNCH("gemm_tn_f32");
+  const dim3 grid((Mo / 128) * (No / 128), used);
+  if (bias_grad) hipLaunchKernelGGL(gemm_tn_f32_kernel<true>, grid, dim3(256), 0, s, a);
+  else hipLaunchKernelGGL(gemm_tn_f32_kernel<false>, grid, dim3(256), 0, s, a);
+  LHRS_CHECK_LAUNCH(who);
   if (used > 1) {
     const long work = (long)Mo * (No / 4);
     int rg = (int)((work + 255) / 256); if (rg > 8192) rg = 8192;
-    hipLaunchKernelGGL(tn_slab_reduce_kernel, dim3(rg), dim3(256), 0, s, workspace, C, ldc, Mo, No, used);
-    LHRS_CHECK_LAUNCH("gemm_tn_f32 reduce");
+    hipLaunchKernelGGL(tn_slab_reduce_kernel, dim3(rg), dim3(256), 0, s, workspace, C, ldc, Mo, No, used, bpart, bias_grad);
+    LHRS_CHECK_LAUNCH(who);
   }
   return 0;
 }
+
+extern "C" int lhrs_gemm_tn_f32(const void* P, long ldp, const void* Q, long ldq, float* C, long ldc, int T, int Mo, int No,
+                                float* workspace, void* stream) {
+  return gemm_tn_launch(P, ldp, Q, ldq, C, ldc, nullptr, T, Mo, No, workspace, stream, "gemm_tn_f32");
+}
+
+extern "C" int lhrs_gemm_tn_f32_bias(const void* P, long ldp, const void* Q, long ldq, float* C, long ldc, float* bias_grad, int T, int Mo,
+                                     int No, float* workspace, void* stream) {
+  LHRS_REQUIRE(bias_grad != nullptr && ((size_t)bias_grad & 3) == 0, "gemm_tn_f32_bias: bias_grad=%p", (void*)bias_grad);
+  return gemm_tn_launch(P, ldp, Q, ldq, C, ldc, bias_grad, T, Mo, No, workspace, stream, "gemm_tn_f32_bias");
+}
diff --git a/lhrs_bot_amd/kernels.py b/lhrs_bot_amd/kernels.py
--- a/lhrs_bot_amd/kernels.py
+++ b/lhrs_bot_amd/kernels.py
@@ -166,6 +166,28 @@
     return dgu
 
 
+def gemm_gelu_fwd(x, w, bias):
+    M, K = x.shape
+    N = w.shape[0]
+    pre = torch.empty((M, N), device=x.device, dtype=torch.bfloat16)
+    act = torch.empty((M, N), device=x.device, dtype=torch.bfloat16)
+    st = _L().lhrs_gemm_gelu_fwd(x.data_ptr(), x.stride(0), w.data_ptr(), w.stride(0), _p(bias), pre.data_ptr(), pre.stride(0), act.data_ptr(),
+                                 act.stride(0), M, N, K, _stream())
+    _lib.check(st, "gemm_gelu_fwd")
+    return pre, act
+
+
+def gemm_gelu_bwd(dy, w_t, pre):
+    M, K = dy.shape
+    N = w_t.shape[0]
+    assert pre.shape == (M, N) and pre.stride(1) == 1
+    dpre = torch.empty((M, N), device=dy.device, dtype=torch.bfloat16)
+    st = _L().lhrs_gemm_gelu_bwd(dy.data_ptr(), dy.stride(0), w_t.data_ptr(), w_t.stride(0), pre.data_ptr(), pre.stride(0), dpre.data_ptr(),
+                                 dpre.stride(0), M, N, K, _stream())
+    _lib.check(st, "gemm_gelu_bwd")
+    return dpre
+
+
 def gemm_fp8_nt(a8, sa, b8, sb, out=None, *, residual=None, alpha=1.0, a2=None, b2=None):
     M, K = a8.shape
     N = b8.shape[0]
@@ -217,6 +239,19 @@
     ws = torch.empty(splits * Mo * No, device=p.device, dtype=torch.float32) if splits > 1 else None
     st = L.lhrs_gemm_tn_f32(p.data_ptr(), p.stride(0), q.data_ptr(), q.stride(0), out.data_ptr(), out.stride(0), T, Mo, No, _p(ws), _stream())
     _lib.check(st, "gemm_tn_f32")
+    return out
+
+
+def gemm_tn_f32_bias(p, q, out, bias_out):
+    T, Mo = p.shape
+    No = q.shape[1]
+    assert bias_out.dtype == torch.float32 and bias_out.numel() == Mo and bias_out.is_contiguous()
+    L = _L()
+    splits = L.lhrs_gemm_tn_splits(T, Mo, No)
+    ws = torch.empty(splits * (Mo * No + Mo), device=p.device, dtype=torch.float32) if splits > 1 else None
+    st = L.lhrs_gemm_tn_f32_bias(p.data_ptr(), p.stride(0), q.data_ptr(), q.stride(0), out.data_ptr(), out.stride(0), bias_out.data_ptr(),
+                                 T, Mo, No, _p(ws), _stream())
+    _lib.check(st, "gemm_tn_f32_bias")
     return out
 
 
diff --git a/lhrs_bot_amd/pooler.py b/lhrs_bot_amd/pooler.py
--- a/lhrs_bot_amd/pooler.py
+++ b/lhrs_bot_amd/pooler.py
@@ -14,6 +14,10 @@
 
 def _dw_tn_enabled() -> bool:
     return _os.environ.get("LHRS_DW_TRANSPOSED", "0") != "1"
+
+
+FUSE_DW_BIAS = True
+FUSE_GELU = True
 
 
 class AttnPooler:
@@ -169,8 +173,11 @@
             hk.attn_fwd(q, kvp[:, :d], kvp[:, d:], o, lse, desc, nseq, H, d // H, max(STAGE_NUM), LTkv, LTq, False, scale)
             t1 = hk.gemm_nt(o, w[b + "attn.out_proj.weight"], bias=w[b + "attn.out_proj.bias"], residual=t)
             t1n, t1_mean, t1_rstd = hk.layernorm_fwd(t1, w[b + "ln_2.weight"], w[b + "ln_2.bias"], save_stats=True)
-            hpre = hk.gemm_nt(t1n, w[b + "mlp.c_fc.weight"], bias=w[b + "mlp.c_fc.bias"])
-            hact = hk.map_(hk.MAP_GELU, hpre)
+            if FUSE_GELU:
+                hpre, hact = hk.gemm_gelu_fwd(t1n, w[b + "mlp.c_fc.weight"], w[b + "mlp.c_fc.bias"])
+            else:
+                hpre = hk.gemm_nt(t1n, w[b + "mlp.c_fc.weight"], bias=w[b + "mlp.c_fc.bias"])
+                hact = hk.map_(hk.MAP_GELU, hpre)
             t2 = hk.gemm_nt(hact, w[b + "mlp.c_proj.weight"], bias=w[b + "mlp.c_proj.bias"], residual=t1)
             if save_ctx:
                 layers.append(dict(t=t, tn=tn, t_stats=(t_mean, t_rstd), kvn=kvn, kv_stats=(kv_mean, kv_rstd), q=q, kvp=kvp, o=o,
@@ -183,10 +190,16 @@
 
     __call__ = forward
 
-    def _dw(self, name: str, dy: torch.Tensor, x: torch.Tensor, rows=None) -> None:
+    def _dw(self, name: str, dy: torch.Tensor, x: torch.Tensor, rows=None, bias: str = None) -> None:
         g = self.g[name] if rows is None else self.g[name][rows[0]: rows[1]]
+        gb = None if bias is None else (self.g[bias] if rows is None else self.g[bias][rows[0]: rows[1]])
         tn_ok = (g.shape[0] % 128 == 0 and g.shape[1] % 128 == 0 and dy.stride(1) == 1 and x.stride(1) == 1 and dy.stride(0) % 8 == 0 and
                  x.stride(0) % 8 == 0 and dy.data_ptr() % 16 == 0 and x.data_ptr() % 16 == 0 and g.data_ptr() % 16 == 0 and g.stride(1) == 1)
+        if _dw_tn_enabled() and tn_ok and gb is not None and FUSE_DW_BIAS:
+            hk.gemm_tn_f32_bias(dy, x, g, gb)
+            return
+        if gb is not None:
+            hk.colsum(dy, gb)
         if _dw_tn_enabled() and tn_ok:
             hk.gemm_tn_f32(dy, x, g)
             return
@@ -202,8 +215,7 @@
         nseq, desc, LTq, LTkv = 3 * B, c["desc"], c["LTq"], c["LTkv"]
         scale = (d // H) ** -0.5
         d_out = d_out.reshape(B * self.nq, self.out_dim)
-        hk.colsum(d_out, g["out_proj.bias"])
-        self._dw("out_proj.weight", d_out, c["t_final"])
+        self._dw("out_proj.weight", d_out, c["t_final"], bias="out_proj.bias")
         dt = hk.gemm_nt(d_out, wT["out_proj.weight"])
         if on_ready:
             on_ready("out_proj")
@@ -211,16 +223,16 @@
         for l in reversed(range(self.nl)):
             b = f"layers.{l}."
             s = c["layers"][l]
-            hk.colsum(dt, g[b + "mlp.c_proj.bias"])
-            self._dw(b + "mlp.c_proj.weight", dt, s["hact"])
-            dh = hk.gemm_nt(dt, wT[b + "mlp.c_proj.weight"])
-            dh = hk.map_(hk.MAP_GELU_BWD, dh, s["hpre"], out=dh)
-            hk.colsum(dh, g[b + "mlp.c_fc.bias"])
-            self._dw(b + "mlp.c_fc.weight", dh, s["t1n"])
+            self._dw(b + "mlp.c_proj.weight", dt, s["hact"], bias=b + "mlp.c_proj.bias")
+            if FUSE_GELU:
+                dh = hk.gemm_gelu_bwd(dt, wT[b + "mlp.c_proj.weight"], s["hpre"])
+            else:
+                dh = hk.gemm_nt(dt, wT[b + "mlp.c_proj.weight"])
+                dh = hk.map_(hk.MAP_GELU_BWD, dh, s["hpre"], out=dh)
+            self._dw(b + "mlp.c_fc.weight", dh, s["t1n"], bias=b + "mlp.c_fc.bias")
             dt1n = hk.gemm_nt(dh, wT[b + "mlp.c_fc.weight"])
             dt1 = hk.layernorm_bwd(dt1n, s["t1"], w[b + "ln_2.weight"], *s["t1_stats"], g[b + "ln_2.weight"], g[b + "ln_2.bias"], add=dt)
-            hk.colsum(dt1, g[b + "attn.out_proj.bias"])
-            self._dw(b + "attn.out_proj.weight", dt1, s["o"])
+            self._dw(b + "attn.out_proj.weight", dt1, s["o"], bias=b + "attn.out_proj.bias")
             do = hk.gemm_nt(dt1, wT[b + "attn.out_proj.weight"])
             delta = torch.empty((nseq, H, LTq), device=self.device, dtype=torch.float32)
             hk.attn_delta(s["o"], do, delta, desc, nseq, H, d // H, max(STAGE_NUM), LTq)
@@ -229,11 +241,8 @@
             dkvp = torch.empty_like(kvp)
             hk.attn_bwd(s["q"], kvp[:, :d], kvp[:, d:], do, s["lse"], delta, dq, dkvp[:, :d], dkvp[:, d:], desc, nseq, H, d // H,
                         max(STAGE_NUM), LTkv, LTq, False, scale)
-            gb = g[b + "attn.in_proj_bias"]
-            hk.colsum(dq, gb[:d])
-            hk.colsum(dkvp, gb[d:])
-            self._dw(b + "attn.in_proj_weight", dq, s["tn"], rows=(0, d))
-            self._dw(b + "attn.in_proj_weight", dkvp, s["kvn"], rows=(d, 3 * d))
+            self._dw(b + "attn.in_proj_weight", dq, s["tn"], rows=(0, d), bias=b + "attn.in_proj_bias")
+            self._dw(b + "attn.in_proj_weight", dkvp, s["kvn"], rows=(d, 3 * d), bias=b + "attn.in_proj_bias")
             dtn = hk.gemm_nt(dq, wT[b + "q"])
             dt = hk.layernorm_bwd(dtn, s["t"], w[b + "ln_1.weight"], *s["t_stats"], g[b + "ln_1.weight"], g[b + "ln_1.bias"], add=dt1)
             dkvn = hk.gemm_nt(dkvp, wT[b + "kv"])
```

Result: no change. 169.8, median of 6 (+0.5%).
